# laomao0/BIN

Measured on AMD Instinct MI355X. Metric: interpolated frames/sec at 1280x720, higher is better.
Workload: dtype f16x3 (fp16 hi+lo pairs = 22-bit significands, 3 MFMA products, f32 accumulate; fp32-class: 1e-6 vs the fp32 reference); 1 GPU; Adobe240 test_blur 1280x720 inference, batch=1 per GPU (6-frame window padded to 768x1344 by the test.py rule), window-sharded; precision=f16x3, streams=1, pipelined_steps=False, four_call_schedule=False, parity=max-abs <= 2e-5 (f16x3) vs the fp32 reference (tests/)

## Files before the change

### __graft_entry__.py

```python
import os
import sys

REPO = os.path.dirname(os.path.abspath(__file__))
if REPO not in sys.path:
    sys.path.insert(0, REPO)


def build():
    from bin_amd.build import build_library
    path = build_library(force=True)
    import bin_amd
    from bin_amd import _lib
    lib = _lib.lib()
    missing = [s for s in _lib.exported_symbols() if not hasattr(lib, s)]
    if missing:
        raise RuntimeError(f"libbinhip.so is missing symbols: {missing}")
    _lib.optlib()
    _lib.gradlib()
    _lib.emalib()
    from oracle import rdn_oracle
    print(f"built {path} (binhip version {lib.binhip_version()})")


def smoke():
    import torch
    from bin_amd.models.archs.RDN import bin_stage4_lstm
    from bin_amd.weights import reference_state_dict, canonical_weights, synthetic_frames
    from oracle import rdn_oracle as O

    assert torch.cuda.is_available(), "smoke() needs a GPU"
    dev = torch.device("cuda:0")
    net = bin_stage4_lstm()
    net.load_state_dict(reference_state_dict(0), strict=True)
    net = net.to(dev).eval()
    frames = synthetic_frames(1234, 1, 64, 64, 6)
    canon = {k: torch.from_numpy(v) for k, v in canonical_weights(0).items()}
    with torch.no_grad():
        ref = O.bin_stage4_forward(frames, canon)
        for prec, tol in (("f16x3", 2e-5), ("f16", 1e-3)):
            net.set_precision(prec)
            out = net(*[f.to(dev) for f in frames])
            torch.cuda.synchronize()
            from bin_amd import ops
            ops.check_status()
            err = max(float((a.cpu() - b).abs().max()) for a, b in zip(out, ref))
            print(f"smoke: precision={prec} 14 outputs {tuple(out[13].shape)} max|hip-oracle| = {err:.3e} (tol {tol})")
            assert err <= tol, f"parity failure: {err} > {tol}"
    print("smoke ok")


if __name__ == "__main__":
    build()
    if "--smoke" in sys.argv:
        smoke()
```

### bin_amd/_lib.py

```python
import ctypes as C
import os

from .build import EMA_LIB_PATH, GRAD_LIB_PATH, LIB_PATH, OPT_LIB_PATH

RDN_LAYERS = 66
RDN_MAX_LAYERS, RDN_MAX_CONVS = 192, 7
PLAN_KEEP_ACTS, PLAN_NO_FUSE, PLAN_RDB3, PLAN_FUSED_UPNET, PLAN_FUSED_UPNET_TRAIN = 1, 2, 4, 8, 16
BWD_ACCUMULATE = 1
BWD_SAVED_X3 = 2
BWD_FUSED_UPNET = 4
EPI_PLANES, EPI_SHUFFLE, EPI_FINAL, EPI_FINAL_SUBPIX = 0, 1, 2, 4
PROF_WGRAD = 16
LOSS_CHARBONNIER, LOSS_L1_SUM, LOSS_L2_SUM = 0, 1, 2
RDN_LAYOUT_WORDS, RDN_BWD_LAYOUT_WORDS = 16, 24


class BinConvDesc(C.Structure):
    _fields_ = [("N", C.c_int32), ("H", C.c_int32), ("W", C.c_int32), ("ksize", C.c_int32),
                ("cin_chunks", C.c_int32), ("cout", C.c_int32), ("cout_pad", C.c_int32),
                ("nterms", C.c_int32), ("epilogue", C.c_int32), ("relu", C.c_int32),
                ("x_cpg", C.c_int32), ("x_group_stride", C.c_int64), ("n_images", C.c_int32),
                ("reserved", C.c_int32), ("status", C.c_void_p)]


LOSS_MAX_TERMS = 24
CONV_HALF_LAST_CHUNK = 1


class BinLossTerms(C.Structure):
    _fields_ = [("x", C.c_void_p * LOSS_MAX_TERMS), ("y", C.c_void_p * LOSS_MAX_TERMS), ("n_terms", C.c_int32)]


class BinLossGrads(C.Structure):
    _fields_ = [("out", C.c_void_p * LOSS_MAX_TERMS), ("term_a", C.c_int32 * LOSS_MAX_TERMS),
                ("term_b", C.c_int32 * LOSS_MAX_TERMS), ("sign_a", C.c_float * LOSS_MAX_TERMS),
                ("sign_b", C.c_float * LOSS_MAX_TERMS), ("n_out", C.c_int32)]


class BinRdnShape(C.Structure):
    _fields_ = [("G0", C.c_int32), ("D", C.c_int32), ("C", C.c_int32), ("G", C.c_int32)]


class BinRdnPlan(C.Structure):
    _fields_ = [("N", C.c_int32), ("H", C.c_int32), ("W", C.c_int32), ("n_inputs", C.c_int32),
                ("nterms", C.c_int32), ("reserved", C.c_int32), ("shape", BinRdnShape),
                ("w_hi", C.c_void_p * RDN_MAX_LAYERS), ("w_lo", C.c_void_p * RDN_MAX_LAYERS),
                ("bias", C.c_void_p * RDN_MAX_LAYERS), ("status", C.c_void_p), ("profiler", C.c_void_p)]


class BinRdnBwdPlan(C.Structure):
    _fields_ = [("N", C.c_int32), ("H", C.c_int32), ("W", C.c_int32), ("n_inputs", C.c_int32),
                ("nterms", C.c_int32), ("reserved", C.c_int32), ("shape", BinRdnShape),
                ("wt_hi", C.c_void_p * RDN_MAX_LAYERS), ("wt_lo", C.c_void_p * RDN_MAX_LAYERS),
                ("zero_bias", C.c_void_p),
                ("dw", C.c_void_p * RDN_MAX_LAYERS), ("db", C.c_void_p * RDN_MAX_LAYERS), ("gin", C.c_void_p * 5),
                ("status", C.c_void_p), ("aux_stream", C.c_void_p), ("profiler", C.c_void_p)]


class BinRelayoutItem(C.Structure):
    _fields_ = [("w", C.c_void_p * (RDN_MAX_CONVS + 1)), ("bias", C.c_void_p), ("w_hi", C.c_void_p), ("w_lo", C.c_void_p),
                ("bias_out", C.c_void_p), ("kind", C.c_int32), ("cout", C.c_int32), ("cin", C.c_int32),
                ("ksize", C.c_int32), ("rows_pad", C.c_int32), ("cin_chunks", C.c_int32), ("cout_block", C.c_int32),
                ("shuffle_or_group", C.c_int32), ("shape", BinRdnShape)]


RELAYOUT_FWD, RELAYOUT_DGRAD, RELAYOUT_RDB_GATHER = 0, 1, 2
SCORE_SSIM_G11, SCORE_SSIM_U7 = 1, 2
SCORE_MAX_PAIRS = 32

ADAM_MAX_TENSORS = 64


class BinAdamTensor(C.Structure):
    _fields_ = [("p", C.c_void_p), ("g", C.c_void_p), ("m", C.c_void_p), ("v", C.c_void_p), ("numel", C.c_int64),
                ("step_size", C.c_float), ("inv_sqrt_bc2", C.c_float)]


GRAD_MAX_TENSORS = 128
GRAD_FLAG_NONFINITE, GRAD_FLAG_STATUS = 1, 2


class BinGradTensor(C.Structure):
    _fields_ = [("g", C.c_void_p), ("numel", C.c_int64)]


class BinGradRecord(C.Structure):
    _fields_ = [("sumsq", C.c_double), ("norm", C.c_float), ("coef", C.c_float), ("flags", C.c_int32), ("status", C.c_uint32),
                ("reserved", C.c_int32 * 2)]


EMA_MAX_TENSORS = 136


class BinEmaTensor(C.Structure):
    _fields_ = [("e", C.c_void_p), ("p", C.c_void_p), ("numel", C.c_int64)]


_SIGNATURES = {
    "binhip_version": (C.c_int, []),
    "binhip_device_cus": (C.c_int, []),
    "binhip_conv_cout_block": (C.c_int, [C.c_int, C.c_int, C.c_int]),
    "binhip_weights_bytes": (C.c_size_t, [C.c_int, C.c_int, C.c_int]),
    "binhip_weights_relayout": (C.c_int, [C.c_void_p, C.c_void_p, C.c_int, C.c_int, C.c_int, C.c_int, C.c_int,
                                          C.c_int, C.c_int, C.c_void_p, C.c_void_p, C.c_void_p, C.c_void_p]),
    "binhip_weights_relayout_batch": (C.c_int, [C.POINTER(BinRelayoutItem), C.c_int, C.c_void_p]),
    "binhip_conv2d_fwd": (C.c_int, [C.POINTER(BinConvDesc)] + [C.c_void_p] * 10 +
                          [C.POINTER(C.c_void_p), C.c_void_p]),
    "binhip_nchw_to_planes": (C.c_int, [C.c_void_p, C.c_int, C.c_int, C.c_int, C.c_int, C.c_void_p, C.c_void_p,
                                        C.c_void_p, C.c_void_p]),
    "binhip_planes_to_nchw": (C.c_int, [C.c_void_p, C.c_void_p, C.c_int, C.c_int, C.c_int, C.c_int, C.c_void_p,
                                        C.c_void_p]),
    "binhip_pixel_unshuffle_f32": (C.c_int, [C.c_void_p, C.c_int, C.c_int, C.c_int, C.c_int, C.c_int, C.c_void_p,
                                             C.c_void_p]),
    "binhip_pack_inputs": (C.c_int, [C.POINTER(C.c_void_p), C.c_int, C.c_int, C.c_int, C.c_int, C.c_void_p,
                                     C.c_void_p, C.c_void_p, C.c_void_p]),
    "binhip_u8_to_frame": (C.c_int, [C.c_void_p, C.c_int, C.c_int, C.c_int, C.c_int, C.c_int, C.c_int, C.c_void_p,
                                     C.c_void_p]),
    "binhip_frame_to_u8": (C.c_int, [C.c_void_p, C.c_int, C.c_int, C.c_int, C.c_int, C.c_int, C.c_int, C.c_void_p,
                                     C.c_void_p]),
    "binhip_convlstm_fwd": (C.c_int, [C.c_void_p] * 5 + [C.c_float, C.c_int, C.c_int, C.c_int, C.c_void_p,
                                                          C.c_void_p, C.c_void_p]),
    "binhip_lstm_gates_fwd": (C.c_int, [C.c_void_p, C.c_void_p, C.c_float, C.c_int, C.c_int, C.c_int, C.c_int, C.c_void_p,
                                        C.c_void_p, C.c_void_p]),
    "binhip_lstm_gates_bwd": (C.c_int, [C.c_void_p] * 4 + [C.c_float, C.c_int, C.c_int, C.c_int, C.c_int, C.c_void_p, C.c_void_p,
                                        C.c_void_p]),
    "binhip_charbonnier_partials": (C.c_int, [C.c_int64]),
    "binhip_charbonnier_fwd": (C.c_int, [C.c_void_p, C.c_void_p, C.c_int64, C.c_float, C.c_void_p, C.c_void_p,
                                         C.c_void_p]),
    "binhip_charbonnier_bwd": (C.c_int, [C.c_void_p, C.c_void_p, C.c_int64, C.c_float, C.c_void_p, C.c_void_p,
                                         C.c_void_p, C.c_void_p]),
    "binhip_pixel_loss_fwd": (C.c_int, [C.c_int, C.c_void_p, C.c_void_p, C.c_int64, C.c_float, C.c_void_p, C.c_void_p,
                                        C.c_void_p]),
    "binhip_pixel_loss_bwd": (C.c_int, [C.c_int, C.c_void_p, C.c_void_p, C.c_int64, C.c_float, C.c_void_p, C.c_void_p,
                                        C.c_void_p, C.c_void_p]),
    "binhip_multi_loss_fwd": (C.c_int, [C.c_int, C.POINTER(BinLossTerms), C.c_int64, C.c_float, C.c_void_p, C.c_void_p,
                                        C.c_void_p, C.c_void_p]),
    "binhip_multi_loss_bwd": (C.c_int, [C.c_int, C.POINTER(BinLossTerms), C.c_int64, C.c_float, C.c_void_p,
                                        C.POINTER(BinLossGrads), C.c_void_p]),
    "binhip_dgrad_rows_pad": (C.c_int, [C.c_int, C.c_int]),
    "binhip_weights_relayout_dgrad": (C.c_int, [C.c_void_p, C.c_int, C.c_int, C.c_int, C.c_int, C.c_int, C.c_int,
                                                C.c_int, C.c_void_p, C.c_void_p, C.c_void_p, C.c_void_p]),
    "binhip_weights_relayout_rdb_gather": (C.c_int, [C.c_void_p, C.c_int, C.c_int, C.c_void_p, C.c_void_p, C.c_void_p,
                                                     C.c_void_p]),
    "binhip_conv2d_bwd_data": (C.c_int, [C.POINTER(BinConvDesc)] + [C.c_void_p] * 7 + [C.c_int, C.c_void_p,
                                         C.c_void_p, C.c_void_p, C.c_int, C.c_int, C.c_int64, C.c_void_p,
                                         C.c_void_p, C.c_void_p]),
    "binhip_wgrad_workspace_bytes": (C.c_size_t, [C.c_int] * 6),
    "binhip_conv2d_bwd_weight": (C.c_int, [C.POINTER(BinConvDesc)] + [C.c_void_p] * 6 + [C.c_size_t, C.c_void_p,
# ... 4 lines not shown
    "binhip_unshuffle_planes": (C.c_int, [C.c_void_p, C.c_void_p, C.c_int, C.c_int, C.c_int, C.c_int, C.c_void_p,
                                          C.c_void_p, C.c_void_p]),
    "binhip_unpack_input_grads": (C.c_int, [C.c_void_p, C.c_void_p, C.c_void_p, C.c_void_p, C.c_int, C.c_int, C.c_int,
                                            C.c_int, C.POINTER(C.c_void_p), C.c_void_p]),
    "binhip_convlstm_bwd_workspace_bytes": (C.c_size_t, [C.c_int, C.c_int, C.c_int]),
    "binhip_convlstm_bwd": (C.c_int, [C.c_void_p] * 5 + [C.c_float, C.c_int, C.c_int, C.c_int, C.c_void_p, C.c_void_p,
                                      C.c_void_p, C.c_size_t] + [C.c_void_p] * 6),
    "binhip_rdn_backward_workspace_bytes": (C.c_size_t, [C.c_int] * 5 + [C.POINTER(BinRdnShape)]),
    "binhip_rdn_backward": (C.c_int, [C.POINTER(BinRdnBwdPlan), C.c_void_p, C.c_size_t, C.c_void_p, C.c_void_p,
                                      C.c_size_t, C.c_void_p]),
    "binhip_profiler_create": (C.c_int, [C.c_int, C.c_int, C.c_int, C.c_int, C.POINTER(C.c_void_p)]),
    "binhip_profiler_read": (C.c_int, [C.c_void_p, C.POINTER(C.c_double), C.POINTER(C.c_int)]),
    "binhip_profiler_destroy": (None, [C.c_void_p]),
    "binhip_rdb_tail_fwd": (C.c_int, [C.c_int, C.c_int, C.c_int, C.c_int] + [C.c_void_p] * 10 +
                            [C.c_int, C.c_void_p, C.c_void_p]),
    "binhip_rdn_workspace_bytes": (C.c_size_t, [C.c_int, C.c_int, C.c_int, C.c_int, C.c_int, C.POINTER(BinRdnShape)]),
    "binhip_rdn_workspace_layout": (C.c_int, [C.c_int] * 5 + [C.POINTER(BinRdnShape), C.POINTER(C.c_int64), C.c_int]),
    "binhip_rdn_backward_workspace_layout": (C.c_int, [C.c_int] * 5 + [C.POINTER(BinRdnShape), C.POINTER(C.c_int64), C.c_int]),
    "binhip_rdn_forward": (C.c_int, [C.POINTER(BinRdnPlan), C.POINTER(C.c_void_p), C.c_void_p, C.c_void_p,
                                     C.c_size_t, C.c_void_p]),
    "binhip_image_score_workspace_bytes": (C.c_size_t, [C.c_int] * 4),
    "binhip_image_score": (C.c_int, [C.c_void_p, C.c_void_p, C.c_int, C.c_int, C.c_int, C.c_int, C.POINTER(C.c_double),
                                     C.c_void_p, C.c_size_t, C.c_void_p, C.c_void_p]),
    "binhip_frame_score_workspace_bytes": (C.c_size_t, [C.c_int] * 4),
    "binhip_frame_score": (C.c_int, [C.POINTER(C.c_void_p), C.POINTER(C.c_void_p), C.c_int, C.c_int, C.c_int, C.c_int,
                                     C.POINTER(C.c_double), C.c_void_p, C.c_size_t, C.c_void_p, C.c_void_p]),
    "binhip_gather_windows": (C.c_int, [C.c_void_p, C.c_int, C.c_int, C.c_int, C.c_void_p, C.c_int, C.c_int, C.c_int, C.c_int,
                                        C.c_void_p, C.c_void_p]),
    "binhip_gather_windows_blur": (C.c_int, [C.c_void_p, C.c_int, C.c_int, C.c_int, C.c_void_p] + [C.c_int] * 5 +
                                   [C.c_void_p, C.c_void_p]),
}

OPT_VERSION = 100
_OPT_SIGNATURES = {
    "binopt_version": (C.c_int, []),
    "binopt_adam_step": (C.c_int, [C.POINTER(BinAdamTensor), C.c_int, C.c_float, C.c_float, C.c_float, C.c_float, C.c_void_p]),
}

GRAD_VERSION = 100
_GRAD_SIGNATURES = {
    "bingrad_version": (C.c_int, []),
    "bingrad_norm_workspace_bytes": (C.c_int64, [C.POINTER(BinGradTensor), C.c_int]),
    "bingrad_norm": (C.c_int, [C.POINTER(BinGradTensor), C.c_int, C.c_float, C.c_void_p, C.c_uint32, C.c_void_p, C.c_void_p,
                               C.c_void_p]),
    "bingrad_scale": (C.c_int, [C.POINTER(BinGradTensor), C.c_int, C.c_void_p, C.c_void_p]),
}

EMA_VERSION = 100
_EMA_SIGNATURES = {
    "binema_version": (C.c_int, []),
    "binema_step": (C.c_int, [C.POINTER(BinEmaTensor), C.c_int, C.c_float, C.c_void_p]),
}

STATUS_SATURATED = 1
STATUS_SYNC_TIMEOUT = 2

_lib = None


def exported_symbols():
    return sorted(_SIGNATURES)


def lib():
    global _lib
    if _lib is None:
        path = os.environ.get("BIN_AMD_LIB", LIB_PATH)
        if not os.path.exists(path):
            raise RuntimeError(
                f"bin_amd: HIP library {LIB_PATH} not built. Run `python -c 'import __graft_entry__ as g; "
                f"g.build()'` (hipcc --offload-arch=gfx950). There is no CPU fallback by design.")
        h = C.CDLL(path)
        for name, (res, args) in _SIGNATURES.items():
            fn = getattr(h, name)
            fn.restype = res
            fn.argtypes = args
        _lib = h
    return _lib


_optlib = None


def opt_exported_symbols():
    return sorted(_OPT_SIGNATURES)


def optlib():
    global _optlib
    if _optlib is None:
        path = OPT_LIB_PATH
        if not os.path.exists(path):
            raise RuntimeError(
                f"bin_amd: HIP library {OPT_LIB_PATH} not built. Run `python -c 'import __graft_entry__ as g; "
                f"g.build()'` (hipcc --offload-arch=gfx950). There is no CPU fallback by design.")
        h = C.CDLL(path)
        for name, (res, args) in _OPT_SIGNATURES.items():
            fn = getattr(h, name)
            fn.restype = res
            fn.argtypes = args
        if h.binopt_version() != OPT_VERSION:
            raise RuntimeError(f"bin_amd: {path} is version {h.binopt_version()}, this binding is for {OPT_VERSION}")
        _optlib = h
    return _optlib


_gradlib = None


def grad_exported_symbols():
    return sorted(_GRAD_SIGNATURES)


def gradlib():
    global _gradlib
    if _gradlib is None:
        path = GRAD_LIB_PATH
        if not os.path.exists(path):
            raise RuntimeError(
                f"bin_amd: HIP library {GRAD_LIB_PATH} not built. Run `python -c 'import __graft_entry__ as g; "
                f"g.build()'` (hipcc --offload-arch=gfx950). There is no CPU fallback by design.")
        h = C.CDLL(path)
        for name, (res, args) in _GRAD_SIGNATURES.items():
            fn = getattr(h, name)
            fn.restype = res
            fn.argtypes = args
        if h.bingrad_version() != GRAD_VERSION:
            raise RuntimeError(f"bin_amd: {path} is version {h.bingrad_version()}, this binding is for {GRAD_VERSION}")
        _gradlib = h
    return _gradlib


_emalib = None


def ema_exported_symbols():
    return sorted(_EMA_SIGNATURES)


def emalib():
    global _emalib
    if _emalib is None:
        path = EMA_LIB_PATH
        if not os.path.exists(path):
            raise RuntimeError(
                f"bin_amd: HIP library {EMA_LIB_PATH} not built. Run `python -c 'import __graft_entry__ as g; "
                f"g.build()'` (hipcc --offload-arch=gfx950). There is no CPU fallback by design.")
        h = C.CDLL(path)
        for name, (res, args) in _EMA_SIGNATURES.items():
            fn = getattr(h, name)
            fn.restype = res
            fn.argtypes = args
        if h.binema_version() != EMA_VERSION:
            raise RuntimeError(f"bin_amd: {path} is version {h.binema_version()}, this binding is for {EMA_VERSION}")
        _emalib = h
    return _emalib


def check(rc, what):
    if rc != 0:
        kind = {-1: "bad argument", -2: "unsupported shape", -3: "workspace too small"}.get(rc, f"hipError {rc}")
        raise RuntimeError(f"bin_amd: {what} failed: {kind}")
```

### bin_amd/autograd.py

```python
import ctypes as C
import os

import torch

from . import _lib as L
from .ops import _ptr, _stream, on_device, status_word
from .rdn_plan import c_shape, layer_names, rdn_forward, workspace



def default_wgrad_side_stream():
    return os.environ.get("BIN_AMD_WGRAD_STREAM", "1") != "0"


_aux_streams = {}


def _aux_stream(device):
    s = _aux_streams.get(device.index)
    if s is None:
        s = torch.cuda.Stream(device=device)
        _aux_streams[device.index] = s
    return s


def train_fused_upnet():
    return os.environ.get("BIN_AMD_FUSED_UPNET_TRAIN", "1") != "0"


def default_backward_precision():
    return os.environ.get("BIN_AMD_BACKWARD_PRECISION") or None


def train_precision(module):
    from .models.archs.RDN import PRECISIONS
    p = module.precision or os.environ.get("BIN_AMD_TRAIN_PRECISION", "f16x3")
    if PRECISIONS[p] == 1 and not getattr(module, "allow_f16_training", False):
        if not any(q.requires_grad for q in module.parameters()):
            if not getattr(module, "_warned_f16_input_grads", False):
                import warnings
                warnings.warn("bin_amd: differentiating through an RDN in precision 'f16' with frozen parameters: input gradients "
                              "are computed with single fp16 products (a few per cent of noise); use 'f16x3' for fp32-class gradients",
                              stacklevel=3)
                module._warned_f16_input_grads = True
            return PRECISIONS[p]
        raise RuntimeError(
            "bin_amd: training with precision 'f16' (one fp16 product in forward and backward) is not a supported mode — its "
            "parameter gradients are only verified to 25 %.  Train in 'f16x3' (the default; set network_G.precision: f16x3 or "
            "leave it unset), optionally with network_G.backward_precision: f16 for the faster mixed mode; 'f16' is the "
            "inference mode (wrap inference in torch.no_grad()).  To train in it regardless (it converged like f16x3 on the synthetic "
            "task of profiles/r06_training_modes.md) set network_G.allow_f16_training: true, or module.allow_f16_training = True.")
    return PRECISIONS[p]


class _RdnFn(torch.autograd.Function):
    @staticmethod
    def forward(ctx, module, nterms, n_frames, *args):
        frames = [a.contiguous().float() for a in args[:n_frames]]
        weights = module.kernel_weights(nterms)
        n, _, h, w = frames[0].shape
        lib = L.lib()
        nbytes = lib.binhip_rdn_workspace_bytes(n, h, w, n_frames, nterms, C.byref(c_shape(weights.shape)))
        if nbytes == 0:
            raise RuntimeError(f"bin_amd: unsupported RDN shape N={n} H={h} W={w}")
        saved = torch.empty(nbytes, dtype=torch.uint8, device=frames[0].device)
        fused = (bool(module.plan_flags & L.PLAN_FUSED_UPNET) and train_fused_upnet() and
                 weights.ensure_fused_upnet(train=True) is not None)
        flags = module.plan_flags | L.PLAN_KEEP_ACTS | (L.PLAN_FUSED_UPNET_TRAIN if fused else 0)
        out = rdn_forward(weights, frames, ws=saved, flags=flags, profiler=module.profiler)
        ctx.fused_up = fused
        if module.debug_hook is not None:
            module.debug_hook("forward", module, (n, h, w, n_frames, nterms), saved, {"shape": module.shape, "fused_upnet": fused})
        ctx.module, ctx.nterms, ctx.n_frames = module, nterms, n_frames
        ctx.saved_ws = saved
        ctx.weights = weights
        ctx.dims = (n, h, w)
        ctx.param_meta = [(tuple(a.shape), a.device) for a in args[n_frames:]]
        ctx.params = args[n_frames:]
        ctx.param_versions = [(a._version, a.data_ptr()) for a in args[n_frames:]]
        ctx.weights_gen = module._wgen
        module._bwd_pending = getattr(module, "_bwd_pending", 0) + 1
        ctx.owes_backward = True
        return out

    @staticmethod
    def backward(ctx, gout):
        if ctx.saved_ws is None:
            raise RuntimeError("bin_amd: the saved activations of this RDN call were released by an earlier backward through it (the "
                               "forward's private workspace is freed as soon as its backward has run or was refused; "
                               "retain_graph=True does not keep it): run the forward again")
        try:
            return _RdnFn._backward(ctx, gout)
        except BaseException:
            ctx.saved_ws = ctx.weights = None
            _RdnFn._settle(ctx)
            raise

    @staticmethod
    def _settle(ctx):
        if ctx.owes_backward:
            ctx.owes_backward = False
            ctx.module._bwd_pending = getattr(ctx.module, "_bwd_pending", 1) - 1

    @staticmethod
    def _backward(ctx, gout):
        module, nterms, k = ctx.module, ctx.nterms, ctx.n_frames
        n, h, w = ctx.dims
        if ctx.weights_gen != module._wgen or any((a._version, a.data_ptr()) != v for a, v in zip(ctx.params, ctx.param_versions)):
            raise RuntimeError("bin_amd: a parameter of this RDN was modified in place between its forward and its backward "
                               "(optimizer step, load_state_dict, broadcast, re-pointed storage ...): the gradient would be computed with "
                               "weights the forward did not use")
        dev = gout.device
        gout = gout.contiguous().float()
        lib = L.lib()
        weights = ctx.weights
        fused = ctx.fused_up
        nt_bwd = 1 if (module.backward_precision == "f16" and nterms == 3) else nterms
        dgw = weights.dgrad(module, nt_bwd, fused=fused)
        plan = L.BinRdnBwdPlan()
        plan.N, plan.H, plan.W, plan.n_inputs, plan.nterms = n, h, w, k, nt_bwd
        if nt_bwd != nterms:
            plan.reserved = L.BWD_SAVED_X3
        dgw.fill_plan(plan)
        plan.status = status_word(dev).data_ptr()
        plan.aux_stream = (_aux_stream(dev).cuda_stream
                           if module.wgrad_side_stream and not torch.cuda.is_current_stream_capturing() else None)
        plan.profiler = module.bwd_profiler if module.bwd_profiler else None
        params = ctx.params
        direct = module._direct_grads and all(ctx.needs_input_grad[3 + k:])
        have = False
        if direct:
            states = [p.grad is not None for p in params]
            have = all(states)
            direct = (have or not any(states)) and all(
                p.grad is None or (p.grad.dtype == torch.float32 and p.grad.is_contiguous() and p.grad.device == dev)
                for p in params)
        if direct and have:
            grads = [p.grad for p in params]
            plan.reserved |= L.BWD_ACCUMULATE
        else:
            grads = [torch.empty(shape, dtype=torch.float32, device=dev) for shape, _ in ctx.param_meta]
        for i in range(len(grads) // 2):
            plan.dw[i] = grads[2 * i].data_ptr()
            plan.db[i] = grads[2 * i + 1].data_ptr()
        if fused:
            nl, g0 = len(grads) // 2, module.shape[0]
            plan.reserved |= L.BWD_FUSED_UPNET
            up_dw4 = torch.empty((12, g0, 5, 5), dtype=torch.float32, device=dev)
            up_db4 = torch.empty((12,), dtype=torch.float32, device=dev)
            up_dwr = torch.zeros((n, 9, 12, 25, g0), dtype=torch.float32, device=dev)
            up_dbr = torch.zeros((n, 9, 12), dtype=torch.float32, device=dev)
            plan.dw[nl], plan.db[nl], plan.dw[nl + 1], plan.db[nl + 1] = (up_dw4.data_ptr(), up_db4.data_ptr(), up_dwr.data_ptr(),
                                                                        up_dbr.data_ptr())
        gins = []
        for i in range(k):
            if ctx.needs_input_grad[3 + i]:
                g = torch.empty((n, 3, h, w), dtype=torch.float32, device=dev)
                plan.gin[i] = g.data_ptr()
                gins.append(g)
            else:
                plan.gin[i] = None
                gins.append(None)
        nbytes = lib.binhip_rdn_backward_workspace_bytes(n, h, w, k, nt_bwd, C.byref(plan.shape))
        ws = workspace(nbytes, dev, key="bwd")
        with on_device(gout):
            L.check(lib.binhip_rdn_backward(C.byref(plan), _ptr(ctx.saved_ws), ctx.saved_ws.numel(), _ptr(gout),
                                            _ptr(ws), ws.numel(), _stream()), "rdn_backward")
        if module.debug_hook is not None:
            module.debug_hook("backward", module, (n, h, w, k, nt_bwd), ws, {"input_grads": any(g is not None for g in gins),
                                                                              "shape": module.shape, "fused_upnet": fused})
        ctx.saved_ws = ctx.weights = None
        if fused:
            nl = len(grads) // 2
            dW = up_dwr.sum(0)
            dB = up_dbr.sum(0)
            dW[4], dB[4] = up_dw4.reshape(12, g0, 25).permute(0, 2, 1), up_db4
            leaves, Wr, Br = weights.fused_graph
            gup = torch.autograd.grad([Wr, Br], leaves, [dW, dB], retain_graph=True)
            for slot, g in zip((2 * (nl - 2), 2 * (nl - 2) + 1, 2 * (nl - 1), 2 * (nl - 1) + 1), gup):
                if plan.reserved & L.BWD_ACCUMULATE:
                    grads[slot].add_(g.float())
                else:
                    grads[slot].copy_(g.float())
        _RdnFn._settle(ctx)
        if module._bwd_pending == 0 and direct:
            cb = getattr(module, "_grads_ready_cb", None)
            if cb is not None:
                cb()
        if direct:
            if not have:
                for p, g in zip(params, grads):
                    p.grad = g
            return (None, None, None, *gins, *([None] * len(grads)))
        pgrads = [g if ctx.needs_input_grad[3 + k + i] else None for i, g in enumerate(grads)]
        return (None, None, None, *gins, *pgrads)


def rdn_apply(module, frames):
    nterms = train_precision(module)
    params = dict(module.named_parameters())
    flat = []
    for nm in layer_names(module.shape):
        flat += [params[nm + ".weight"], params[nm + ".bias"]]
    return _RdnFn.apply(module, nterms, len(frames), *frames, *flat)


class _ConvLstmFn(torch.autograd.Function):
    @staticmethod
    def forward(ctx, x, c_prev, h_prev, weight, bias, forget_bias):
        from . import ops
        state = None if c_prev is None else [c_prev, h_prev]
        h, (c, _) = ops.convlstm_cell(x, state, weight, bias, forget_bias)
        ctx.save_for_backward(x.contiguous().float(), None if c_prev is None else c_prev.contiguous().float(),
                              None if h_prev is None else h_prev.contiguous().float(),
                              weight.detach().contiguous().float(), bias.detach().contiguous().float())
        ctx.fb = float(forget_bias)
        return h, c

    @staticmethod
    def backward(ctx, gh, gc):
        x, cp, hp, w, b = ctx.saved_tensors
        n, _, hh, ww = x.shape
        dev = x.device
        lib = L.lib()
        gh = gh.contiguous().float() if gh is not None else None
        gc = gc.contiguous().float() if gc is not None else None
        if gh is None and gc is None:
            return None, None, None, None, None, None
        gx = torch.empty_like(x) if ctx.needs_input_grad[0] else None
        gcp = torch.empty_like(x) if (cp is not None and ctx.needs_input_grad[1]) else None
        ghp = torch.empty_like(x) if (hp is not None and ctx.needs_input_grad[2]) else None
        need_w = ctx.needs_input_grad[3] or ctx.needs_input_grad[4]
        dw = torch.zeros_like(w) if need_w else None
        db = torch.zeros_like(b) if need_w else None
        ws = workspace(lib.binhip_convlstm_bwd_workspace_bytes(n, hh, ww), dev, key="clstm")
        L.check(lib.binhip_convlstm_bwd(_ptr(x), _ptr(cp), _ptr(hp), _ptr(w), _ptr(b), ctx.fb, n, hh, ww, _ptr(gh),
                                        _ptr(gc), _ptr(ws), ws.numel(), _ptr(gx), _ptr(ghp), _ptr(gcp), _ptr(dw),
                                        _ptr(db), _stream()), "convlstm_bwd")
        return gx, gcp, ghp, dw, db, None


GENERAL_NTERMS = 3


class _ConvFn(torch.autograd.Function):

    @staticmethod
    def forward(ctx, x, weight, bias):
        from . import ops
        nt = GENERAL_NTERMS
        cw = ops.ConvWeights(weight, bias, nterms=nt)
        xp = ops.nchw_to_planes(x, nt)
        y = ops.planes_to_nchw(ops.conv2d(xp, cw), weight.shape[0])
        ctx.xp, ctx.weight, ctx.has_bias = xp, weight, bias is not None
        ctx.weight_version = weight._version
        return y

    @staticmethod
    def backward(ctx, gy):
        from . import ops
        nt = GENERAL_NTERMS
        if ctx.weight._version != ctx.weight_version:
            raise RuntimeError("bin_amd: a ConvLSTM gate weight was modified in place between forward and backward "
                               "(optimizer step / broadcast / load_state_dict): its gradient would not belong to the forward")
        cout, cin, ks, _ = ctx.weight.shape
        gp, sc = ops.grad_planes(gy, nt)
        dw = db = gx = None
        if ctx.needs_input_grad[1] or ctx.needs_input_grad[2]:
            dw, db = ops.conv2d_bwd_weight(ctx.xp, gp, cout, cin, ks, nt, inv_scale=sc[1:2])
        if ctx.needs_input_grad[0]:
            gxs = ops.planes_to_nchw(ops.conv2d_bwd_data(gp, ops.DgradWeights(ctx.weight, nterms=nt)), cin)
            gx = gxs * sc[1]
        return gx, dw, (db if ctx.has_bias else None)


class _LstmGatesFn(torch.autograd.Function):
    @staticmethod
    def forward(ctx, gates, c_prev, forget_bias, hidden):
        from . import ops
        c1, h1 = ops.lstm_gates(gates, c_prev, forget_bias, hidden)
        ctx.save_for_backward(gates, c_prev)
        ctx.fb, ctx.hidden = float(forget_bias), hidden
        return h1, c1

    @staticmethod
    def backward(ctx, gh, gc):
        from . import ops
# ... 24 lines not shown
```

### bin_amd/build.py

```python
import os
import subprocess
import sys

HERE = os.path.dirname(os.path.abspath(__file__))
CSRC = os.path.join(HERE, "csrc")
SOURCES = ["binhip_conv.hip", "binhip_conv_x3.hip", "binhip_fused.hip", "binhip_fused_x3.hip", "binhip_wgrad.hip", "binhip_misc.hip", "binhip_plan.hip",
           "binhip_metrics.hip", "binhip_data.hip"]
LIB_PATH = os.path.join(CSRC, "libbinhip.so")
OPT_SOURCES = ["binopt_adam.hip"]
OPT_LIB_PATH = os.path.join(CSRC, "libbinopt.so")
OPT_HEADER = os.path.join(os.path.dirname(HERE), "include", "binopt.h")
GRAD_SOURCES = ["bingrad_norm.hip"]
GRAD_LIB_PATH = os.path.join(CSRC, "libbingrad.so")
GRAD_HEADER = os.path.join(os.path.dirname(HERE), "include", "bingrad.h")
EMA_SOURCES = ["binema_step.hip"]
EMA_LIB_PATH = os.path.join(CSRC, "libbinema.so")
EMA_HEADER = os.path.join(os.path.dirname(HERE), "include", "binema.h")


HEADER = os.path.join(os.path.dirname(HERE), "include", "binhip.h")


def abi_symbols():
    import re
    with open(HEADER) as f:
        return re.findall(r"(?m)^BINHIP_API\s+[\w\s\*]+?\b(binhip_\w+)\s*\(", f.read())


def opt_abi_symbols():
    import re
    with open(OPT_HEADER) as f:
        return re.findall(r"(?m)^BINOPT_API\s+[\w\s\*]+?\b(binopt_\w+)\s*\(", f.read())


def grad_abi_symbols():
    import re
    with open(GRAD_HEADER) as f:
        return re.findall(r"(?m)^BINGRAD_API\s+[\w\s\*]+?\b(bingrad_\w+)\s*\(", f.read())


def ema_abi_symbols():
    import re
    with open(EMA_HEADER) as f:
        return re.findall(r"(?m)^BINEMA_API\s+[\w\s\*]+?\b(binema_\w+)\s*\(", f.read())


def _stale():
    libs = (LIB_PATH, OPT_LIB_PATH, GRAD_LIB_PATH, EMA_LIB_PATH)
    if not all(os.path.exists(p) for p in libs):
        return True
    t = min(os.path.getmtime(p) for p in libs)
    deps = [os.path.join(CSRC, f) for f in os.listdir(CSRC) if f.endswith((".hip", ".h"))]
    deps += [os.path.join(os.path.dirname(HERE), "include", "binhip.h"), OPT_HEADER, GRAD_HEADER, EMA_HEADER]
    return any(os.path.getmtime(d) > t for d in deps)


def build_library(force=False, verbose=True, defines=(), out=None):
    lib_path = out or LIB_PATH
    if out is None and not force and not _stale():
        return LIB_PATH
    hipcc = os.environ.get("HIPCC", "/opt/rocm/bin/hipcc")
    objdir = CSRC if out is None else os.path.dirname(os.path.abspath(out))
    os.makedirs(objdir, exist_ok=True)
    tag = "" if out is None else "." + os.path.splitext(os.path.basename(out))[0]
    procs, objs, opt_objs, grad_objs, ema_objs = [], [], [], [], []
    for src in SOURCES + (OPT_SOURCES + GRAD_SOURCES + EMA_SOURCES if out is None else []):
        obj = os.path.join(objdir, src.replace(".hip", tag + ".o"))
        cmd = [hipcc, "--offload-arch=gfx950", "-O3", "-std=c++17", "-fPIC", "-fvisibility=hidden"] + [f"-D{d}" for d in defines] + \
              ["-c", os.path.join(CSRC, src), "-o", obj]
        if verbose:
            print(" ".join(cmd), file=sys.stderr)
        procs.append((cmd, subprocess.Popen(cmd)))
        (opt_objs if src in OPT_SOURCES else grad_objs if src in GRAD_SOURCES else ema_objs if src in EMA_SOURCES else objs).append(obj)
    for cmd, p in procs:
        if p.wait() != 0:
            raise subprocess.CalledProcessError(p.returncode, cmd)
    vmap = os.path.join(objdir, "binhip_exports" + tag + ".map")
    names = abi_symbols() + (["binhip_set_timeline"] if any(d.startswith("BINHIP_TIMELINE") for d in defines) else [])
    with open(vmap, "w") as f:
        f.write("{\n  global:\n" + "".join(f"    {n};\n" for n in names) + "  local: *;\n};\n")
    cmd = [hipcc, "--offload-arch=gfx950", "-shared", "-fPIC", "-Wl,-z,defs", f"-Wl,--version-script={vmap}",
           "-o", lib_path] + objs
    if verbose:
        print(" ".join(cmd), file=sys.stderr)
    subprocess.check_call(cmd)
    for name, symbols, path, lib_objs in ((("binopt", opt_abi_symbols(), OPT_LIB_PATH, opt_objs),
                                           ("bingrad", grad_abi_symbols(), GRAD_LIB_PATH, grad_objs),
                                           ("binema", ema_abi_symbols(), EMA_LIB_PATH, ema_objs)) if out is None else ()):
        vmap = os.path.join(objdir, f"binhip_exports.{name}.map")
        with open(vmap, "w") as f:
            f.write("{\n  global:\n" + "".join(f"    {n};\n" for n in symbols) + "  local: *;\n};\n")
        cmd = [hipcc, "--offload-arch=gfx950", "-shared", "-fPIC", "-Wl,-z,defs", f"-Wl,--version-script={vmap}",
               "-o", path] + lib_objs
        if verbose:
            print(" ".join(cmd), file=sys.stderr)
        subprocess.check_call(cmd)
    return lib_path


if __name__ == "__main__":
    build_library(force="--force" in sys.argv)
    print(LIB_PATH)
```

### bin_amd/csrc/binhip_conv.hip

```cpp
#include "binhip_conv_common.h"
#include <vector>
#include <cstdio>
#include <cstdlib>

template <int KS, int MT, int WM, int R, int WN, int KC, int NT, int NBUF, int EPI>
struct ConvCfg {
    static constexpr int PAD = KS / 2;
    static constexpr int COUTB = 32 * MT * WM;
    static constexpr int TH = R * WN;
    static constexpr int PH = TH + KS - 1;
    static constexpr int PW = 32 + KS - 1;
    static constexpr int PP = (PH * PW * 2 + 63) / 64;
    static constexpr int WP = KS * KS * MT * WM;
    static constexpr int CHUNK_BYTES = (PP + WP) * 1024;
    static constexpr int NPL = (NT == 3) ? 2 : 1;
    static constexpr int PLANE_BYTES = KC * CHUNK_BYTES;
    static constexpr int BUF_BYTES = NPL * PLANE_BYTES;
    static constexpr int NW = WM * WN;
    static constexpr int LDS_BYTES = NBUF * BUF_BYTES + 1024;
    static constexpr int NPJ = (PP + NW - 1) / NW;
    static constexpr int NWJ = (WP + NW - 1) / NW;
    static constexpr int PS = NPL * KC * (NPJ + NWJ);
    static_assert(NW == 4 || NW == 8 || NW == 16, "4, 8 or 16 waves per workgroup");
    static_assert(LDS_BYTES <= 160 * 1024, "LDS budget");
// ... 221 lines not shown
    int ks = 0, cout_pad = 0, epi = 0;
    std::vector<hipEvent_t> ev;
    size_t used = 0;
};
namespace { constexpr size_t PROF_MAX_PAIRS = 16384; }

int bh_conv_cout_block(int ksize, int cout_pad, int nterms) {
    if (cout_pad <= 0 || cout_pad % 32) return -1;
    if (ksize == 3 && nterms == 3) return 32;
    if (ksize == 3 && cout_pad == 256) return 128;
    if (ksize == 5) return 32;
    if (ksize == 1 && cout_pad == 224) return 224;
    if (ksize == 1 && cout_pad == 1152) return 192;
    if (cout_pad % 96 == 0) return 96;
    if (ksize == 3 && cout_pad % 64 == 0) return 64;
    return 32;
}

static int bh_dispatch_conv(const ConvKArgs& a, int k, int cp, int nt, int e, hipStream_t s);
int bh_launch_conv_x3(const ConvKArgs& a, int cout_pad, int epilogue, hipStream_t s);
int bh_launch_final_dot2(const ConvKArgs& a, hipStream_t s);
int bh_launch_conv_x3_k5(const ConvKArgs& a, int cout_pad, hipStream_t s);
int bh_launch_conv_x3_k5_subpix(const ConvKArgs& a, hipStream_t s);
int bh_launch_final_m16(const ConvKArgs& a, hipStream_t s);

int bh_prepare_conv(const BhConvCall& c, ConvKArgs* out) {
    const BinConvDesc& d = c.d;
    if (!c.x_hi || !c.w_hi || !c.bias) return BINHIP_E_ARG;
    if (d.nterms != 1 && d.nterms != 3) return BINHIP_E_ARG;
    if (d.nterms == 3 && (!c.x_lo || !c.w_lo)) return BINHIP_E_ARG;
    if (d.N <= 0 || d.H <= 0 || d.W <= 0 || d.cin_chunks <= 0) return BINHIP_E_SHAPE;
    if ((long long)d.N * d.H * d.W >= (1ll << 26)) return BINHIP_E_SHAPE;
    ConvKArgs a;
    a.x_hi = (const _Float16*)c.x_hi; a.x_lo = (const _Float16*)c.x_lo;
    a.w_hi = (const _Float16*)c.w_hi; a.w_lo = (const _Float16*)c.w_lo;
    a.bias = c.bias;
    a.y_hi = (_Float16*)c.y_hi; a.y_lo = (_Float16*)c.y_lo;
    a.r_hi = (const _Float16*)c.r_hi; a.r_lo = (const _Float16*)c.r_lo;
    a.r2_hi = (const _Float16*)c.r2_hi; a.r2_lo = (const _Float16*)c.r2_lo;
    a.m_hi = (const _Float16*)c.m_hi;
    a.flags = (unsigned*)c.status;
    a.res_chunks = c.res_chunks > 0 ? c.res_chunks : (1 << 30);
    a.mask_from = c.mask_from;
    a.y_cpg = c.y_cpg; a.y_group_stride = c.y_group_stride;
    a.y_cpg_inv = c.y_cpg > 0 ? (unsigned)(((1u << 20) + c.y_cpg - 1) / c.y_cpg) : 0u;
    if (c.y_cpg > 128 || (c.y_cpg > 0 && d.cout_pad / 16 >= 4096)) return BINHIP_E_SHAPE;
    a.half_last = (d.reserved & BINHIP_CONV_HALF_LAST_CHUNK) ? 1 : 0;
    a.y_unshuf = c.y_unshuf;
    if (c.y_unshuf && (d.epilogue != BINHIP_EPI_PLANES || c.y_cpg > 0 || (d.H & 1) || (d.W & 1) || c.y_unshuf * 16 < d.cout))
        return BINHIP_E_SHAPE;
    if (c.r2_hi && d.nterms == 3 && !c.r2_lo) return BINHIP_E_ARG;
    a.out_f32 = c.y_f32;
    for (int i = 0; i < 5; ++i) a.img[i] = c.images[i];
    a.group_stride = d.x_group_stride;
    a.N = d.N; a.H = d.H; a.W = d.W;
    a.nchunks = d.cin_chunks;
    a.cpg = d.x_cpg;
    a.relu = d.relu; a.has_res = (c.r_hi != nullptr); a.nimg = d.n_images; a.cout = d.cout;
    a.och_limit = (d.epilogue == BINHIP_EPI_PLANES) ? (d.cout + 15) / 16 : (1 << 30);
    a.tiles_x = a.tiles_y = 0;
    a.ncol = 1;
    a.xcd_remap = 1;
    a.dbg = 0;
    a.wt = 0;
    a.prog_prio = 0;
#if BINHIP_TIMELINE
    a.tl = nullptr; a.tl_launch = 0; a.tl_base = 0;
#endif
    const int P = BINHIP_EPI_PLANES, S = BINHIP_EPI_SHUFFLE, F = BINHIP_EPI_FINAL;
    if (d.epilogue == P) {
        if (!c.y_hi || (d.nterms == 3 && !c.y_lo)) return BINHIP_E_ARG;
        if (a.has_res && d.nterms == 3 && !c.r_lo) return BINHIP_E_ARG;
    } else if (d.epilogue == S) {
        if (!c.y_hi || (d.nterms == 3 && !c.y_lo)) return BINHIP_E_ARG;
        if (d.cout % 4) return BINHIP_E_SHAPE;
    } else if (d.epilogue == F) {
        if (!c.y_f32 || d.cout > 4 || d.n_images < 0 || d.n_images > 5) return BINHIP_E_ARG;
    } else if (d.epilogue == BINHIP_EPI_FINAL_SUBPIX) {
        if (!c.y_f32 || d.cout <= 0 || (d.cout & 3) || d.cout > 12 || d.n_images < 0 || d.n_images > 5) return BINHIP_E_ARG;
        if (d.ksize != 5 || d.cout_pad != 32) return BINHIP_E_SHAPE;
    } else {
        return BINHIP_E_ARG;
    }
    {
        const int e = d.epilogue, cp = d.cout_pad;
        const long long out_chunks = (e == BINHIP_EPI_SHUFFLE) ? (a.cout / 4 + 15) / 16 : (cp + 15) / 16;
        const long long px = (long long)a.N * a.H * a.W * ((e == BINHIP_EPI_SHUFFLE) ? 4 : 1);
        const long long span = (a.y_cpg > 0 ? ((out_chunks + a.y_cpg - 1) / a.y_cpg) * a.y_group_stride * 2 : out_chunks * px * 32);
        a.wt = (e == BINHIP_EPI_PLANES && span < (1ll << 32) - 64) ? 1 : 0;
    }
    *out = a;
    return 0;
}

bool bh_prof_begin(BinhipProfiler* pr, int ks, int cout_pad, int epi, hipStream_t s) {
    if (!pr || ks != pr->ks || cout_pad != pr->cout_pad || epi != pr->epi || pr->used + 2 > pr->ev.size()) return false;
    (void)hipEventRecord(pr->ev[pr->used], s);
    return true;
}
void bh_prof_end(BinhipProfiler* pr, hipStream_t s) {
    (void)hipEventRecord(pr->ev[pr->used + 1], s);
    pr->used += 2;
}

int bh_launch_conv(const BhConvCall& c, hipStream_t s) {
    ConvKArgs a;
// ... 407 lines not shown
```

### bin_amd/csrc/binhip_conv_common.h

```cpp
#pragma once
#include "binhip_internal.h"
#ifndef BINHIP_TIMELINE
#define BINHIP_TIMELINE 0
#endif

typedef _Float16 half8 __attribute__((ext_vector_type(8)));
typedef _Float16 half4 __attribute__((ext_vector_type(4)));
typedef float floatx16 __attribute__((ext_vector_type(16)));
typedef float floatx4 __attribute__((ext_vector_type(4)));
typedef __attribute__((address_space(3))) void lds_void_t;
typedef unsigned u32x4 __attribute__((ext_vector_type(4)));

int bh_launch_upnet_ring(const void* x_hi, const void* x_lo, const float* wvar, const float* bvar, float* out, const float* const* images,
                         int nimg, int N, int H, int W, int cin, hipStream_t s);
int bh_upnet_gsub(const float* g, int N, int H, int W, const float* scale, void* y_hi, void* y_lo, void* status, hipStream_t s);
int bh_upnet_ring_dgrad(const float* g, const float* wvar, const float* scale, void* gx_hi, void* gx_lo, void* status, int N, int H, int W,
                        int cin, hipStream_t s);
int bh_upnet_ring_wgrad(const float* g, const void* x_hi, const void* x_lo, float* dwvar, float* dbvar, int N, int H, int W, int cin,
                        int accumulate, hipStream_t s);
struct ConvKArgs {
    const _Float16* x_hi;
    const _Float16* x_lo;
    const _Float16* w_hi;
    const _Float16* w_lo;
    const float* bias;
    _Float16* y_hi;
    _Float16* y_lo;
    const _Float16* r_hi;
    const _Float16* r_lo;
    const _Float16* r2_hi;
    const _Float16* r2_lo;
    const _Float16* m_hi;
    float* out_f32;
    const float* img[5];
    unsigned* flags;
    long long group_stride;
    int N, H, W;
    int nchunks;
    int cpg;
    int tiles_x, tiles_y;
    int ncol;
    int relu, has_res, nimg, cout;
    int xcd_remap;
    int wt;
    int och_limit;
    int dbg;
    int res_chunks;
    int mask_from;
    int y_cpg;
    unsigned y_cpg_inv;
    long long y_group_stride;
    int prog_prio;
    int half_last;
#if BINHIP_TIMELINE
    void* tl;
    unsigned tl_launch;
    unsigned tl_base;
#endif
    int y_unshuf;
};

#if BINHIP_TIMELINE
#include <atomic>
struct BhTlRec {
    unsigned kind_launch, bid, hwid, xcc;
    unsigned long long rt[5];
    unsigned long long clk[2];
    unsigned long long pad;
};
static_assert(sizeof(BhTlRec) == 80, "record size (tools/wg_timeline.py)");
struct BhTlBuf { unsigned cursor, cap, pad[2]; BhTlRec rec[1]; };
inline void* g_bh_tl_buf = nullptr;
inline unsigned g_bh_tl_cap = 0;
inline std::atomic<unsigned> g_bh_tl_serial{0}, g_bh_tl_next{0};
inline void* bh_tl_reserve(unsigned n, unsigned* base) {
    if (!g_bh_tl_buf) return nullptr;
    const unsigned b = g_bh_tl_next.fetch_add(n);
    *base = b;
    return (b + n <= g_bh_tl_cap) ? g_bh_tl_buf : nullptr;
}
struct BhTl {
    unsigned long long rt[5], clk[2];
    __device__ __forceinline__ void stamp(int i) {
        __builtin_amdgcn_sched_barrier(0);
        rt[i] = __builtin_amdgcn_s_memrealtime();
        __builtin_amdgcn_sched_barrier(0);
    }
    __device__ __forceinline__ void begin() { clk[0] = __builtin_amdgcn_s_memtime(); stamp(0); }
    __device__ __forceinline__ void finish(void* tl, unsigned kind_launch, unsigned i) {
        stamp(3);
        if (threadIdx.x < 64) asm volatile("s_waitcnt vmcnt(0)" ::: "memory");
        stamp(4);
        clk[1] = __builtin_amdgcn_s_memtime();
        if (tl && threadIdx.x == 0) {
            BhTlBuf* b = (BhTlBuf*)tl;
            {
                BhTlRec& r = b->rec[i];
                r.kind_launch = kind_launch; r.bid = blockIdx.x;
                r.hwid = __builtin_amdgcn_s_getreg((31 << 11) | 4);
                r.xcc = __builtin_amdgcn_s_getreg((31 << 11) | 20);
                for (int k = 0; k < 5; ++k) r.rt[k] = rt[k];
                r.clk[0] = clk[0]; r.clk[1] = clk[1];
            }
        }
    }
};
#define BH_TL_DECL BhTl tl__
#define BH_TL_BEGIN() tl__.begin()
#define BH_TL_STAMP(i) tl__.stamp(i)
#define BH_TL_FINISH(a, i) tl__.finish((a).tl, (a).tl_launch, (a).tl_base + (unsigned)(i))
#else
#define BH_TL_DECL
#define BH_TL_BEGIN()
#define BH_TL_STAMP(i)
#define BH_TL_FINISH(a, i)
#endif

#define BINHIP_EPI_PLANES_LFFD 3

template <int N>
__device__ __forceinline__ void wait_vmcnt() {
    asm volatile("s_waitcnt vmcnt(%0)" ::"n"(N) : "memory");
}

__device__ __forceinline__ void store16(_Float16* base, long long off_elems, uint4 v, int wt) {
    if (wt) {
        __amdgpu_buffer_rsrc_t rs = __builtin_amdgcn_make_buffer_rsrc((void*)base, 0, 0xFFFFFFFFu, 0x00020000);
        u32x4 d = {v.x, v.y, v.z, v.w};
        __builtin_amdgcn_raw_buffer_store_b128(d, rs, (int)(off_elems * 2), 0, 16);
    } else {
        *reinterpret_cast<uint4*>(base + off_elems) = v;
    }
}

__device__ __forceinline__ int xcd_band(int bid, int nwg) {
    const int q = nwg >> 3, r = nwg & 7, xcd = bid & 7, k = bid >> 3;
    return (xcd < r ? xcd * (q + 1) : r * (q + 1) + (xcd - r) * q) + k;
}

template <int MT, int R, int NT, int EPI, bool XTRA>
__device__ __forceinline__ void conv_epilogue(const ConvKArgs& a, const float* __restrict__ bias, floatx16 (&acc)[MT][R],
                                              int img, int row0, int tx0, int co0, bool first_col, int n, int kg,
                                              long long plane_elems) {
    const int H = a.H, W = a.W;
    const int gx = tx0 + n;
    auto bias4 = [&](int co_u, float (&bv)[4]) {
        float b8[8];
#pragma unroll
        for (int j = 0; j < 8; ++j) b8[j] = bias[co_u + j];
#pragma unroll
        for (int j = 0; j < 4; ++j) bv[j] = kg ? b8[4 + j] : b8[j];
    };
    if constexpr (EPI == BINHIP_EPI_FINAL_SUBPIX) {
        const int ncolour = a.cout >> 2;
        const int H2 = 2 * H, W2 = 2 * W;
        float bv[2][4];
        bias4(co0, bv[0]);
        bias4(co0 + 8, bv[1]);
        const bool col_ok = first_col && (gx < W);
        float sum[R][2][4];
#pragma unroll
        for (int r = 0; r < R; ++r) {
            const int gy = row0 + r;
#pragma unroll
            for (int g = 0; g < 2; ++g) {
                const int c = 2 * g + kg;
                const bool ok = col_ok && gy < H && c < ncolour;
#pragma unroll
                for (int q = 0; q < 4; ++q) {
                    float sj = 0.f;
                    if (ok && a.nimg > 0) {
                        const long long idx = (((long long)img * ncolour + c) * H2 + 2 * gy + (q >> 1)) * W2 + 2 * gx + (q & 1);
                        sj = a.img[0][idx];
                        for (int t = 1; t < a.nimg; ++t) sj += a.img[t][idx];
                        sj = sj / (float)a.nimg;
                    }
                    sum[r][g][q] = sj;
                }
            }
        }
#pragma unroll
        for (int r = 0; r < R; ++r) {
            const int gy = row0 + r;
#pragma unroll
            for (int g = 0; g < 2; ++g) {
                const int c = 2 * g + kg;
                if (!(col_ok && gy < H && c < ncolour)) continue;
#pragma unroll
                for (int q = 0; q < 4; ++q) {
                    const long long idx = (((long long)img * ncolour + c) * H2 + 2 * gy + (q >> 1)) * W2 + 2 * gx + (q & 1);
                    a.out_f32[idx] = (acc[0][r][4 * g + q] + bv[g][q]) + sum[r][g][q];
                }
            }
        }
    } else if constexpr (EPI == BINHIP_EPI_FINAL) {
        float bv[4];
        bias4(co0, bv);
        const bool mine = (kg == 0) && first_col && (gx < W);
        float sum[R][4];
#pragma unroll
        for (int r = 0; r < R; ++r) {
            const int gy = row0 + r;
#pragma unroll
            for (int j = 0; j < 4; ++j) {
                float sj = 0.f;
                if (mine && gy < H && j < a.cout && a.nimg > 0) {
                    const long long idx = (((long long)img * a.cout + j) * H + gy) * W + gx;
                    sj = a.img[0][idx];
                    for (int t = 1; t < a.nimg; ++t) sj += a.img[t][idx];
                    sj = sj / (float)a.nimg;
                }
                sum[r][j] = sj;
            }
        }
#pragma unroll
        for (int r = 0; r < R; ++r) {
            const int gy = row0 + r;
            if (!(mine && gy < H)) continue;
#pragma unroll
            for (int j = 0; j < 4; ++j) {
                if (j >= a.cout) break;
                const long long idx = (((long long)img * a.cout + j) * H + gy) * W + gx;
                a.out_f32[idx] = (acc[0][r][j] + bv[j]) + sum[r][j];
            }
        }
    } else {
        union H4 { half4 h; unsigned u[2]; };
        unsigned sat = 0;
        const int gxc = gx < W ? gx : W - 1;
        constexpr bool X = XTRA && (EPI == BINHIP_EPI_PLANES || EPI == BINHIP_EPI_PLANES_LFFD);
        constexpr int MTG = (X && MT >= 6) ? 2 : 1;
        const bool use_res = X && a.has_res;
        const bool use_r2 = X && (a.r2_hi != nullptr);
        const bool use_m = X && (a.m_hi != nullptr);
        constexpr bool LFFD = EPI == BINHIP_EPI_PLANES_LFFD;
        static_assert(!LFFD || (XTRA && MT == 7 && NT == 3), "the LFF backward-data epilogue");
        if constexpr (LFFD) {
            {
#pragma unroll
                for (int r = 0; r < R; ++r) {
                    const int gy = row0 + r;
                    const bool ok = (gy < H) && (gx < W);
                    const int gyc = gy < H ? gy : H - 1;
                    const long long pix = (((long long)img * H + gyc) * W + gxc) << 4;
                    auto emit = [&](const int mt, const half4 (&xr)[4], const half4 (&xrl)[4], const half4 (&xm)[4], const int kind)
                        __attribute__((always_inline)) {
#pragma unroll
                        for (int gp = 0; gp < 2; ++gp) {
                            H4 hv[2], lv[2];
                            long long o_slot = 0;
#pragma unroll
                            for (int ge = 0; ge < 2; ++ge) {
                                const int g = 2 * gp + ge;
                                float bv[4];
                                bias4(mt * 32 + 8 * g, bv);
                                float v[4] = {acc[mt][r][4 * g + 0] + bv[0], acc[mt][r][4 * g + 1] + bv[1],
                                              acc[mt][r][4 * g + 2] + bv[2], acc[mt][r][4 * g + 3] + bv[3]};
                                const int co = mt * 32 + 8 * g + 4 * kg;
                                const long long o = (long long)(co >> 4) * plane_elems + pix + (co & 15);
                                if (kind == 1) {
#pragma unroll
                                    for (int j = 0; j < 4; ++j) v[j] += (float)xr[g][j];
// ... 208 lines not shown
```

### bin_amd/csrc/binhip_conv_x3.hip

```cpp
#include "binhip_conv_common.h"
constexpr int X3_R = 2, X3_WN = 8;

template <int KS, int R, int WN>
struct X3Cfg {
    static constexpr int PAD = KS / 2;
    static constexpr int TH = R * WN;
    static constexpr int PH = TH + KS - 1;
    static constexpr int PW = 32 + KS - 1;
    static constexpr int PP = (PH * PW * 2 + 63) / 64;
    static constexpr int WP = KS * KS;
    static constexpr int NW = WN;
    static constexpr int PATCH_BYTES = PP * 1024;
    static constexpr int WBUF_BYTES = 2 * WP * 1024;
    static constexpr int LDS_BYTES = 2 * PATCH_BYTES + 2 * WBUF_BYTES;
    static constexpr int NPJ = (PP + NW - 1) / NW;
    static constexpr int NWJ = (2 * WP + NW - 1) / NW;
    static_assert((KS == 3 ? 2 : 1) * LDS_BYTES <= 160 * 1024, "LDS budget");
};

template <class C>
__device__ __forceinline__ void x3_issue_patch(const ConvKArgs& a, char* smem, int c, int pl, int buf, int wave,
                                               const unsigned* voff, long long plane_elems, unsigned plane_bytes) {
    const _Float16* xb = pl ? a.x_lo : a.x_hi;
    const long long coff = (a.cpg > 0) ? (long long)(c / a.cpg) * a.group_stride + (long long)(c % a.cpg) * plane_elems
// ... 414 lines not shown
    union W2 { unsigned u; half2v p; };

    const int nchunks = a.nchunks;
    auto compute = [&](const char* pb, int c, bool hi_plane) {
        const unsigned* wh = w_hi32 + (long long)c * (9 * 32 * 8);
        const unsigned* wl = w_lo32 + (long long)c * (9 * 32 * 8);
#pragma unroll
        for (int t = 0; t < 9; ++t) {
            const int dy = t / 3, dx = t % 3;
#pragma unroll
            for (int cg = 0; cg < 2; ++cg) {
                X8 x;
                x.h = *reinterpret_cast<const half8*>(pb + cg * (C::PH * C::PW * 16) + base_off + (dy * C::PW + dx) * 16);
#pragma unroll
                for (int r = 0; r < 3; ++r) {
#pragma unroll
                    for (int k = 0; k < 4; ++k) {
                        W2 w;
                        w.u = wh[(t * 32 + r) * 8 + cg * 4 + k];
                        acc[r] = __builtin_amdgcn_fdot2(x.p[k], w.p, acc[r], false);
                        if (NT == 3 && hi_plane) {
                            W2 v;
                            v.u = wl[(t * 32 + r) * 8 + cg * 4 + k];
                            acc[r] = __builtin_amdgcn_fdot2(x.p[k], v.p, acc[r], false);
                        }
                    }
                }
            }
        }
    };

    x3_issue_patch<C>(a, smem, 0, 0, 0, wave, voff, plane_elems, plane_bytes);
    for (int c = 0; c < nchunks; ++c) {
        wait_vmcnt<0>();
        __builtin_amdgcn_s_barrier();
        __builtin_amdgcn_sched_barrier(0);
        if constexpr (NT == 3) {
            x3_issue_patch<C>(a, smem, c, 1, 1, wave, voff, plane_elems, plane_bytes);
            compute(smem, c, true);
            wait_vmcnt<0>();
            __builtin_amdgcn_s_barrier();
            __builtin_amdgcn_sched_barrier(0);
            if (c + 1 < nchunks) x3_issue_patch<C>(a, smem, c + 1, 0, 0, wave, voff, plane_elems, plane_bytes);
            compute(smem + C::PATCH_BYTES, c, false);
        } else {
            if (c + 1 < nchunks) x3_issue_patch<C>(a, smem, c + 1, 0, (c + 1) & 1, wave, voff, plane_elems, plane_bytes);
            compute(smem + (c & 1) * C::PATCH_BYTES, c, true);
        }
    }
    const int gy = ty0 + py, gx = tx0 + px;
    if (gy < H && gx < W) {
        float sum[3], bj[3];
        const int nimg = a.nimg;
#pragma unroll
        for (int j = 0; j < 3; ++j) {
            const long long idx = (((long long)img * a.cout + (j < a.cout ? j : 0)) * H + gy) * W + gx;
            float v[5];
#pragma unroll
            for (int t = 0; t < 5; ++t) v[t] = (t < nimg) ? a.img[t][idx] : 0.f;
            bj[j] = a.bias[j < a.cout ? j : 0];
            float sj = v[0];
#pragma unroll
            for (int t = 1; t < 5; ++t)
                if (t < nimg) sj += v[t];
            sum[j] = nimg > 0 ? sj / (float)nimg : 0.f;
        }
#pragma unroll
        for (int j = 0; j < 3; ++j) asm volatile("" : "+v"(sum[j]), "+v"(bj[j]));
        __builtin_amdgcn_sched_barrier(0);
#pragma unroll
        for (int j = 0; j < 3; ++j) {
            if (j >= a.cout) break;
            const long long idx = (((long long)img * a.cout + j) * H + gy) * W + gx;
            a.out_f32[idx] = (acc[j] + bj[j]) + sum[j];
        }
    }
}

struct M16 {
    using C = X3Cfg<3, 2, 8>;
    static constexpr int NSTAGE = 3;
    static constexpr int WPIECES = 5;
    static constexpr int W_OFF = NSTAGE * C::PATCH_BYTES;
    static constexpr int LDS_BYTES = W_OFF + 2 * WPIECES * 1024;
    static_assert(2 * LDS_BYTES <= 160 * 1024, "two workgroups per CU");
};

template <bool HI>
__device__ __forceinline__ void m16_compute(const char* pb, const char* wb, int a_lane_off, int b_lane_off, int slot, int a_zero,
                                            floatx4 (&acc)[2][2]) {
    using C = X3Cfg<3, 2, 8>;
    half8 Ah[2], Al[2], B[2][2][2];
    auto tap_off = [](int t) { return ((t / 3) * C::PW + (t % 3)) * 16; };
    auto load = [&](int p, half8& ah, half8& al, half8 (&b)[2][2]) {
        const int aoff = (p < 4) ? (2 * p + slot) * 128 + a_lane_off : (slot ? 8 * 128 + a_zero : 8 * 128 + a_lane_off);
        ah = x3_ld8(wb + aoff);
        if constexpr (HI) al = x3_ld8(wb + M16::WPIECES * 1024 + aoff);
        const int boff = b_lane_off + tap_off(2 * p) + slot * (p < 4 ? tap_off(2 * p + 1) - tap_off(2 * p) : 0);
#pragma unroll
        for (int r = 0; r < 2; ++r)
#pragma unroll
            for (int g = 0; g < 2; ++g) b[r][g] = x3_ld8(pb + boff + (r * C::PW + g * 16) * 16);
    };
    load(0, Ah[0], Al[0], B[0]);
#pragma unroll
    for (int p = 0; p < 5; ++p) {
        if (p + 1 < 5) load(p + 1, Ah[(p + 1) & 1], Al[(p + 1) & 1], B[(p + 1) & 1]);
        __builtin_amdgcn_sched_barrier(0);
#pragma unroll
        for (int r = 0; r < 2; ++r)
#pragma unroll
            for (int g = 0; g < 2; ++g) {
// ... 29 lines not shown
        const int q = i * 64 + lane;
        const int cg = q >= C::PH * C::PW ? 1 : 0;
        const int p = q - cg * (C::PH * C::PW);
        const int py = p / C::PW;
        const int px = p - py * C::PW;
        const int gy = ty0 + py - 1;
        const int gx = tx0 + px - 1;
        const bool ok = (p < C::PH * C::PW) && (gy >= 0) && (gy < H) && (gx >= 0) && (gx < W);
        voff[j] = ok ? (unsigned)((((long long)img * H + gy) * W + gx) * 32 + cg * 16) : 0x80000000u;
    }
    const int n16 = lane & 15, kb = lane >> 4;
    const int slot = kb >> 1;
    const int a_lane_off = ((n16 < 3 ? n16 : 3) * 2 + (kb & 1)) * 16;
    const int a_zero = (3 * 2 + (kb & 1)) * 16;
    const int b_lane_off = ((kb & 1) * (C::PH * C::PW) + wave * 2 * C::PW + n16) * 16;
    floatx4 acc[2][2];
#pragma unroll
    for (int r = 0; r < 2; ++r)
#pragma unroll
        for (int g = 0; g < 2; ++g) acc[r][g] = floatx4{0.f, 0.f, 0.f, 0.f};

    const int nchunks = a.nchunks;
    const int nstage = 2 * nchunks;
    {
        const int ntaps = nchunks * 9;
        for (int i = wave; i < 2 * M16::WPIECES; i += C::NW) {
            const int pl = i >= M16::WPIECES ? 1 : 0;
            const int t = (i - pl * M16::WPIECES) * 8 + (lane >> 3);
            __amdgpu_buffer_rsrc_t rs = __builtin_amdgcn_make_buffer_rsrc((void*)(pl ? a.w_lo : a.w_hi), 0, (unsigned)(ntaps * 1024), 0x00020000);
            const unsigned off = t < ntaps ? (unsigned)(t * 1024 + (lane & 7) * 16) : 0x80000000u;
            __builtin_amdgcn_raw_ptr_buffer_load_lds(rs, (lds_void_t*)(smem + M16::W_OFF + i * 1024), 16, off, 0, 0, 0);
        }
    }
    x3_issue_patch<C>(a, smem, 0, 0, 0, wave, voff, plane_elems, plane_bytes);
    if (nstage > 1) x3_issue_patch<C>(a, smem, 0, 1, 1, wave, voff, plane_elems, plane_bytes);
    const bool three = wave < (C::PP - 2 * C::NW);
    for (int s = 0; s < nstage; ++s) {
        if (s + 1 < nstage) {
            if (three) wait_vmcnt<3>(); else wait_vmcnt<2>();
        } else {
            wait_vmcnt<0>();
        }
        __builtin_amdgcn_s_barrier();
        __builtin_amdgcn_sched_barrier(0);
        if (s + 2 < nstage) x3_issue_patch<C>(a, smem, (s + 2) >> 1, (s + 2) & 1, (s + 2) % 3, wave, voff, plane_elems, plane_bytes);
        const char* pb = smem + (s % 3) * C::PATCH_BYTES;
        const char* wb = smem + M16::W_OFF + (s >> 1) * (9 * 128);
        if (s & 1) m16_compute<false>(pb, wb, a_lane_off, b_lane_off, slot, a_zero, acc);
        else m16_compute<true>(pb, wb, a_lane_off, b_lane_off, slot, a_zero, acc);
    }
    if (kb == 0) {
        float sum[2][2][3];
        const int nimg = a.nimg;
#pragma unroll
        for (int r = 0; r < 2; ++r)
#pragma unroll
            for (int g = 0; g < 2; ++g) {
                const int gy = ty0 + wave * 2 + r, gx = tx0 + g * 16 + n16;
                const bool ok = gy < H && gx < W;
                const int gyc = gy < H ? gy : H - 1, gxc = gx < W ? gx : W - 1;
#pragma unroll
                for (int j = 0; j < 3; ++j) {
                    const long long idx = (((long long)img * a.cout + (j < a.cout ? j : 0)) * H + gyc) * W + gxc;
                    float v[5];
#pragma unroll
                    for (int t = 0; t < 5; ++t) v[t] = (t < nimg) ? a.img[t][idx] : 0.f;
                    float sj = v[0];
#pragma unroll
                    for (int t = 1; t < 5; ++t)
                        if (t < nimg) sj += v[t];
                    sum[r][g][j] = (ok && nimg > 0) ? sj / (float)nimg : 0.f;
                }
            }
        float bj[3];
#pragma unroll
        for (int j = 0; j < 3; ++j) bj[j] = bias[j < a.cout ? j : 0];
#pragma unroll
        for (int r = 0; r < 2; ++r)
#pragma unroll
            for (int g = 0; g < 2; ++g)
#pragma unroll
                for (int j = 0; j < 3; ++j) asm volatile("" : "+v"(sum[r][g][j]));
#pragma unroll
        for (int j = 0; j < 3; ++j) asm volatile("" : "+v"(bj[j]));
        __builtin_amdgcn_sched_barrier(0);
#pragma unroll
        for (int r = 0; r < 2; ++r)
#pragma unroll
            for (int g = 0; g < 2; ++g) {
                const int gy = ty0 + wave * 2 + r, gx = tx0 + g * 16 + n16;
                if (gy >= H || gx >= W) continue;
#pragma unroll
                for (int j = 0; j < 3; ++j) {
                    if (j >= a.cout) break;
                    const long long idx = (((long long)img * a.cout + j) * H + gy) * W + gx;
                    a.out_f32[idx] = (acc[r][g][j] + bj[j]) + sum[r][g][j];
                }
            }
    }
}

int bh_launch_final_m16(const ConvKArgs& ka, hipStream_t s) {
    using C = X3Cfg<3, 2, 8>;
    static std::atomic<unsigned long long> lds_set{0};
    if (ka.nchunks * 9 > M16::WPIECES * 8) return BINHIP_E_SHAPE;
    if (int rc = bh_set_max_lds(&final_m16_kernel, M16::LDS_BYTES, lds_set)) return rc;
    ConvKArgs a = ka;
    a.tiles_x = (a.W + 31) / 32;
    a.tiles_y = (a.H + C::TH - 1) / C::TH;
    a.ncol = 1;
    final_m16_kernel<<<dim3((unsigned)(a.tiles_x * a.tiles_y * a.N)), dim3(512), M16::LDS_BYTES, s>>>(a, a.bias);
    BH_CHECK_LAUNCH();
    return 0;
}

int bh_launch_final_dot2(const ConvKArgs& ka, hipStream_t s) {
    using C = X3Cfg<3, 2, 4>;
    ConvKArgs a = ka;
    a.tiles_x = (a.W + 31) / 32;
    a.tiles_y = (a.H + C::TH - 1) / C::TH;
    a.ncol = 1;
    dim3 grid((unsigned)(a.tiles_x * a.tiles_y * a.N));
    const unsigned* wh = reinterpret_cast<const unsigned*>(a.w_hi);
    final_dot2_kernel<1><<<grid, dim3(256), 2 * C::PATCH_BYTES, s>>>(a, wh, wh);
    BH_CHECK_LAUNCH();
    return 0;
}

int bh_launch_conv_x3_k5(const ConvKArgs& a, int cout_pad, hipStream_t s) {
    return launch_x3<5, X3_R, X3_WN, BINHIP_EPI_PLANES, 1>(a, cout_pad, s);
}

int bh_launch_conv_x3_k5_subpix(const ConvKArgs& a, hipStream_t s) {
    return launch_x3<5, X3_R, X3_WN, BINHIP_EPI_FINAL_SUBPIX, 0>(a, 32, s);
}

struct RingArgs {
    const _Float16* x_hi;
    const _Float16* x_lo;
    const float* wvar;
    const float* bvar;
    float* out;
    const float* img[5];
    int N, H, W, cin, nimg;
};
constexpr int RING_THREADS = 128;
__global__ void __launch_bounds__(RING_THREADS) upnet_ring_kernel(const RingArgs a) {
    __shared__ float red[3][RING_THREADS / 64];
    const int tid = threadIdx.x, lane = tid & 63, wave = tid >> 6;
    const int H = a.H, W = a.W, H2 = 2 * H, W2 = 2 * W;
    const int ring = 2 * W2 + 2 * (H2 - 2);
    int id = blockIdx.x;
    const int img = id / ring;
    id -= img * ring;
    int Y, X;
    if (id < W2) { Y = 0; X = id; }
    else if (id < 2 * W2) { Y = H2 - 1; X = id - W2; }
    else { const int k = id - 2 * W2; Y = 1 + (k >> 1); X = (k & 1) ? W2 - 1 : 0; }
    const int y = Y >> 1, i = Y & 1, x = X >> 1, j = X & 1;
    const int vy = (Y == 0) ? 0 : (Y == H2 - 1 ? 2 : 1), vx = (X == 0) ? 0 : (X == W2 - 1 ? 2 : 1);
    const int var = 3 * vy + vx, sub = 2 * i + j;
    const int cin = a.cin, ng = cin >> 3, items = 25 * ng;
    const long long wstride = (long long)25 * cin;
    const float* w = a.wvar + ((long long)var * 12 + sub) * wstride;
    float s0 = 0.f, s1 = 0.f, s2 = 0.f;
    for (int it = tid; it < items; it += RING_THREADS) {
        const int tap = it / ng, ci = (it - tap * ng) << 3;
        const int yy = y + tap / 5 - 2, xx = x + tap % 5 - 2;
        if (yy < 0 || yy >= H || xx < 0 || xx >= W) continue;
        const long long o = (((((long long)(ci >> 4) * a.N + img) * H + yy) * W + xx) << 4) + (ci & 15);
        const half8 xh = *reinterpret_cast<const half8*>(a.x_hi + o);
        half8 xl;
        if (a.x_lo) xl = *reinterpret_cast<const half8*>(a.x_lo + o);
        const float* wq = w + (long long)tap * cin + ci;
        floatx4 wa[3][2];
#pragma unroll
        for (int c = 0; c < 3; ++c) {
            wa[c][0] = *reinterpret_cast<const floatx4*>(wq + 4 * c * wstride);
            wa[c][1] = *reinterpret_cast<const floatx4*>(wq + 4 * c * wstride + 4);
        }
#pragma unroll
        for (int e = 0; e < 8; ++e) {
            float v = (float)xh[e];
            if (a.x_lo) v += (float)xl[e];
            s0 = fmaf(wa[0][e >> 2][e & 3], v, s0);
            s1 = fmaf(wa[1][e >> 2][e & 3], v, s1);
            s2 = fmaf(wa[2][e >> 2][e & 3], v, s2);
        }
    }
#pragma unroll
    for (int off = 32; off > 0; off >>= 1) {
        s0 += __shfl_xor(s0, off);
        s1 += __shfl_xor(s1, off);
        s2 += __shfl_xor(s2, off);
    }
    if (lane == 0) { red[0][wave] = s0; red[1][wave] = s1; red[2][wave] = s2; }
    __syncthreads();
    if (tid < 3) {
        const int c = tid;
        const float v = red[c][0] + red[c][1];
        const long long idx = (((long long)img * 3 + c) * H2 + Y) * W2 + X;
        float m = 0.f;
        if (a.nimg > 0) {
            m = a.img[0][idx];
            for (int t = 1; t < a.nimg; ++t) m += a.img[t][idx];
            m = m / (float)a.nimg;
        }
        a.out[idx] = (v + a.bvar[var * 12 + 4 * c + sub]) + m;
    }
}
int bh_launch_upnet_ring(const void* x_hi, const void* x_lo, const float* wvar, const float* bvar, float* out, const float* const* images,
                         int nimg, int N, int H, int W, int cin, hipStream_t s) {
    if (!x_hi || !wvar || !bvar || !out || N <= 0 || H <= 0 || W <= 0 || cin <= 0 || (cin & 15) || nimg < 0 || nimg > 5) return BINHIP_E_ARG;
    RingArgs a;
    a.x_hi = (const _Float16*)x_hi; a.x_lo = (const _Float16*)x_lo; a.wvar = wvar; a.bvar = bvar; a.out = out;
    for (int t = 0; t < 5; ++t) a.img[t] = (t < nimg) ? images[t] : nullptr;
    a.N = N; a.H = H; a.W = W; a.cin = cin; a.nimg = nimg;
    const long long ring = 4ll * W + 4ll * H - 4;
    upnet_ring_kernel<<<dim3((unsigned)(ring * N)), dim3(RING_THREADS), 0, s>>>(a);
    BH_CHECK_LAUNCH();
    return 0;
}

int bh_launch_conv_x3(const ConvKArgs& a, int cout_pad, int epilogue, hipStream_t s) {
    if (epilogue == BINHIP_EPI_PLANES)
        return cout_pad == 32 ? launch_x3<3, X3_R, X3_WN, BINHIP_EPI_PLANES, 0>(a, cout_pad, s)
                              : launch_x3<3, X3_R, X3_WN, BINHIP_EPI_PLANES, 1>(a, cout_pad, s);
    if (epilogue == BINHIP_EPI_SHUFFLE) return launch_x3<3, X3_R, X3_WN, BINHIP_EPI_SHUFFLE, 1>(a, cout_pad, s);
    if (epilogue == BINHIP_EPI_FINAL) return launch_x3<3, X3_R, X3_WN, BINHIP_EPI_FINAL, 0>(a, cout_pad, s);
    return BINHIP_E_SHAPE;
}
```

### bin_amd/csrc/binhip_internal.h

```cpp
#pragma once
#include <hip/hip_runtime.h>
#include <stdint.h>
#include "../../include/binhip.h"


static inline int64_t bh_plane_elems(int N, int H, int W) { return (int64_t)N * H * W * 16; }
static inline int bh_chunks(int C) { return (C + 15) / 16; }
__device__ static inline int bh_chunks_dev(int C) { return (C + 15) / 16; }

#define BH_CHECK_LAUNCH()                                   \
    do {                                                    \
        hipError_t e__ = hipGetLastError();                 \
        if (e__ != hipSuccess) return (int)e__;             \
    } while (0)

#define BINHIP_F16_MAX 65504.0f
#define BINHIP_FLAG_SATURATED 1u

__device__ __forceinline__ _Float16 split_hi(float v, unsigned& sat) {
    sat |= !(fabsf(v) <= BINHIP_F16_MAX) ? 1u : 0u;
    return (_Float16)__builtin_amdgcn_fmed3f(v, -BINHIP_F16_MAX, BINHIP_F16_MAX);
}
__device__ __forceinline__ _Float16 split_lo(float v, _Float16 hi) {
    return (_Float16)(__builtin_amdgcn_fmed3f(v, -BINHIP_F16_MAX, BINHIP_F16_MAX) - (float)hi);
}

__device__ __forceinline__ void split_pair(float a, float b, unsigned& sat, unsigned& hi2, unsigned& lo2, bool relu = false) {
    const unsigned smask = relu ? 0xffffffffu : 0x7fffffffu;
    const float lb = relu ? 0.f : -BINHIP_F16_MAX;
    sat |= !(__uint_as_float(__float_as_uint(a) & smask) <= BINHIP_F16_MAX) ? 1u : 0u;
    sat |= !(__uint_as_float(__float_as_uint(b) & smask) <= BINHIP_F16_MAX) ? 1u : 0u;
    const float ac = __builtin_amdgcn_fmed3f(a, lb, BINHIP_F16_MAX);
    const float bc = __builtin_amdgcn_fmed3f(b, lb, BINHIP_F16_MAX);
    unsigned h, l;
    asm("v_cvt_pk_f16_f32 %0, %1, %2" : "=v"(h) : "v"(ac), "v"(bc));
    asm("v_fma_mixlo_f16 %0, %1, -1.0, %2 op_sel_hi:[1,0,0]" : "=v"(l) : "v"(h), "v"(ac));
    asm("v_fma_mixhi_f16 %0, %1, -1.0, %2 op_sel:[1,0,0] op_sel_hi:[1,0,0]" : "+v"(l) : "v"(h), "v"(bc));
    hi2 = h; lo2 = l;
}

struct BhConvCall {
    BinConvDesc d;
    const void *x_hi, *x_lo, *w_hi, *w_lo;
    const float* bias;
    const void *r_hi, *r_lo;
    const void *r2_hi = nullptr, *r2_lo = nullptr;
    const void* m_hi = nullptr;
    int res_chunks = 0;
    int mask_from = 0;
    int y_cpg = 0;
    int64_t y_group_stride = 0;
    int y_unshuf = 0;
    void *y_hi, *y_lo;
    float* y_f32;
    const float* images[5];
    void* status = nullptr;
    BinhipProfiler* prof = nullptr;
};
int bh_launch_conv(const BhConvCall& c, hipStream_t s);
bool bh_prof_begin(BinhipProfiler* pr, int ks, int cout_pad, int epi, hipStream_t s);
void bh_prof_end(BinhipProfiler* pr, hipStream_t s);
struct ConvKArgs;
int bh_prepare_conv(const BhConvCall& c, ConvKArgs* out);
int bh_launch_rdb3_x3(const ConvKArgs* convs, unsigned* flags, unsigned epoch, int cus, hipStream_t s);

#define BH_WGRAD_BATCH 8
struct BhWgradReduce {
    const float* partial;
    const float* partial_b;
    float* dw;
    float* db;
    long long nrows;
    int PB, ncp, ncot, ks, tr, cout, cin, shuffle;
};
int bh_wgrad_partials(const BinConvDesc* d, const void* x_hi, const void* x_lo, const void* gy_hi, const void* gy_lo,
                      void* workspace, size_t workspace_bytes, float* dw_oihw, float* dbias, int cin, int shuffle_perm,
                      BhWgradReduce* out, void* stream);
int bh_wgrad_reduce_batch(const BhWgradReduce* items, int n, const float* inv_scale, int accumulate, void* stream);
int bh_conv_cout_block(int ksize, int cout_pad, int nterms);

#include <atomic>
template <class K>
static inline int bh_set_max_lds(K kernel, int bytes, std::atomic<unsigned long long>& done) {
    int dev = 0;
    hipError_t e = hipGetDevice(&dev);
    if (e != hipSuccess) return (int)e;
    const unsigned long long bit = 1ull << (dev & 63);
    if (done.load(std::memory_order_acquire) & bit) return 0;
    e = hipFuncSetAttribute(reinterpret_cast<const void*>(kernel), hipFuncAttributeMaxDynamicSharedMemorySize, bytes);
    if (e != hipSuccess) return (int)e;
    done.fetch_or(bit, std::memory_order_release);
    return 0;
}
```

### bin_amd/csrc/binhip_misc.hip

```cpp
#include "binhip_internal.h"

typedef _Float16 half8 __attribute__((ext_vector_type(8)));

__global__ void nchw_to_planes_kernel(const float* __restrict__ x, int N, int C, int H, int W,
                                      _Float16* __restrict__ y_hi, _Float16* __restrict__ y_lo,
                                      const float* __restrict__ scale, unsigned* __restrict__ flags) {
    const float sc = scale ? scale[0] : 1.f;
    const long long HW = (long long)H * W;
    const long long total = (long long)bh_chunks_dev(C) * N * HW * 2;
    const long long t = (long long)blockIdx.x * blockDim.x + threadIdx.x;
    if (t >= total) return;
    const int s = (int)(t & 1);
    long long u = t >> 1;
    const long long pix = u % HW; u /= HW;
    const int n = (int)(u % N);
    const int ch = (int)(u / N);
    half8 hv, lv;
    unsigned sat = 0;
#pragma unroll
    for (int e = 0; e < 8; ++e) {
        const int c = ch * 16 + s * 8 + e;
        const float v = (c < C) ? x[((long long)n * C + c) * HW + pix] * sc : 0.f;
        hv[e] = split_hi(v, sat);
        lv[e] = split_lo(v, hv[e]);
    }
    *reinterpret_cast<half8*>(y_hi + t * 8) = hv;
    if (y_lo) *reinterpret_cast<half8*>(y_lo + t * 8) = lv;
    if (sat != 0 && flags) atomicOr(flags, BINHIP_FLAG_SATURATED);
}

__global__ void planes_to_nchw_kernel(const _Float16* __restrict__ x_hi, const _Float16* __restrict__ x_lo,
                                      int N, int C, int H, int W, float* __restrict__ y) {
    const long long HW = (long long)H * W;
    const long long total = (long long)N * C * HW;
    const long long t = (long long)blockIdx.x * blockDim.x + threadIdx.x;
    if (t >= total) return;
    const long long pix = t % HW;
    const int c = (int)((t / HW) % C);
    const int n = (int)(t / (HW * C));
    const long long o = (((long long)(c >> 4) * N + n) * HW + pix) * 16 + (c & 15);
    float v = (float)x_hi[o];
    if (x_lo) v += (float)x_lo[o];
    y[t] = v;
}

__global__ void pixel_unshuffle_f32_kernel(const float* __restrict__ x, int N, int C, int H, int W, int r,
                                           float* __restrict__ y) {
    const int h = H / r, w = W / r;
    const long long total = (long long)N * C * H * W;
    const long long t = (long long)blockIdx.x * blockDim.x + threadIdx.x;
    if (t >= total) return;
    const int ox = (int)(t % w);
    const int oy = (int)((t / w) % h);
    const int oc = (int)((t / ((long long)w * h)) % (C * r * r));
    const int n = (int)(t / ((long long)w * h * C * r * r));
    const int c = oc / (r * r), i = (oc / r) % r, j = oc % r;
    y[t] = x[(((long long)n * C + c) * H + (oy * r + i)) * W + (ox * r + j)];
}

struct PackArgs {
    const float* img[5];
    int nimg, N, H, W;
};
__global__ void pack_inputs_kernel(PackArgs a, _Float16* __restrict__ y_hi, _Float16* __restrict__ y_lo,
                                   unsigned* __restrict__ flags) {
    const int h = a.H / 2, w = a.W / 2;
    const long long hw = (long long)h * w;
    const int C = 12 * a.nimg;
    const int nch = (C + 15) / 16;
    const long long total = (long long)nch * a.N * hw * 2;
    const long long t = (long long)blockIdx.x * blockDim.x + threadIdx.x;
    if (t >= total) return;
    const int s = (int)(t & 1);
    long long u = t >> 1;
    const long long pix = u % hw; u /= hw;
    const int n = (int)(u % a.N);
    const int ch = (int)(u / a.N);
    const int y = (int)(pix / w), x = (int)(pix % w);
    half8 hv, lv;
    unsigned sat = 0;
#pragma unroll
    for (int e = 0; e < 8; ++e) {
        const int c = ch * 16 + s * 8 + e;
        float v = 0.f;
        if (c < C) {
            const int cc = c >> 2, i = (c >> 1) & 1, j = c & 1;
            const int im = cc / 3, rgb = cc - im * 3;
            v = a.img[im][(((long long)n * 3 + rgb) * a.H + (2 * y + i)) * a.W + (2 * x + j)];
        }
        hv[e] = split_hi(v, sat);
        lv[e] = split_lo(v, hv[e]);
    }
    *reinterpret_cast<half8*>(y_hi + t * 8) = hv;
    if (y_lo) *reinterpret_cast<half8*>(y_lo + t * 8) = lv;
    if (sat != 0 && flags) atomicOr(flags, BINHIP_FLAG_SATURATED);
}

__global__ void u8_to_frame_kernel(const unsigned char* __restrict__ img, int H, int W, int pl, int pt, int Hp, int Wp,
                                   float* __restrict__ out) {
    const long long total = (long long)3 * Hp * Wp;
    const long long t = (long long)blockIdx.x * blockDim.x + threadIdx.x;
    if (t >= total) return;
    const int x = (int)(t % Wp), y = (int)((t / Wp) % Hp), c = (int)(t / ((long long)Wp * Hp));
    int sy = y - pt, sx = x - pl;
    sy = sy < 0 ? 0 : (sy >= H ? H - 1 : sy);
    sx = sx < 0 ? 0 : (sx >= W ? W - 1 : sx);
    out[t] = (float)img[((long long)sy * W + sx) * 3 + (2 - c)] / 255.f;
}
__global__ void frame_to_u8_kernel(const float* __restrict__ x, int Hp, int Wp, int top, int left, int H, int W,
                                   unsigned char* __restrict__ out) {
    const long long total = (long long)H * W * 3;
    const long long t = (long long)blockIdx.x * blockDim.x + threadIdx.x;
    if (t >= total) return;
    const int c = (int)(t % 3), xx = (int)((t / 3) % W), yy = (int)(t / (3LL * W));
    float v = x[((long long)(2 - c) * Hp + (yy + top)) * Wp + (xx + left)];
    v = fminf(fmaxf(v, 0.f), 1.f);
    out[t] = (unsigned char)rintf(v * 255.0f);
}

__device__ __forceinline__ float sigmoidf_(float v) { return 1.f / (1.f + __expf(-v)); }
__device__ __forceinline__ void lstm_point_fwd(float gi, float gj, float gf, float go, float cprev, float fb, float& c1, float& h1) {
    c1 = fmaf(cprev, sigmoidf_(gf + fb), __fmul_rn(sigmoidf_(gi), tanhf(gj)));
    h1 = __fmul_rn(tanhf(c1), sigmoidf_(go));
}
__device__ __forceinline__ void lstm_point_bwd(float gi, float gj, float gf, float go, float cprev, float fb, float ghv, float gcv,
                                               float& di, float& dj, float& df, float& dob, float& dcp) {
    const float si = sigmoidf_(gi), tj = tanhf(gj), sf = sigmoidf_(gf + fb), so = sigmoidf_(go);
    const float c1 = fmaf(cprev, sf, __fmul_rn(si, tj));
    const float tc = tanhf(c1);
    const float gct = fmaf(__fmul_rn(ghv, so), fmaf(-tc, tc, 1.f), gcv);
    di = __fmul_rn(__fmul_rn(gct, tj), __fmul_rn(si, 1.f - si));
    dj = __fmul_rn(__fmul_rn(gct, si), fmaf(-tj, tj, 1.f));
    df = __fmul_rn(__fmul_rn(gct, cprev), __fmul_rn(sf, 1.f - sf));
    dob = __fmul_rn(__fmul_rn(ghv, tc), __fmul_rn(so, 1.f - so));
    dcp = __fmul_rn(gct, sf);
}

__global__ void __launch_bounds__(256)
convlstm_kernel(const float* __restrict__ x, const float* __restrict__ cp, const float* __restrict__ hp,
                const float* __restrict__ w, const float* __restrict__ b, float fb, int N, int H, int W,
                float* __restrict__ cn, float* __restrict__ hn) {
// ... 712 lines not shown
#pragma unroll
        for (int c = 0; c < 3; ++c) {
            a.dwvar[(((((long long)n * 9 + var) * 12 + 4 * c + sub) * 25 + tap) * cin) + ci] = sv[c];
        }
    }
    if (tap == 0 && ci == 0) {
        const float bv[3] = {b0, b1, b2};
#pragma unroll
        for (int c = 0; c < 3; ++c) {
            a.dbvar[((long long)n * 9 + var) * 12 + 4 * c + sub] = bv[c];
        }
    }
}

int bh_upnet_gsub(const float* g, int N, int H, int W, const float* scale, void* y_hi, void* y_lo, void* status, hipStream_t s) {
    if (!g || !y_hi || N <= 0 || H <= 0 || W <= 0) return BINHIP_E_ARG;
    const long long total = (long long)N * H * W * 2;
    upnet_gsub_kernel<<<dim3((unsigned)((total + 255) / 256)), dim3(256), 0, s>>>(g, N, H, W, scale, (_Float16*)y_hi, (_Float16*)y_lo,
                                                                             (unsigned*)status);
    BH_CHECK_LAUNCH();
    return 0;
}
static int ring_bwd_args(RingBwdArgs& a, const float* g, const float* wvar, const float* scale, const void* x_hi, const void* x_lo,
                         void* gx_hi, void* gx_lo, float* dwvar, float* dbvar, void* status, int N, int H, int W, int cin, int accumulate) {
    if (!g || N <= 0 || H <= 0 || W <= 0 || cin <= 0 || (cin & 15) || cin > 256) return BINHIP_E_ARG;
    a.g = g; a.wvar = wvar; a.scale = scale; a.x_hi = (const _Float16*)x_hi; a.x_lo = (const _Float16*)x_lo;
    a.gx_hi = (_Float16*)gx_hi; a.gx_lo = (_Float16*)gx_lo; a.dwvar = dwvar; a.dbvar = dbvar; a.flags = (unsigned*)status;
    a.N = N; a.H = H; a.W = W; a.cin = cin; a.accumulate = accumulate;
    return 0;
}
int bh_upnet_ring_dgrad(const float* g, const float* wvar, const float* scale, void* gx_hi, void* gx_lo, void* status, int N, int H, int W,
                        int cin, hipStream_t s) {
    RingBwdArgs a;
    if (!wvar || !gx_hi) return BINHIP_E_ARG;
    if (int rc = ring_bwd_args(a, g, wvar, scale, nullptr, nullptr, gx_hi, gx_lo, nullptr, nullptr, status, N, H, W, cin, 0)) return rc;
    const int nrow = H < 6 ? H : 6, ncolx = W < 6 ? W : 6, mid = H > 6 ? H - 6 : 0;
    const long long total = ((long long)nrow * W + (long long)mid * ncolx) * N * (cin >> 3);
    upnet_ring_dgrad_kernel<<<dim3((unsigned)((total + 255) / 256)), dim3(256), 0, s>>>(a);
    BH_CHECK_LAUNCH();
    return 0;
}
int bh_upnet_ring_wgrad(const float* g, const void* x_hi, const void* x_lo, float* dwvar, float* dbvar, int N, int H, int W, int cin,
                        int accumulate, hipStream_t s) {
    RingBwdArgs a;
    if (!x_hi || !dwvar || !dbvar) return BINHIP_E_ARG;
    if (int rc = ring_bwd_args(a, g, nullptr, nullptr, x_hi, x_lo, nullptr, nullptr, dwvar, dbvar, nullptr, N, H, W, cin, accumulate)) return rc;
    const int ncg = (cin + 31) / 32;
    upnet_ring_wgrad_kernel<<<dim3((unsigned)(12 * 25 * N * ncg)), dim3(32, 8), 0, s>>>(a);
    BH_CHECK_LAUNCH();
    return 0;
}


extern "C" {


int binhip_version(void) { return BINHIP_VERSION; }

int binhip_device_cus(void) {
    int dev = 0;
    if (hipGetDevice(&dev) != hipSuccess) return -1;
    int n = 0;
    if (hipDeviceGetAttribute(&n, hipDeviceAttributeMultiprocessorCount, dev) != hipSuccess) return -1;
    return n;
}

int binhip_nchw_to_planes(const float* x, int N, int C, int H, int W, void* y_hi, void* y_lo, void* status, void* stream) {
    if (!x || !y_hi) return BINHIP_E_ARG;
    if (N <= 0 || C <= 0 || H <= 0 || W <= 0) return BINHIP_E_SHAPE;
    const long long total = (long long)bh_chunks(C) * N * H * W * 2;
    hipLaunchKernelGGL(nchw_to_planes_kernel, dim3((unsigned)((total + 255) / 256)), dim3(256), 0, (hipStream_t)stream,
                       x, N, C, H, W, (_Float16*)y_hi, (_Float16*)y_lo, (const float*)nullptr, (unsigned*)status);
    BH_CHECK_LAUNCH();
    return 0;
}

int binhip_nchw_to_planes_scaled(const float* x, int N, int C, int H, int W, const float* scale, void* y_hi,
                                 void* y_lo, void* status, void* stream) {
    if (!x || !y_hi || !scale) return BINHIP_E_ARG;
    if (N <= 0 || C <= 0 || H <= 0 || W <= 0) return BINHIP_E_SHAPE;
    const long long total = (long long)bh_chunks(C) * N * H * W * 2;
    hipLaunchKernelGGL(nchw_to_planes_kernel, dim3((unsigned)((total + 255) / 256)), dim3(256), 0, (hipStream_t)stream,
                       x, N, C, H, W, (_Float16*)y_hi, (_Float16*)y_lo, scale, (unsigned*)status);
    BH_CHECK_LAUNCH();
    return 0;
}

int binhip_planes_to_nchw(const void* x_hi, const void* x_lo, int N, int C, int H, int W, float* y, void* stream) {
    if (!x_hi || !y) return BINHIP_E_ARG;
    if (N <= 0 || C <= 0 || H <= 0 || W <= 0) return BINHIP_E_SHAPE;
    const long long total = (long long)N * C * H * W;
    hipLaunchKernelGGL(planes_to_nchw_kernel, dim3((unsigned)((total + 255) / 256)), dim3(256), 0, (hipStream_t)stream,
                       (const _Float16*)x_hi, (const _Float16*)x_lo, N, C, H, W, y);
    BH_CHECK_LAUNCH();
    return 0;
}

int binhip_pixel_unshuffle_f32(const float* x, int N, int C, int H, int W, int r, float* y, void* stream) {
    if (!x || !y) return BINHIP_E_ARG;
    if (N <= 0 || C <= 0 || H <= 0 || W <= 0 || r < 1 || H % r || W % r) return BINHIP_E_SHAPE;
    const long long total = (long long)N * C * H * W;
    hipLaunchKernelGGL(pixel_unshuffle_f32_kernel, dim3((unsigned)((total + 255) / 256)), dim3(256), 0, (hipStream_t)stream, x,
                       N, C, H, W, r, y);
    BH_CHECK_LAUNCH();
    return 0;
}

int binhip_pack_inputs(const float* const* images, int n_images, int N, int H, int W, void* y_hi, void* y_lo,
                       void* status, void* stream) {
    if (!images || !y_hi) return BINHIP_E_ARG;
    if (n_images < 1 || n_images > 5 || N <= 0 || H <= 0 || W <= 0 || (H & 1) || (W & 1)) return BINHIP_E_SHAPE;
    PackArgs a;
    for (int i = 0; i < 5; ++i) a.img[i] = (i < n_images) ? images[i] : nullptr;
    for (int i = 0; i < n_images; ++i) if (!images[i]) return BINHIP_E_ARG;
    a.nimg = n_images; a.N = N; a.H = H; a.W = W;
    const long long total = (long long)bh_chunks(12 * n_images) * N * (H / 2) * (W / 2) * 2;
    hipLaunchKernelGGL(pack_inputs_kernel, dim3((unsigned)((total + 255) / 256)), dim3(256), 0, (hipStream_t)stream,
                       a, (_Float16*)y_hi, (_Float16*)y_lo, (unsigned*)status);
    BH_CHECK_LAUNCH();
    return 0;
}

static inline bool convlstm_vec4_ok(int W, const void* a, const void* b, const void* c, const void* d, const void* e, const void* f,
                                    const void* g) {
    uintptr_t m = 0;
    for (const void* p : {a, b, c, d, e, f, g}) m |= (uintptr_t)p;
    return (W & 3) == 0 && (m & 15) == 0;
}

int binhip_convlstm_fwd(const float* x, const float* c_prev, const float* h_prev, const float* w, const float* b,
                        float forget_bias, int N, int H, int W, float* c_new, float* h_new, void* stream) {
    if (!x || !w || !b || !h_new) return BINHIP_E_ARG;
    if ((c_prev == nullptr) != (h_prev == nullptr)) return BINHIP_E_ARG;
    if (N <= 0 || H <= 0 || W <= 0) return BINHIP_E_SHAPE;
    const long long total = (long long)N * H * W;
    if (convlstm_vec4_ok(W, x, c_prev, h_prev, c_new, h_new, nullptr, nullptr))
        hipLaunchKernelGGL(convlstm4_kernel, dim3((unsigned)((total / 4 + 255) / 256)), dim3(256), 0, (hipStream_t)stream,
                           x, c_prev, h_prev, w, b, forget_bias, N, H, W, c_new, h_new);
    else
        hipLaunchKernelGGL(convlstm_kernel, dim3((unsigned)((total + 255) / 256)), dim3(256), 0, (hipStream_t)stream,
                           x, c_prev, h_prev, w, b, forget_bias, N, H, W, c_new, h_new);
    BH_CHECK_LAUNCH();
    return 0;
}

int binhip_lstm_gates_fwd(const float* gates, const float* c_prev, float forget_bias, int N, int hidden, int H, int W,
                          float* c_new, float* h_new, void* stream) {
    if (!gates || !c_new || !h_new) return BINHIP_E_ARG;
    if (N <= 0 || hidden <= 0 || H <= 0 || W <= 0) return BINHIP_E_SHAPE;
    const long long HW = (long long)H * W, total = (long long)N * hidden * HW;
    hipLaunchKernelGGL(lstm_gates_fwd_kernel, dim3((unsigned)((total + 255) / 256)), dim3(256), 0, (hipStream_t)stream, gates,
                       c_prev, forget_bias, hidden, HW, total, c_new, h_new);
    BH_CHECK_LAUNCH();
    return 0;
}

int binhip_lstm_gates_bwd(const float* gates, const float* c_prev, const float* g_h, const float* g_c, float forget_bias, int N,
                          int hidden, int H, int W, float* g_gates, float* g_cprev, void* stream) {
    if (!gates || !g_gates || (!g_h && !g_c)) return BINHIP_E_ARG;
    if (N <= 0 || hidden <= 0 || H <= 0 || W <= 0) return BINHIP_E_SHAPE;
    const long long HW = (long long)H * W, total = (long long)N * hidden * HW;
    hipLaunchKernelGGL(lstm_gates_bwd_kernel, dim3((unsigned)((total + 255) / 256)), dim3(256), 0, (hipStream_t)stream, gates,
                       c_prev, g_h, g_c, forget_bias, hidden, HW, total, g_gates, g_cprev);
    BH_CHECK_LAUNCH();
    return 0;
}

int binhip_charbonnier_partials(int64_t numel) { (void)numel; return CHARB_BLOCKS; }

int binhip_pixel_loss_fwd(int kind, const float* x, const float* y, int64_t numel, float eps, float* partials, float* loss,
                          void* stream) {
// ... 200 lines not shown
```

### bin_amd/csrc/binhip_plan.hip

```cpp
#include "binhip_conv_common.h"

namespace {

struct Shp {
    int G0, D, C, G;
    int c0, cg, cb;
    int L;
    bool stage4;
};
bool resolve_shape(const BinRdnShape* s, Shp* o) {
    Shp h;
    const bool dflt = !s || (s->G0 == 0 && s->D == 0 && s->C == 0 && s->G == 0);
    h.G0 = dflt ? 96 : s->G0; h.D = dflt ? 12 : s->D; h.C = dflt ? 4 : s->C; h.G = dflt ? 32 : s->G;
    if (h.G0 < 32 || h.G0 > 256 || h.G0 % 32 || h.G < 32 || h.G > 128 || h.G % 32) return false;
    if (h.C < 1 || h.C > BINHIP_RDN_MAX_CONVS || h.D < 1 || h.D > 20) return false;
    h.c0 = h.G0 / 16; h.cg = h.G / 16; h.cb = h.c0 + h.C * h.cg;
    h.L = 2 + h.D * (h.C + 1) + 4;
    if (h.L > BINHIP_RDN_MAX_LAYERS) return false;
    h.stage4 = (h.G0 == 96 && h.C == 4 && h.G == 32);
    *o = h;
    return true;
}
inline int layer_conv(const Shp& sh, int d, int c) { return 2 + d * (sh.C + 1) + c; }

struct Ws {
    int64_t P, PF;
    int kc0;
    int64_t x0, f1, blk, g0, g1, u, total;
    int64_t sync;
    int tiles;
    int64_t s_x0, s_f1, s_blk, s_g, s_u;
    int nt;
};

Ws make_ws(int N, int H, int W, int nin, int nt, const Shp& sh) {
    Ws w;
    const int h = H / 2, ww = W / 2;
    w.P = (int64_t)N * h * ww * 16;
    w.PF = (int64_t)N * H * W * 16;
    w.kc0 = (12 * nin + 15) / 16;
    w.nt = nt;
    const int mul = (nt == 3) ? 2 : 1;
    w.s_x0 = w.kc0 * w.P; w.s_f1 = sh.c0 * w.P; w.s_blk = (int64_t)(sh.D + 1) * sh.cb * w.P; w.s_g = sh.c0 * w.P;
    w.s_u = 4 * w.PF;
    int64_t o = 0;
    w.x0 = o; o += mul * w.s_x0;
    w.f1 = o; o += mul * w.s_f1;
    w.blk = o; o += mul * w.s_blk;
    w.g0 = o; o += mul * w.s_g;
    w.g1 = o; o += mul * w.s_g;
    w.u = o; o += mul * w.s_u;
    w.tiles = N * ((h + 15) / 16) * ((ww + 31) / 32);
    o = (o + 127) & ~(int64_t)127;
    w.sync = o; o += 2 * (32 + 2 * (int64_t)w.tiles);
    w.total = o;
    return w;
}

}

extern "C" {

size_t binhip_rdn_workspace_bytes(int N, int H, int W, int n_inputs, int nterms, const BinRdnShape* shape) {
    if (N <= 0 || H <= 0 || W <= 0 || (H & 1) || (W & 1)) return 0;
    if (n_inputs != 2 && n_inputs != 3 && n_inputs != 5) return 0;
    Shp sh;
    if (!resolve_shape(shape, &sh)) return 0;
    return (size_t)make_ws(N, H, W, n_inputs, nterms, sh).total * 2 + 256;
}

int binhip_rdn_workspace_layout(int N, int H, int W, int n_inputs, int nterms, const BinRdnShape* shape, int64_t* out,
                                int n_out) {
    if (!out || n_out < BINHIP_RDN_LAYOUT_WORDS) return BINHIP_E_ARG;
    Shp sh;
    if (!resolve_shape(shape, &sh) || binhip_rdn_workspace_bytes(N, H, W, n_inputs, nterms, shape) == 0) return BINHIP_E_SHAPE;
    const Ws w = make_ws(N, H, W, n_inputs, nterms, sh);
    const int64_t v[BINHIP_RDN_LAYOUT_WORDS] = {w.P, w.PF, w.kc0, w.x0, w.s_x0, w.f1, w.s_f1, w.blk, w.s_blk,
                                                 w.g0, w.s_g, w.g1, w.s_g, w.u, w.s_u, nterms == 3 ? 1 : 0};
    for (int i = 0; i < BINHIP_RDN_LAYOUT_WORDS; ++i) out[i] = v[i];
    return 0;
}

int binhip_rdn_forward(const BinRdnPlan* p, const float* const* inputs, float* out, void* workspace,
                       size_t workspace_bytes, void* stream) {
    if (!p || !inputs || !out || !workspace) return BINHIP_E_ARG;
    const int N = p->N, H = p->H, W = p->W, nin = p->n_inputs, nt = p->nterms;
    if (N <= 0 || H <= 0 || W <= 0 || (H & 1) || (W & 1)) return BINHIP_E_SHAPE;
    if (nin != 2 && nin != 3 && nin != 5) return BINHIP_E_SHAPE;
    if (nt != 1 && nt != 3) return BINHIP_E_ARG;
    Shp sh;
    if (!resolve_shape(&p->shape, &sh)) return BINHIP_E_SHAPE;
    const size_t need = binhip_rdn_workspace_bytes(N, H, W, nin, nt, &p->shape);
    if (workspace_bytes < need) return BINHIP_E_WORKSPACE;
    for (int i = 0; i < nin; ++i) if (!inputs[i]) return BINHIP_E_ARG;
    for (int i = 0; i < sh.L; ++i)
        if (!p->w_hi[i] || !p->bias[i] || (nt == 3 && !p->w_lo[i])) return BINHIP_E_ARG;

    hipStream_t s = (hipStream_t)stream;
    const Ws w = make_ws(N, H, W, nin, nt, sh);
    const int h = H / 2, ww = W / 2;
    _Float16* base = (_Float16*)(((uintptr_t)workspace + 255) & ~(uintptr_t)255);
    auto HI = [&](int64_t off) { return (void*)(base + off); };
    auto LO = [&](int64_t off, int64_t size) { return nt == 3 ? (void*)(base + off + size) : (void*)nullptr; };

    int rc = binhip_pack_inputs(inputs, nin, N, H, W, HI(w.x0), LO(w.x0, w.s_x0), p->status, stream);
    if (rc) return rc;

    auto mk = [&](int layer, int ks, int cin_chunks, int cout, int cout_pad, int epi, int relu, int Hc, int Wc,
                  int64_t x_off, int64_t x_size, int cpg, int64_t gstride,
                  int64_t y_off, int64_t y_size, int64_t r_off, int64_t r_size) -> BhConvCall {
        BhConvCall c;
        c.d.N = N; c.d.H = Hc; c.d.W = Wc; c.d.ksize = ks; c.d.cin_chunks = cin_chunks; c.d.cout = cout;
        c.d.cout_pad = cout_pad; c.d.nterms = nt; c.d.epilogue = epi; c.d.relu = relu;
        c.d.x_cpg = cpg; c.d.x_group_stride = gstride; c.d.n_images = 0; c.d.reserved = 0; c.d.status = p->status;
        if (ks == 1 && epi == BINHIP_EPI_PLANES && Wc > 32 && Wc % 32 == 0) { c.d.H = Hc * (Wc / 32); c.d.W = 32; }
        if (layer == 0 && ks == 5 && (12 * nin) % 16 >= 1 && (12 * nin) % 16 <= 8) c.d.reserved = BINHIP_CONV_HALF_LAST_CHUNK;
        c.x_hi = HI(x_off); c.x_lo = LO(x_off, x_size);
        c.w_hi = p->w_hi[layer]; c.w_lo = p->w_lo[layer]; c.bias = p->bias[layer];
        c.r_hi = (r_off >= 0) ? HI(r_off) : nullptr;
        c.r_lo = (r_off >= 0) ? LO(r_off, r_size) : nullptr;
        c.y_hi = (y_off >= 0) ? HI(y_off) : nullptr;
        c.y_lo = (y_off >= 0) ? LO(y_off, y_size) : nullptr;
        c.y_f32 = nullptr;
        c.status = p->status;
        c.prof = p->profiler;
        for (int i = 0; i < 5; ++i) c.images[i] = nullptr;
        if (epi == BINHIP_EPI_FINAL || epi == BINHIP_EPI_FINAL_SUBPIX) {
            c.y_f32 = out;
            c.d.n_images = nin;
            for (int i = 0; i < nin; ++i) c.images[i] = inputs[i];
        }
        return c;
    };
    auto conv = [&](int layer, int ks, int cin_chunks, int cout, int cout_pad, int epi, int relu, int Hc, int Wc,
                    int64_t x_off, int64_t x_size, int cpg, int64_t gstride,
                    int64_t y_off, int64_t y_size, int64_t r_off, int64_t r_size) -> int {
        return bh_launch_conv(mk(layer, ks, cin_chunks, cout, cout_pad, epi, relu, Hc, Wc, x_off, x_size, cpg, gstride,
                                 y_off, y_size, r_off, r_size), s);
    };
    const bool rdb3 = (p->reserved & BINHIP_PLAN_RDB3) && nt == 3 && sh.stage4;
    unsigned* sync_words = (unsigned*)(base + w.sync);
    const int cus = binhip_device_cus();
    if (rdb3) {
        hipError_t me = hipMemsetAsync(sync_words, 0, (size_t)(32 + 2 * (size_t)w.tiles) * 4, s);
        if (me != hipSuccess) return (int)me;
    }
    const int P_ = BINHIP_EPI_PLANES;
    const int64_t P = w.P;
    const int G0 = sh.G0, G = sh.G, C = sh.C, D = sh.D, c0 = sh.c0, cg = sh.cg, cb = sh.cb;
    if ((rc = conv(0, 5, w.kc0, G0, G0, P_, 0, h, ww, w.x0, w.s_x0, 0, 0, w.f1, w.s_f1, -1, 0))) return rc;
    if ((rc = conv(1, 3, c0, G0, G0, P_, 0, h, ww, w.f1, w.s_f1, 0, 0, w.blk, w.s_blk, -1, 0))) return rc;
    for (int d = 0; d < D; ++d) {
        const int64_t b = w.blk + (int64_t)d * cb * P;
        const bool fuse = sh.stage4 && !(p->reserved & BINHIP_PLAN_NO_FUSE);
        bool done3 = false;
        if (rdb3 && fuse) {
            ConvKArgs ka[3];
            bool ok3 = true;
            for (int c = 0; c < 3 && ok3; ++c) {
                BhConvCall cc = mk(layer_conv(sh, d, c), 3, c0 + cg * c, G, G, P_, 1, h, ww, b, w.s_blk, 0, 0,
                                   b + (int64_t)(c0 + cg * c) * P, w.s_blk, -1, 0);
                if ((rc = bh_prepare_conv(cc, &ka[c]))) return rc;
                ok3 = ok3 && ka[c].wt;
            }
            if (ok3) {
                rc = bh_launch_rdb3_x3(ka, sync_words + 32, (unsigned)(d + 1), cus, s);
                if (rc == 0) done3 = true;
                else if (rc != BINHIP_E_SHAPE) return rc;
            }
        }
        for (int c = 0; c < (fuse ? C - 1 : C) && !done3; ++c) {
            if ((rc = conv(layer_conv(sh, d, c), 3, c0 + cg * c, G, G, P_, 1, h, ww, b, w.s_blk, 0, 0,
                           b + (int64_t)(c0 + cg * c) * P, w.s_blk, -1, 0))) return rc;
        }
        if (fuse) {
            const int L3 = layer_conv(sh, d, 3), LF = layer_conv(sh, d, 4);
            if ((rc = binhip_rdb_tail_fwd(N, h, ww, nt, HI(b), LO(b, w.s_blk), p->w_hi[L3], p->w_lo[L3], p->bias[L3],
                                          p->w_hi[LF], p->w_lo[LF], p->bias[LF], HI(b + (int64_t)cb * P),
                                          LO(b + (int64_t)cb * P, w.s_blk), (p->reserved & BINHIP_PLAN_KEEP_ACTS) ? 1 : 0, p->status, stream)))
                return rc;
        } else if ((rc = conv(layer_conv(sh, d, C), 1, cb, G0, G0, P_, 0, h, ww, b, w.s_blk, 0, 0, b + (int64_t)cb * P, w.s_blk, b, w.s_blk)))
            return rc;
    }
    const int LG = sh.L - 4;
    if ((rc = conv(LG, 1, D * c0, G0, G0, P_, 0, h, ww, w.blk + (int64_t)cb * P, w.s_blk, c0, (int64_t)cb * P, w.g0, w.s_g, -1, 0))) return rc;
    if ((rc = conv(LG + 1, 3, c0, G0, G0, P_, 0, h, ww, w.g0, w.s_g, 0, 0, w.g1, w.s_g, w.f1, w.s_f1))) return rc;
    const bool fused_up = (p->reserved & BINHIP_PLAN_FUSED_UPNET) &&
                          (!(p->reserved & BINHIP_PLAN_KEEP_ACTS) || (p->reserved & BINHIP_PLAN_FUSED_UPNET_TRAIN)) &&
                          sh.L + 1 < BINHIP_RDN_MAX_LAYERS && p->w_hi[sh.L] && (nt == 1 || p->w_lo[sh.L]) && p->bias[sh.L] &&
                          p->w_hi[sh.L + 1] && p->bias[sh.L + 1];
    if (fused_up) {
        if ((rc = bh_launch_conv(mk(sh.L, 5, c0, 12, 32, BINHIP_EPI_FINAL_SUBPIX, 0, h, ww, w.g1, w.s_g, 0, 0, -1, 0, -1, 0), s))) return rc;
        return bh_launch_upnet_ring(HI(w.g1), LO(w.g1, w.s_g), (const float*)p->w_hi[sh.L + 1], p->bias[sh.L + 1], out, inputs, nin, N, h, ww,
                                    G0, s);
    }
    if ((rc = conv(LG + 2, 3, c0, 256, 256, BINHIP_EPI_SHUFFLE, 0, h, ww, w.g1, w.s_g, 0, 0, w.u, w.s_u, -1, 0))) return rc;
    if ((rc = conv(LG + 3, 3, 4, 3, 32, BINHIP_EPI_FINAL, 0, H, W, w.u, w.s_u, 0, 0, -1, 0, -1, 0))) return rc;
    return 0;
}

}

namespace {

struct Bws {
    int64_t P, PF;
    int kc0, gx0_chunks;
    int64_t gout, gu, guu, gg1, gg0, gf1, gy, gcat, gcat2, gx0, total_halfs;
    int64_t s_gout, s_gu, s_guu, s_g, s_gy, s_gcat, s_gx0;
    size_t wg_bytes, sc_off_bytes, wg_off_bytes, total_bytes;
};

Bws make_bws(int N, int H, int W, int nin, int nt, const Shp& sh) {
    Bws b;
    const int h = H / 2, w = W / 2;
    b.P = (int64_t)N * h * w * 16;
    b.PF = (int64_t)N * H * W * 16;
    b.kc0 = (12 * nin + 15) / 16;
    b.gx0_chunks = ((12 * nin + 31) / 32) * 2;
    const int mul = (nt == 3) ? 2 : 1;
    b.s_gout = b.PF; b.s_gu = 4 * b.PF; b.s_guu = 16 * b.P; b.s_g = sh.c0 * b.P; b.s_gy = (int64_t)(sh.D + 1) * sh.c0 * b.P;
    b.s_gcat = (int64_t)sh.cb * b.P; b.s_gx0 = (int64_t)b.gx0_chunks * b.P;
    int64_t o = 0;
    b.gout = o; o += mul * b.s_gout;
    b.gu = o; o += mul * b.s_gu;
    b.guu = o; o += mul * b.s_guu;
    b.gg1 = o; o += mul * b.s_g;
    b.gg0 = o; o += mul * b.s_g;
    b.gf1 = o; o += mul * b.s_g;
    b.gy = o; o += mul * b.s_gy;
    b.gcat = o; o += mul * b.s_gcat;
    b.gcat2 = o; o += mul * b.s_gcat;
    b.gx0 = o; o += mul * b.s_gx0;
    b.total_halfs = o;
    size_t wg = 0;
    auto mx = [&](size_t v) { if (v > wg) wg = v; };
    mx(binhip_wgrad_workspace_bytes(3, N, H, W, 4, 3));
    mx(binhip_wgrad_workspace_bytes(3, N, h, w, sh.c0, 256));
    mx(binhip_wgrad_workspace_bytes(3, N, h, w, sh.c0, sh.G0));
    mx(binhip_wgrad_workspace_bytes(1, N, h, w, sh.D * sh.c0, sh.G0));
    mx(binhip_wgrad_workspace_bytes(1, N, h, w, sh.cb, sh.G0));
    for (int c = 0; c < sh.C; ++c) mx(binhip_wgrad_workspace_bytes(3, N, h, w, sh.c0 + sh.cg * c, sh.G));
    mx(binhip_wgrad_workspace_bytes(5, N, h, w, b.kc0, sh.G0));
    b.wg_bytes = wg;
    size_t bytes = ((size_t)b.total_halfs * 2 + 255) & ~(size_t)255;
    b.sc_off_bytes = bytes; bytes += 8192;
    b.wg_off_bytes = bytes; bytes += (size_t)(sh.C + 1) * wg;
// ... 207 lines not shown
```

### bin_amd/models/archs/RDN.py

```python
import ctypes as C
import os

import torch
import torch.nn as nn
import torch.nn.init as weight_init

from ... import ops
from ...rdn_plan import RdnWeights, rdn_forward

PRECISIONS = {"f16": 1, "f16x3": 3}


def default_precision():
    p = os.environ.get("BIN_AMD_PRECISION", "f16x3")
    if p not in PRECISIONS:
        raise ValueError(f"BIN_AMD_PRECISION must be one of {sorted(PRECISIONS)}, got {p!r}")
    return p


class _nullctx:
    def __enter__(self):
        return self

    def __exit__(self, *a):
# ... 82 lines not shown
        self.shape = check_shape((G0, D, C, G))
        self.G0, self.D, self.C, self.G = G0, D, C, G
        kSize = 3
        self.SFENet1 = nn.Conv2d(12 * self.N_INPUTS, G0, 5, padding=2, stride=1)
        self.SFENet2 = nn.Conv2d(G0, G0, kSize, padding=1, stride=1)
        self.RDBs = nn.ModuleList([RDB(growRate0=G0, growRate=G, nConvLayers=C) for _ in range(D)])
        self.GFF = nn.Sequential(nn.Conv2d(D * G0, G0, 1, padding=0, stride=1),
                                 nn.Conv2d(G0, G0, kSize, padding=1, stride=1))
        self.UPNet = nn.Sequential(nn.Conv2d(G0, 256, kSize, padding=1, stride=1), nn.PixelShuffle(2),
                                   nn.Conv2d(64, 3, kSize, padding=1, stride=1))
        self.precision = None
        from ...autograd import default_backward_precision, default_wgrad_side_stream
        from ...rdn_plan import default_plan_flags
        self.backward_precision = default_backward_precision()
        self._direct_grads = False
        self.allow_f16_training = False
        self.wgrad_side_stream = default_wgrad_side_stream()
        self.plan_flags = default_plan_flags()
        self.profiler = None
        self.bwd_profiler = None
        self.debug_hook = None
        self._wcache = None
        self._wgen = 0

    def direct_param_grads(self, on=True):
        return _DirectParamGrads([self], on)

    def _weights_key(self, nterms):
        params = list(self.parameters())
        return (nterms, str(params[0].device), self._wgen, tuple((p.data_ptr(), p._version) for p in params))

    def invalidate_kernel_weights(self):
        self._wgen += 1

    def kernel_weights(self, nterms):
        key = self._weights_key(nterms)
        if self._wcache is None or self._wcache[0] != key:
            with torch.no_grad():
                self._wcache = (key, RdnWeights(dict(self.named_parameters()), self.N_INPUTS, nterms, shape=self.shape))
        return self._wcache[1]

    def _run(self, *frames):
        if len(frames) != self.N_INPUTS:
            raise TypeError(f"{type(self).__name__}.forward takes {self.N_INPUTS} frames")
        if not all(f.is_cuda for f in frames):
            raise RuntimeError("bin_amd: RDN sub-networks run on a HIP device only (no CPU fallback; see oracle/)")
        with torch.cuda.device(frames[0].device):
            if torch.is_grad_enabled() and (any(f.requires_grad for f in frames) or
                                             any(p.requires_grad for p in self.parameters())):
                from ...autograd import rdn_apply
                return rdn_apply(self, frames)
            nterms = PRECISIONS[self.precision or default_precision()]
            return rdn_forward(self.kernel_weights(nterms), list(frames), flags=self.plan_flags, profiler=self.profiler)


class RDN_residual_interp_2_input(_RDNBase):
    N_INPUTS = 2

    def forward(self, B0, B1):
        return self._run(B0, B1)


class RDN_residual_interp_2_1_input(_RDNBase):
    N_INPUTS = 3

    def forward(self, I0, I1, I2):
        return self._run(I0, I1, I2)


class RDN_residual_interp_4_1_input(_RDNBase):
    N_INPUTS = 5

    def forward(self, B0, B1, B2, B3, B4):
        return self._run(B0, B1, B2, B3, B4)


class RDN_residual_interp_5_input(nn.Module):

    def __init__(self, lstm=False, GO=64, D=6):
        super().__init__()
        if not lstm:
            raise NotImplementedError("reference RDN.py:358 references an undefined class when lstm=False")
        self.lstm = lstm
        self.model1_1 = RDN_residual_interp_2_input(G0=GO, D=D)
        self.model1_2 = self.model1_1
        self.model1_3 = self.model1_1
        self.model1_4 = self.model1_1
        self.model2_1 = RDN_residual_interp_2_1_input(G0=GO, D=D)
        self.model2_2 = self.model2_1
        self.model2_3 = self.model2_1
        self.model3_1 = RDN_residual_interp_4_1_input(G0=GO, D=D)
        self.model3_2 = self.model3_1
        self.model4_1 = RDN_residual_interp_4_1_input(G0=GO, D=D)

    def forward(self, B1, B3, B5, B7, B9, previous_input=None, stage1=None):
        s1 = stage1 or (None, None, None, None)
        I2 = s1[0] if s1[0] is not None else self.model1_1(B1, B3)
        I4 = s1[1] if s1[1] is not None else self.model1_2(B3, B5)
        I6 = s1[2] if s1[2] is not None else self.model1_3(B5, B7)
        I8 = s1[3] if s1[3] is not None else self.model1_4(B7, B9)
        if previous_input is not None and previous_input[0] is not None:
            p4, p6, p8, p5, p7, p6b = previous_input
            I3 = self.model2_1(p4, I2, I4)
            I5 = self.model2_2(p6, I4, I6)
            I7 = self.model2_3(p8, I6, I8)
            I4pp = self.model3_1(p5, B3, I3, I5, B5)
# ... 212 lines not shown

    def cell(si, c, x):
        return launch(si, lambda: c(x, None)[0], [x])

    B1, B3, B5, B7, B9, B11 = B

    touched = set()

    def memo(si, k, *ins):
        if stage1_cache is None:
            return rdn(si, k, *ins)
        key = (k, wkeys[k]) + tuple(id(t) for t in ins)
        touched.add(key)
        hit = stage1_cache.get(key)
        if hit is not None and all(a is b for a, b in zip(hit[1], ins)):
            if hit[2] is not None:
                ready[id(hit[0])] = hit[2]
            return hit[0]
        out = rdn(si, k, *ins)
        stage1_cache[key] = (out, ins, ready.get(id(out)))
        return out

    I2 = memo(0, 1, B1, B3); I4 = memo(1, 1, B3, B5); I6 = memo(2, 1, B5, B7); I8 = memo(3, 1, B7, B9)
    I3 = memo(0, 2, I2, I2, I4); I5 = memo(1, 2, I4, I4, I6); I7 = memo(2, 2, I6, I6, I8)
    h4 = cell(3, cells[0], I4); h6 = cell(3, cells[1], I6); h8 = cell(3, cells[2], I8)
    I4pp = memo(0, 3, I3, B3, I3, I5, B5); I6pp = memo(1, 3, I5, B5, I5, I7, B7)
    h5 = cell(2, cells[3], I5); h7 = cell(2, cells[4], I7)
    I8b = memo(2, 1, B9, B11)
    I5ppp = memo(0, 4, I4, I4, I4pp, I6pp, I6)
    h6pp = cell(1, cells[5], I6pp)
    J3 = rdn(0, 2, h4, I4, I6); J5 = rdn(1, 2, h6, I6, I8); J7 = rdn(2, 2, h8, I8, I8b)
    J4pp = rdn(0, 3, h5, B5, J3, J5, B7); J6pp = rdn(1, 3, h7, B7, J5, J7, B9)
    J5ppp = rdn(0, 4, h6pp, I6, J4pp, J6pp, I8)
    if stage1_cache is not None:
        for key in [key for key in stage1_cache if key not in touched]:
            del stage1_cache[key]
    for s in streams:
        if s is not main:
            main.wait_stream(s)
    outs = (I2, I4, I6, I8, I3, I5, I7, I4pp, I6pp, I5ppp, I8b, J7, J6pp, J5ppp)
    if ns > 1 and mode is None and not torch.cuda.is_current_stream_capturing():
        for t in outs + (h4, h6, h8, h5, h7, h6pp, J3, J5, J4pp):
            for s in streams:
                t.record_stream(s)
            t.record_stream(main)
    self.Ft_p_1 = (I6, I8, I8b, None, J3, J5, J7, J4pp, J6pp, J5ppp)
    return outs


RDN_residual_interp_5_input_ConvLSTM_L._forward_streams = _forward_streams


def _forward_four_calls(self, B):
    m = self.model
    n = B[0].shape[0]
    B1, B3, B5, B7, B9, B11 = B
    cat = torch.cat
    cells = (self.clstm_4_prime, self.clstm_6_prime, self.clstm_8_prime, self.clstm_5_prime_prime,
             self.clstm_7_prime_prime, self.clstm_6_prime_prime_prime)

    def parts(t, k):
        out = torch.split(t, n, 0)
        assert len(out) == k
        return list(out)

    I2, I4, I6, I8, I8b = parts(m.model1_1(cat((B1, B3, B5, B7, B9), 0), cat((B3, B5, B7, B9, B11), 0)), 5)
    h4, h6, h8 = (cells[k](x, None)[0] for k, x in enumerate((I4, I6, I8)))
    I3, I5, I7, J3, J5, J7 = parts(m.model2_1(cat((I2, I4, I6, h4, h6, h8), 0), cat((I2, I4, I6, I4, I6, I8), 0),
                                              cat((I4, I6, I8, I6, I8, I8b), 0)), 6)
    h5, h7 = cells[3](I5, None)[0], cells[4](I7, None)[0]
    I4pp, I6pp, J4pp, J6pp = parts(m.model3_1(cat((I3, I5, h5, h7), 0), cat((B3, B5, B5, B7), 0), cat((I3, I5, J3, J5), 0),
                                              cat((I5, I7, J5, J7), 0), cat((B5, B7, B7, B9), 0)), 4)
    h6pp = cells[5](I6pp, None)[0]
    I5ppp, J5ppp = parts(m.model4_1(cat((I4, h6pp), 0), cat((I4, I6), 0), cat((I4pp, J4pp), 0), cat((I6pp, J6pp), 0),
                                    cat((I6, I8), 0)), 2)
    self.Ft_p_1 = (I6, I8, I8b, None, J3, J5, J7, J4pp, J6pp, J5ppp)
    return (I2, I4, I6, I8, I3, I5, I7, I4pp, I6pp, I5ppp, I8b, J7, J6pp, J5ppp)


RDN_residual_interp_5_input_ConvLSTM_L._forward_four_calls = _forward_four_calls


def bin_stage4_lstm():
    return RDN_residual_interp_5_input_ConvLSTM_L()
```

### bin_amd/ops.py

```python
import ctypes as C
import os

import torch

from . import _lib as L


def _stream(device=None):
    return C.c_void_p(torch.cuda.current_stream(device).cuda_stream)


def on_device(t):
    return torch.cuda.device(t.device)


_status = {}


def status_word(device):
    key = _device_key(device)
    w = _status.get(key)
    if w is None:
        w = torch.zeros(1, dtype=torch.int32, device=torch.device("cuda", key))
        _status[key] = w
# ... 686 lines not shown
    assert raw.size == GRAD_RECORD_WORDS
    return L.BinGradRecord.from_buffer_copy(raw.tobytes())


def grad_norm(rows, workspace, record, max_norm=0.0, status=None, status_mask=0):
    _need_cuda(workspace, record, status)
    if workspace.numel() * workspace.element_size() < rows.workspace_bytes or not workspace.is_contiguous():
        raise ValueError(f"grad_norm: workspace of {workspace.numel() * workspace.element_size()} bytes, need {rows.workspace_bytes}")
    if workspace.data_ptr() % 8:
        raise ValueError("grad_norm: the workspace holds doubles: 8-byte aligned")
    if record.dtype != torch.int32 or record.numel() != GRAD_RECORD_WORDS or not record.is_contiguous() or record.data_ptr() % 8:
        raise ValueError("grad_norm: the record is 8 contiguous int32 words, 8-byte aligned (grad_record)")
    if any(t is not None and t.device != rows.device for t in (workspace, record, status)):
        raise ValueError("grad_norm: workspace, record and status word live on the rows' device")
    with torch.cuda.device(rows.device):
        L.check(L.gradlib().bingrad_norm(rows.table, rows.n, float(max_norm), _ptr(status), int(status_mask) & 0xFFFFFFFF, _ptr(workspace),
                                         _ptr(record), _stream()), "grad_norm")


def grad_scale(rows, record):
    _need_cuda(record)
    if record.dtype != torch.int32 or record.numel() != GRAD_RECORD_WORDS or record.device != rows.device:
        raise ValueError("grad_scale: the record grad_norm wrote (grad_record), on the rows' device")
    if rows.n == 0:
        return
    with torch.cuda.device(rows.device):
        L.check(L.gradlib().bingrad_scale(rows.table, rows.n, _ptr(record), _stream()), "grad_scale")


def ema_rows(n):
    return (L.BinEmaTensor * max(n, 1))()


def ema_row(table, i, e, p):
    _need_cuda(e, p)
    for name, t in (("e", e), ("p", p)):
        if t.dtype != torch.float32:
            raise ValueError(f"ema_step: float32 tensors, got {t.dtype} for {name}")
        if not t.is_contiguous():
            raise ValueError(f"ema_step: contiguous tensors, got strides {tuple(t.stride())} of shape {tuple(t.shape)} for {name}")
        if t.numel() != p.numel() or t.device != p.device:
            raise ValueError(f"ema_step: {name} has {t.numel()} elements on {t.device}, p has {p.numel()} on {p.device}")
    if p.numel() < 1:
        raise ValueError("ema_step: empty tensor")
    r = table[i]
    r.e, r.p, r.numel = e.data_ptr(), p.data_ptr(), p.numel()


def ema_launch(table, n, device, decay):
    if n == 0:
        return
    with torch.cuda.device(device):
        L.check(L.emalib().binema_step(table, n, decay, _stream()), "ema_step")
```

### bin_amd/rdn_plan.py

```python
import ctypes as C

import torch

from . import _lib as L
from .ops import ConvWeights, _ptr, _stream, _need_cuda, on_device, relayout_batch, relayout_item, status_word

STAGE4_SHAPE = (96, 12, 4, 32)


def check_shape(shape):
    G0, D, C, G = (int(v) for v in shape)
    if G0 % 32 or not 32 <= G0 <= 256 or G % 32 or not 32 <= G <= 128 or not 1 <= C <= L.RDN_MAX_CONVS or not 1 <= D <= 20 \
            or 2 + D * (C + 1) + 4 > L.RDN_MAX_LAYERS:
        raise NotImplementedError(
            f"bin_amd RDN: unsupported configuration G0={G0}, D={D}, C={C}, G={G} (built: G0 and G multiples of 32 with "
            f"32 <= G0 <= 256, G <= 128; 1 <= C <= {L.RDN_MAX_CONVS}; 1 <= D <= 20)")
    return G0, D, C, G


def c_shape(shape):
    s = L.BinRdnShape()
    s.G0, s.D, s.C, s.G = shape
    return s

# ... 161 lines not shown
        self.fused_train = None
        self.fused_train_w4 = None
        self.fused_graph = None

    def ensure_fused_upnet(self, train=False):
        if self._up_src is None:
            return None
        if train:
            if self.fused_train is None:
                with torch.enable_grad():
                    leaves = [t.detach().float().requires_grad_() for t in self._up_src]
                    Wr, Br = fused_upnet_operator(*leaves)
                self.fused_graph = (leaves, Wr, Br)
                with torch.no_grad():
                    g0 = Wr.shape[3]
                    self.fused_train_w4 = Wr[4].permute(0, 2, 1).reshape(12, g0, 5, 5).contiguous()
                    main = ConvWeights(self.fused_train_w4, Br[4].detach().contiguous(), nterms=self.nterms)
                    self.fused_train = (main, Wr.detach().contiguous(), Br.detach().contiguous())
            return self.fused_train
        if self.fused_up is None:
            with torch.no_grad():
                W, B = fused_upnet_weights(*self._up_src)
                self.fused_w4 = W[4].float().contiguous()
                main = ConvWeights(self.fused_w4, B[4].float().contiguous(), nterms=self.nterms)
                ring_w = W.permute(0, 1, 3, 4, 2).reshape(9, 12, 25, W.shape[2]).float().contiguous()
                self.fused_up = (main, ring_w, B.float().contiguous())
        return self.fused_up

    def fill_plan(self, plan, fused=None):
        plan.shape = c_shape(self.shape)
        for i, cw in enumerate(self.layers):
            plan.w_hi[i] = cw.w_hi.data_ptr()
            plan.w_lo[i] = cw.w_lo.data_ptr() if cw.w_lo is not None else None
            plan.bias[i] = cw.bias.data_ptr()
        n = len(self.layers)
        if fused is not None:
            main, ring_w, ring_b = fused
            plan.w_hi[n], plan.bias[n] = main.w_hi.data_ptr(), main.bias.data_ptr()
            plan.w_lo[n] = main.w_lo.data_ptr() if main.w_lo is not None else None
            plan.w_hi[n + 1], plan.w_lo[n + 1], plan.bias[n + 1] = ring_w.data_ptr(), None, ring_b.data_ptr()

    def dgrad(self, module, nterms=None, fused=False):
        nterms = self.nterms if nterms is None else nterms
        if self._dgrad is None:
            self._dgrad = {}
        key = (nterms, bool(fused))
        if key not in self._dgrad:
            if fused and self.fused_train is None:
                raise RuntimeError("bin_amd: backward of a fused-UPNet forward on weights that never built the training operands")
            with torch.no_grad():
                self._dgrad[key] = RdnDgradWeights(dict(module.named_parameters()), self.n_inputs, nterms, shape=self.shape,
                                                   fused=(self.fused_train_w4, self.fused_train[1]) if fused else None)
        return self._dgrad[key]


class RdnDgradWeights:

    def __init__(self, params, n_inputs, nterms, prefix="", shape=STAGE4_SHAPE, fused=None):
        lib = L.lib()
        self.shape = G0, D, C, G = check_shape(shape)
        self.w_hi, self.w_lo = [], []
        self.fused_ring_w = None
        dev = None
        names = layer_names(self.shape)
        fp32 = {nm: params[f"{prefix}{nm}.weight"].detach().contiguous().float() for nm in names}

        def alloc(rows, chunks, ks):
            nbytes = lib.binhip_weights_bytes(rows, chunks, ks)
            hi = torch.empty(nbytes // 2, dtype=torch.float16, device=dev)
            lo = torch.empty(nbytes // 2, dtype=torch.float16, device=dev) if nterms == 3 else None
            return hi, lo, torch.empty(rows, dtype=torch.float32, device=dev)

        items, scratch = [], []
        self._src = fp32
        for nm in names:
            w = fp32[nm]
            dev = w.device
            cout, cin, ks, _ = w.shape
            if ".convs." in nm:
                d, g = int(nm.split(".")[1]), int(nm.split(".")[3])
                rows, chunks = (G0 if g == 0 else G), (C - g) * G // 16
                hi, lo, zb = alloc(rows, chunks, 3)
                srcs = [fp32[f"RDBs.{d}.convs.{c}.conv.0"] for c in range(C)]
                cb = lib.binhip_conv_cout_block(3, rows, nterms)
                items.append(relayout_item(L.RELAYOUT_RDB_GATHER, srcs, None, hi, lo, zb, G, G0 + G * g, 3, rows, chunks, cb, g,
                                           shape=self.shape))
            else:
                rows_pad = lib.binhip_dgrad_rows_pad(ks, cin)
                cin_chunks = (cout + 15) // 16
                cb = lib.binhip_conv_cout_block(ks, rows_pad, nterms)
                hi, lo, zb = alloc(rows_pad, cin_chunks, ks)
                items.append(relayout_item(L.RELAYOUT_DGRAD, [w], None, hi, lo, zb, cout, cin, ks, rows_pad, cin_chunks, cb,
                                           1 if nm == "UPNet.0" else 0))
            self.w_hi.append(hi)
            self.w_lo.append(lo)
            scratch.append(zb)
        if fused is not None:
            w4, self.fused_ring_w = fused
            rows_pad = lib.binhip_dgrad_rows_pad(5, G0)
            cb = lib.binhip_conv_cout_block(5, rows_pad, nterms)
            hi, lo, zb = alloc(rows_pad, 1, 5)
            items.append(relayout_item(L.RELAYOUT_DGRAD, [w4], None, hi, lo, zb, 12, G0, 5, rows_pad, 1, cb, 0))
            self.w_hi.append(hi)
            self.w_lo.append(lo)
            scratch.append(zb)
        relayout_batch(items)
        del scratch
        self.zero_bias = torch.zeros(max(D * G0, G0 + C * G, 256, 1152), dtype=torch.float32, device=dev)

    def fill_plan(self, plan):
        plan.shape = c_shape(self.shape)
        for i in range(len(self.w_hi)):
            plan.wt_hi[i] = self.w_hi[i].data_ptr()
            plan.wt_lo[i] = self.w_lo[i].data_ptr() if self.w_lo[i] is not None else None
        if self.fused_ring_w is not None:
            plan.wt_hi[len(self.w_hi)] = self.fused_ring_w.data_ptr()
        plan.zero_bias = self.zero_bias.data_ptr()


from collections import OrderedDict as _OrderedDict

_workspaces = _OrderedDict()
WORKSPACE_CACHE_ENTRIES = 12


def workspace(nbytes, device, key="fwd"):
    stream = torch.cuda.current_stream(device)
    if torch.cuda.is_current_stream_capturing():
        return torch.empty(nbytes, dtype=torch.uint8, device=device)
    key = (device.type, device.index, stream.cuda_stream, key)
    ws = _workspaces.get(key)
    if ws is None or ws.numel() < nbytes:
        ws = torch.empty(nbytes, dtype=torch.uint8, device=device)
        _workspaces[key] = ws
        while len(_workspaces) > WORKSPACE_CACHE_ENTRIES:
            _workspaces.popitem(last=False)
    _workspaces.move_to_end(key)
    return ws


def release_workspaces(stream=None):
    if stream is None:
        _workspaces.clear()
        return
    for k in [k for k in _workspaces if k[2] == stream.cuda_stream and k[1] == stream.device.index]:
        del _workspaces[k]


import os as _os


def default_plan_flags():
    flags = L.PLAN_RDB3 if _os.environ.get("BIN_AMD_RDB3", "0") == "1" else 0
    if _os.environ.get("BIN_AMD_FUSED_UPNET", "1") != "0":
        flags |= L.PLAN_FUSED_UPNET
    return flags


def rdn_forward(weights, inputs, out=None, ws=None, flags=0, profiler=None):
    _need_cuda(*inputs)
    with on_device(inputs[0]):
        return _rdn_forward(weights, inputs, out, ws, flags, profiler)


def _rdn_forward(weights, inputs, out, ws, flags, profiler):
    inputs = [t.contiguous().float() for t in inputs]
    n, c, h, w = inputs[0].shape
    assert c == 3 and len(inputs) == weights.n_inputs
    lib = L.lib()
    plan = L.BinRdnPlan()
    plan.N, plan.H, plan.W, plan.n_inputs, plan.nterms = n, h, w, weights.n_inputs, weights.nterms
    plan.reserved = int(flags or 0)
    plan.status = status_word(inputs[0].device).data_ptr()
    plan.profiler = profiler if profiler else None
    fused = None
    if plan.reserved & L.PLAN_FUSED_UPNET:
        if plan.reserved & L.PLAN_FUSED_UPNET_TRAIN:
            fused = weights.ensure_fused_upnet(train=True)
        elif not (plan.reserved & L.PLAN_KEEP_ACTS):
            fused = weights.ensure_fused_upnet()
    weights.fill_plan(plan, fused)
    nbytes = lib.binhip_rdn_workspace_bytes(n, h, w, weights.n_inputs, weights.nterms, C.byref(plan.shape))
    if nbytes == 0:
        raise RuntimeError(f"bin_amd: unsupported RDN shape N={n} H={h} W={w} (H, W must be even)")
    if ws is None:
        ws = workspace(nbytes, inputs[0].device)
    if out is None:
        out = torch.empty((n, 3, h, w), dtype=torch.float32, device=inputs[0].device)
    arr = (C.c_void_p * len(inputs))(*[t.data_ptr() for t in inputs])
    L.check(lib.binhip_rdn_forward(C.byref(plan), arr, _ptr(out), _ptr(ws), ws.numel(), _stream()), "rdn_forward")
    return out
```

### include/binhip.h

```cpp
#ifndef BINHIP_H
#define BINHIP_H

#include <stddef.h>
#include <stdint.h>

#ifdef __cplusplus
extern "C" {
#endif

#define BINHIP_API __attribute__((visibility("default")))

#define BINHIP_VERSION 622
#define BINHIP_ABI_EXPORTS 51

#define BINHIP_E_ARG      (-1)
#define BINHIP_E_SHAPE    (-2)
#define BINHIP_E_WORKSPACE (-3)

#define BINHIP_STATUS_SATURATED 1u
#define BINHIP_STATUS_SYNC_TIMEOUT 2u

#define BINHIP_EPI_PLANES  0
#define BINHIP_EPI_SHUFFLE 1
#define BINHIP_EPI_FINAL   2
// ... 80 lines not shown
                       int pad_top, int pad_bottom, float* out_chw, void* stream);
BINHIP_API int binhip_frame_to_u8(const float* chw, int Hp, int Wp, int top, int left, int H, int W,
                       unsigned char* bgr_hwc, void* stream);

BINHIP_API int binhip_convlstm_fwd(const float* x, const float* c_prev, const float* h_prev,
                        const float* w , const float* b , float forget_bias,
                        int N, int H, int W, float* c_new, float* h_new, void* stream);

BINHIP_API int binhip_lstm_gates_fwd(const float* gates, const float* c_prev, float forget_bias, int N, int hidden, int H, int W,
                          float* c_new, float* h_new, void* stream);
BINHIP_API int binhip_lstm_gates_bwd(const float* gates, const float* c_prev, const float* g_h, const float* g_c,
                          float forget_bias, int N, int hidden, int H, int W, float* g_gates, float* g_cprev, void* stream);

BINHIP_API int binhip_charbonnier_partials(int64_t numel);
BINHIP_API int binhip_charbonnier_fwd(const float* x, const float* y, int64_t numel, float eps,
                           float* partials, float* loss, void* stream);
BINHIP_API int binhip_charbonnier_bwd(const float* x, const float* y, int64_t numel, float eps,
                           const float* gloss, float* gx, float* gy, void* stream);
#define BINHIP_LOSS_CHARBONNIER 0
#define BINHIP_LOSS_L1_SUM      1
#define BINHIP_LOSS_L2_SUM      2
BINHIP_API int binhip_pixel_loss_fwd(int kind, const float* x, const float* y, int64_t numel, float eps,
                          float* partials, float* loss, void* stream);
BINHIP_API int binhip_pixel_loss_bwd(int kind, const float* x, const float* y, int64_t numel, float eps,
                          const float* gloss, float* gx, float* gy, void* stream);

#define BINHIP_LOSS_MAX_TERMS 24
typedef struct {
    const float* x[BINHIP_LOSS_MAX_TERMS];
    const float* y[BINHIP_LOSS_MAX_TERMS];
    int32_t n_terms;
} BinLossTerms;
BINHIP_API int binhip_multi_loss_fwd(int kind, const BinLossTerms* t, int64_t numel, float eps, float* partials, float* terms,
                          float* loss, void* stream);
typedef struct {
    float* out[BINHIP_LOSS_MAX_TERMS];
    int32_t term_a[BINHIP_LOSS_MAX_TERMS], term_b[BINHIP_LOSS_MAX_TERMS];
    float sign_a[BINHIP_LOSS_MAX_TERMS], sign_b[BINHIP_LOSS_MAX_TERMS];
    int32_t n_out;
} BinLossGrads;
BINHIP_API int binhip_multi_loss_bwd(int kind, const BinLossTerms* t, int64_t numel, float eps, const float* gloss,
                          const BinLossGrads* g, void* stream);

BINHIP_API int binhip_rdb_tail_fwd(int N, int H, int W, int nterms, const void* blk_hi, const void* blk_lo,
                        const void* wc_hi, const void* wc_lo, const float* bias_c,
                        const void* wl_hi, const void* wl_lo, const float* bias_l,
                        void* y_hi, void* y_lo, int store_o3, void* status, void* stream);

#define BINHIP_PLAN_KEEP_ACTS 1
#define BINHIP_PLAN_NO_FUSE   2
#define BINHIP_PLAN_RDB3      4
#define BINHIP_PLAN_FUSED_UPNET 8
#define BINHIP_PLAN_FUSED_UPNET_TRAIN 16
typedef struct BinRdnPlan {
    int32_t N, H, W;
    int32_t n_inputs;
    int32_t nterms;
    int32_t reserved;
    BinRdnShape shape;
    const void* w_hi[BINHIP_RDN_MAX_LAYERS];
    const void* w_lo[BINHIP_RDN_MAX_LAYERS];
    const float* bias[BINHIP_RDN_MAX_LAYERS];
    void* status;
    struct BinhipProfiler* profiler;
} BinRdnPlan;

BINHIP_API size_t binhip_rdn_workspace_bytes(int N, int H, int W, int n_inputs, int nterms, const BinRdnShape* shape );
#define BINHIP_RDN_LAYOUT_WORDS 16
BINHIP_API int binhip_rdn_workspace_layout(int N, int H, int W, int n_inputs, int nterms, const BinRdnShape* shape,
                                int64_t* out, int n_out);
BINHIP_API int binhip_rdn_forward(const BinRdnPlan* plan, const float* const* inputs , float* out ,
                       void* workspace, size_t workspace_bytes, void* stream);

BINHIP_API size_t binhip_wgrad_workspace_bytes(int ksize, int N, int H, int W, int cin_chunks, int cout);
BINHIP_API int binhip_conv2d_bwd_weight(const BinConvDesc* d, const void* x_hi, const void* x_lo,
                             const void* gy_hi, const void* gy_lo, const float* inv_scale,
                             void* workspace, size_t workspace_bytes, float* dw_oihw, float* dbias,
                             int cin, int shuffle_perm, int accumulate, void* stream);

BINHIP_API int binhip_grad_scale(const float* g, int64_t numel, float target, float* partials, float* scale_out,
                      void* stream);
BINHIP_API int binhip_nchw_to_planes_scaled(const float* x, int N, int C, int H, int W, const float* scale,
                                 void* y_hi, void* y_lo, void* status, void* stream);
BINHIP_API int binhip_unshuffle_planes(const void* x_hi, const void* x_lo, int N, int H, int W, int nchunks,
                            void* y_hi, void* y_lo, void* stream);
BINHIP_API int binhip_unpack_input_grads(const void* gx0_hi, const void* gx0_lo, const float* gout,
                              const float* scale, int n_images, int N, int H, int W,
                              float* const* outs, void* stream);

BINHIP_API size_t binhip_convlstm_bwd_workspace_bytes(int N, int H, int W);
BINHIP_API int binhip_convlstm_bwd(const float* x, const float* c_prev, const float* h_prev, const float* w,
                        const float* b, float forget_bias, int N, int H, int W, const float* g_h,
                        const float* g_c, void* workspace, size_t workspace_bytes, float* gx,
                        float* g_hprev, float* g_cprev, float* dw, float* db, void* stream);

#define BINHIP_BWD_ACCUMULATE 1
#define BINHIP_BWD_FUSED_UPNET 4
#define BINHIP_BWD_SAVED_X3   2
typedef struct BinRdnBwdPlan {
    int32_t N, H, W, n_inputs, nterms, reserved;
    BinRdnShape shape;
    const void* wt_hi[BINHIP_RDN_MAX_LAYERS];
    const void* wt_lo[BINHIP_RDN_MAX_LAYERS];
    const float* zero_bias;
    float* dw[BINHIP_RDN_MAX_LAYERS];
    float* db[BINHIP_RDN_MAX_LAYERS];
// ... 44 lines not shown
```

Baseline: 16.31 interpolated frames/s.

## Gather RDN input frames via pointer tables instead of torch.cat copies

```diff
diff --git a/__graft_entry__.py b/__graft_entry__.py
--- a/__graft_entry__.py
+++ b/__graft_entry__.py
@@ -18,6 +18,7 @@
     _lib.optlib()
     _lib.gradlib()
     _lib.emalib()
+    _lib.zerolib()
     from oracle import rdn_oracle
     print(f"built {path} (binhip version {lib.binhip_version()})")
 
diff --git a/bin_amd/_lib.py b/bin_amd/_lib.py
--- a/bin_amd/_lib.py
+++ b/bin_amd/_lib.py
@@ -1,11 +1,14 @@
 import ctypes as C
 import os
 
-from .build import EMA_LIB_PATH, GRAD_LIB_PATH, LIB_PATH, OPT_LIB_PATH
+from .build import EMA_LIB_PATH, GRAD_LIB_PATH, LIB_PATH, OPT_LIB_PATH, ZERO_LIB_PATH
 
 RDN_LAYERS = 66
 RDN_MAX_LAYERS, RDN_MAX_CONVS = 192, 7
 PLAN_KEEP_ACTS, PLAN_NO_FUSE, PLAN_RDB3, PLAN_FUSED_UPNET, PLAN_FUSED_UPNET_TRAIN = 1, 2, 4, 8, 16
+PLAN_GATHER_INPUTS = 32
+GATHER_MAX = 6
+E_ARG, E_SHAPE, E_WORKSPACE = -1, -2, -3
 BWD_ACCUMULATE = 1
 BWD_SAVED_X3 = 2
 BWD_FUSED_UPNET = 4
@@ -94,6 +97,13 @@
 
 class BinEmaTensor(C.Structure):
     _fields_ = [("e", C.c_void_p), ("p", C.c_void_p), ("numel", C.c_int64)]
+
+
+ZERO_MAX_REGIONS = 128
+
+
+class BinZeroRegion(C.Structure):
+    _fields_ = [("ptr", C.c_void_p), ("bytes", C.c_int64)]
 
 
 _SIGNATURES = {
@@ -204,6 +214,12 @@
     "binema_step": (C.c_int, [C.POINTER(BinEmaTensor), C.c_int, C.c_float, C.c_void_p]),
 }
 
+ZERO_VERSION = 100
+_ZERO_SIGNATURES = {
+    "binzero_version": (C.c_int, []),
+    "binzero_regions": (C.c_int, [C.POINTER(BinZeroRegion), C.c_int, C.c_void_p]),
+}
+
 STATUS_SATURATED = 1
 STATUS_SYNC_TIMEOUT = 2
 
@@ -309,6 +325,32 @@
     return _emalib
 
 
+_zerolib = None
+
+
+def zero_exported_symbols():
+    return sorted(_ZERO_SIGNATURES)
+
+
+def zerolib():
+    global _zerolib
+    if _zerolib is None:
+        path = ZERO_LIB_PATH
+        if not os.path.exists(path):
+            raise RuntimeError(
+                f"bin_amd: HIP library {ZERO_LIB_PATH} not built. Run `python -c 'import __graft_entry__ as g; "
+                f"g.build()'` (hipcc --offload-arch=gfx950). There is no CPU fallback by design.")
+        h = C.CDLL(path)
+        for name, (res, args) in _ZERO_SIGNATURES.items():
+            fn = getattr(h, name)
+            fn.restype = res
+            fn.argtypes = args
+        if h.binzero_version() != ZERO_VERSION:
+            raise RuntimeError(f"bin_amd: {path} is version {h.binzero_version()}, this binding is for {ZERO_VERSION}")
+        _zerolib = h
+    return _zerolib
+
+
 def check(rc, what):
     if rc != 0:
         kind = {-1: "bad argument", -2: "unsupported shape", -3: "workspace too small"}.get(rc, f"hipError {rc}")
diff --git a/bin_amd/autograd.py b/bin_amd/autograd.py
--- a/bin_amd/autograd.py
+++ b/bin_amd/autograd.py
@@ -4,8 +4,8 @@
 import torch
 
 from . import _lib as L
-from .ops import _ptr, _stream, on_device, status_word
-from .rdn_plan import c_shape, layer_names, rdn_forward, workspace
+from .ops import _ptr, _stream, on_device, status_word, zero_regions
+from .rdn_plan import c_shape, gather_lists, layer_names, rdn_forward, workspace
 
 
 
@@ -55,15 +55,20 @@
 
 class _RdnFn(torch.autograd.Function):
     @staticmethod
-    def forward(ctx, module, nterms, n_frames, *args):
-        frames = [a.contiguous().float() for a in args[:n_frames]]
+    def forward(ctx, module, nterms, n_frames, k, *args):
+        nt_in = n_frames * max(k, 1)
+        frames = [a.contiguous().float() for a in args[:nt_in]]
         weights = module.kernel_weights(nterms)
         n, _, h, w = frames[0].shape
+        if k:
+            frames = [frames[i * k:(i + 1) * k] for i in range(n_frames)][::-1]
+            gather_lists(frames, n_frames)
+            n *= k
         lib = L.lib()
         nbytes = lib.binhip_rdn_workspace_bytes(n, h, w, n_frames, nterms, C.byref(c_shape(weights.shape)))
         if nbytes == 0:
             raise RuntimeError(f"bin_amd: unsupported RDN shape N={n} H={h} W={w}")
-        saved = torch.empty(nbytes, dtype=torch.uint8, device=frames[0].device)
+        saved = torch.empty(nbytes, dtype=torch.uint8, device=args[0].device)
         fused = (bool(module.plan_flags & L.PLAN_FUSED_UPNET) and train_fused_upnet() and
                  weights.ensure_fused_upnet(train=True) is not None)
         flags = module.plan_flags | L.PLAN_KEEP_ACTS | (L.PLAN_FUSED_UPNET_TRAIN if fused else 0)
@@ -71,13 +76,13 @@
         ctx.fused_up = fused
         if module.debug_hook is not None:
             module.debug_hook("forward", module, (n, h, w, n_frames, nterms), saved, {"shape": module.shape, "fused_upnet": fused})
-        ctx.module, ctx.nterms, ctx.n_frames = module, nterms, n_frames
+        ctx.module, ctx.nterms, ctx.n_frames, ctx.k = module, nterms, n_frames, k
         ctx.saved_ws = saved
         ctx.weights = weights
         ctx.dims = (n, h, w)
-        ctx.param_meta = [(tuple(a.shape), a.device) for a in args[n_frames:]]
-        ctx.params = args[n_frames:]
-        ctx.param_versions = [(a._version, a.data_ptr()) for a in args[n_frames:]]
+        ctx.param_meta = [(tuple(a.shape), a.device) for a in args[nt_in:]]
+        ctx.params = args[nt_in:]
+        ctx.param_versions = [(a._version, a.data_ptr()) for a in args[nt_in:]]
         ctx.weights_gen = module._wgen
         module._bwd_pending = getattr(module, "_bwd_pending", 0) + 1
         ctx.owes_backward = True
@@ -105,6 +110,8 @@
     @staticmethod
     def _backward(ctx, gout):
         module, nterms, k = ctx.module, ctx.nterms, ctx.n_frames
+        kg = max(ctx.k, 1)
+        first_p = 4 + k * kg
         n, h, w = ctx.dims
         if ctx.weights_gen != module._wgen or any((a._version, a.data_ptr()) != v for a, v in zip(ctx.params, ctx.param_versions)):
             raise RuntimeError("bin_amd: a parameter of this RDN was modified in place between its forward and its backward "
@@ -127,7 +134,7 @@
                            if module.wgrad_side_stream and not torch.cuda.is_current_stream_capturing() else None)
         plan.profiler = module.bwd_profiler if module.bwd_profiler else None
         params = ctx.params
-        direct = module._direct_grads and all(ctx.needs_input_grad[3 + k:])
+        direct = module._direct_grads and all(ctx.needs_input_grad[first_p:])
         have = False
         if direct:
             states = [p.grad is not None for p in params]
@@ -148,19 +155,24 @@
             plan.reserved |= L.BWD_FUSED_UPNET
             up_dw4 = torch.empty((12, g0, 5, 5), dtype=torch.float32, device=dev)
             up_db4 = torch.empty((12,), dtype=torch.float32, device=dev)
-            up_dwr = torch.zeros((n, 9, 12, 25, g0), dtype=torch.float32, device=dev)
-            up_dbr = torch.zeros((n, 9, 12), dtype=torch.float32, device=dev)
+            up_dwr = torch.empty((n, 9, 12, 25, g0), dtype=torch.float32, device=dev)
+            up_dbr = torch.empty((n, 9, 12), dtype=torch.float32, device=dev)
+            with on_device(gout):
+                zero_regions((up_dwr, up_dbr))
             plan.dw[nl], plan.db[nl], plan.dw[nl + 1], plan.db[nl + 1] = (up_dw4.data_ptr(), up_db4.data_ptr(), up_dwr.data_ptr(),
                                                                         up_dbr.data_ptr())
         gins = []
         for i in range(k):
-            if ctx.needs_input_grad[3 + i]:
+            a0 = 4 + ((k - 1 - i) if ctx.k else i) * kg
+            need = ctx.needs_input_grad[a0:a0 + kg]
+            if any(need):
                 g = torch.empty((n, 3, h, w), dtype=torch.float32, device=dev)
                 plan.gin[i] = g.data_ptr()
-                gins.append(g)
+                gins.append([g] if not ctx.k else [g[j * (n // kg):(j + 1) * (n // kg)] if need[j] else None for j in range(kg)])
             else:
                 plan.gin[i] = None
-                gins.append(None)
+                gins.append([None] * kg)
+        gins = [g for row in (gins[::-1] if ctx.k else gins) for g in row]
         nbytes = lib.binhip_rdn_backward_workspace_bytes(n, h, w, k, nt_bwd, C.byref(plan.shape))
         ws = workspace(nbytes, dev, key="bwd")
         with on_device(gout):
@@ -181,7 +193,7 @@
                 if plan.reserved & L.BWD_ACCUMULATE:
                     grads[slot].add_(g.float())
                 else:
-                    grads[slot].copy_(g.float())
+                    grads[slot] = g.float().contiguous()
         _RdnFn._settle(ctx)
         if module._bwd_pending == 0 and direct:
             cb = getattr(module, "_grads_ready_cb", None)
@@ -191,9 +203,9 @@
             if not have:
                 for p, g in zip(params, grads):
                     p.grad = g
-            return (None, None, None, *gins, *([None] * len(grads)))
-        pgrads = [g if ctx.needs_input_grad[3 + k + i] else None for i, g in enumerate(grads)]
-        return (None, None, None, *gins, *pgrads)
+            return (None, None, None, None, *gins, *([None] * len(grads)))
+        pgrads = [g if ctx.needs_input_grad[first_p + i] else None for i, g in enumerate(grads)]
+        return (None, None, None, None, *gins, *pgrads)
 
 
 def rdn_apply(module, frames):
@@ -202,7 +214,17 @@
     flat = []
     for nm in layer_names(module.shape):
         flat += [params[nm + ".weight"], params[nm + ".bias"]]
-    return _RdnFn.apply(module, nterms, len(frames), *frames, *flat)
+    return _RdnFn.apply(module, nterms, len(frames), 0, *frames, *flat)
+
+
+def rdn_apply_gathered(module, lists):
+    nterms = train_precision(module)
+    k, _ = gather_lists(lists, len(lists))
+    params = dict(module.named_parameters())
+    flat = []
+    for nm in layer_names(module.shape):
+        flat += [params[nm + ".weight"], params[nm + ".bias"]]
+    return _RdnFn.apply(module, nterms, len(lists), k, *[t for row in reversed(lists) for t in row], *flat)
 
 
 class _ConvLstmFn(torch.autograd.Function):
@@ -215,6 +237,7 @@
                               None if h_prev is None else h_prev.contiguous().float(),
                               weight.detach().contiguous().float(), bias.detach().contiguous().float())
         ctx.fb = float(forget_bias)
+        ctx.set_materialize_grads(False)
         return h, c
 
     @staticmethod
@@ -231,8 +254,8 @@
         gcp = torch.empty_like(x) if (cp is not None and ctx.needs_input_grad[1]) else None
         ghp = torch.empty_like(x) if (hp is not None and ctx.needs_input_grad[2]) else None
         need_w = ctx.needs_input_grad[3] or ctx.needs_input_grad[4]
-        dw = torch.zeros_like(w) if need_w else None
-        db = torch.zeros_like(b) if need_w else None
+        dw = torch.empty_like(w) if need_w else None
+        db = torch.empty_like(b) if need_w else None
         ws = workspace(lib.binhip_convlstm_bwd_workspace_bytes(n, hh, ww), dev, key="clstm")
         L.check(lib.binhip_convlstm_bwd(_ptr(x), _ptr(cp), _ptr(hp), _ptr(w), _ptr(b), ctx.fb, n, hh, ww, _ptr(gh),
                                         _ptr(gc), _ptr(ws), ws.numel(), _ptr(gx), _ptr(ghp), _ptr(gcp), _ptr(dw),
diff --git a/bin_amd/build.py b/bin_amd/build.py
--- a/bin_amd/build.py
+++ b/bin_amd/build.py
@@ -16,6 +16,9 @@
 EMA_SOURCES = ["binema_step.hip"]
 EMA_LIB_PATH = os.path.join(CSRC, "libbinema.so")
 EMA_HEADER = os.path.join(os.path.dirname(HERE), "include", "binema.h")
+ZERO_SOURCES = ["binzero_regions.hip"]
+ZERO_LIB_PATH = os.path.join(CSRC, "libbinzero.so")
+ZERO_HEADER = os.path.join(os.path.dirname(HERE), "include", "binzero.h")
 
 
 HEADER = os.path.join(os.path.dirname(HERE), "include", "binhip.h")
@@ -45,13 +48,19 @@
         return re.findall(r"(?m)^BINEMA_API\s+[\w\s\*]+?\b(binema_\w+)\s*\(", f.read())
 
 
+def zero_abi_symbols():
+    import re
+    with open(ZERO_HEADER) as f:
+        return re.findall(r"(?m)^BINZERO_API\s+[\w\s\*]+?\b(binzero_\w+)\s*\(", f.read())
+
+
 def _stale():
-    libs = (LIB_PATH, OPT_LIB_PATH, GRAD_LIB_PATH, EMA_LIB_PATH)
+    libs = (LIB_PATH, OPT_LIB_PATH, GRAD_LIB_PATH, EMA_LIB_PATH, ZERO_LIB_PATH)
     if not all(os.path.exists(p) for p in libs):
         return True
     t = min(os.path.getmtime(p) for p in libs)
     deps = [os.path.join(CSRC, f) for f in os.listdir(CSRC) if f.endswith((".hip", ".h"))]
-    deps += [os.path.join(os.path.dirname(HERE), "include", "binhip.h"), OPT_HEADER, GRAD_HEADER, EMA_HEADER]
+    deps += [os.path.join(os.path.dirname(HERE), "include", "binhip.h"), OPT_HEADER, GRAD_HEADER, EMA_HEADER, ZERO_HEADER]
     return any(os.path.getmtime(d) > t for d in deps)
 
 
@@ -63,15 +72,16 @@
     objdir = CSRC if out is None else os.path.dirname(os.path.abspath(out))
     os.makedirs(objdir, exist_ok=True)
     tag = "" if out is None else "." + os.path.splitext(os.path.basename(out))[0]
-    procs, objs, opt_objs, grad_objs, ema_objs = [], [], [], [], []
-    for src in SOURCES + (OPT_SOURCES + GRAD_SOURCES + EMA_SOURCES if out is None else []):
+    procs, objs, opt_objs, grad_objs, ema_objs, zero_objs = [], [], [], [], [], []
+    for src in SOURCES + (OPT_SOURCES + GRAD_SOURCES + EMA_SOURCES + ZERO_SOURCES if out is None else []):
         obj = os.path.join(objdir, src.replace(".hip", tag + ".o"))
         cmd = [hipcc, "--offload-arch=gfx950", "-O3", "-std=c++17", "-fPIC", "-fvisibility=hidden"] + [f"-D{d}" for d in defines] + \
               ["-c", os.path.join(CSRC, src), "-o", obj]
         if verbose:
             print(" ".join(cmd), file=sys.stderr)
         procs.append((cmd, subprocess.Popen(cmd)))
-        (opt_objs if src in OPT_SOURCES else grad_objs if src in GRAD_SOURCES else ema_objs if src in EMA_SOURCES else objs).append(obj)
+        (opt_objs if src in OPT_SOURCES else grad_objs if src in GRAD_SOURCES else ema_objs if src in EMA_SOURCES else
+         zero_objs if src in ZERO_SOURCES else objs).append(obj)
     for cmd, p in procs:
         if p.wait() != 0:
             raise subprocess.CalledProcessError(p.returncode, cmd)
@@ -86,7 +96,8 @@
     subprocess.check_call(cmd)
     for name, symbols, path, lib_objs in ((("binopt", opt_abi_symbols(), OPT_LIB_PATH, opt_objs),
                                            ("bingrad", grad_abi_symbols(), GRAD_LIB_PATH, grad_objs),
-                                           ("binema", ema_abi_symbols(), EMA_LIB_PATH, ema_objs)) if out is None else ()):
+                                           ("binema", ema_abi_symbols(), EMA_LIB_PATH, ema_objs),
+                                           ("binzero", zero_abi_symbols(), ZERO_LIB_PATH, zero_objs)) if out is None else ()):
         vmap = os.path.join(objdir, f"binhip_exports.{name}.map")
         with open(vmap, "w") as f:
             f.write("{\n  global:\n" + "".join(f"    {n};\n" for n in symbols) + "  local: *;\n};\n")
diff --git a/bin_amd/csrc/binhip_conv.hip b/bin_amd/csrc/binhip_conv.hip
--- a/bin_amd/csrc/binhip_conv.hip
+++ b/bin_amd/csrc/binhip_conv.hip
@@ -297,6 +297,8 @@
     if (c.r2_hi && d.nterms == 3 && !c.r2_lo) return BINHIP_E_ARG;
     a.out_f32 = c.y_f32;
     for (int i = 0; i < 5; ++i) a.img[i] = c.images[i];
+    a.gtab = c.gather_tab; a.img_per = c.gather_tab ? c.gather_per : 0;
+    if (c.gather_tab && (c.gather_per <= 0 || d.N % c.gather_per || d.N / c.gather_per > BINHIP_GATHER_MAX)) return BINHIP_E_SHAPE;
     a.group_stride = d.x_group_stride;
     a.N = d.N; a.H = d.H; a.W = d.W;
     a.nchunks = d.cin_chunks;
diff --git a/bin_amd/csrc/binhip_conv_common.h b/bin_amd/csrc/binhip_conv_common.h
--- a/bin_amd/csrc/binhip_conv_common.h
+++ b/bin_amd/csrc/binhip_conv_common.h
@@ -12,7 +12,8 @@
 typedef unsigned u32x4 __attribute__((ext_vector_type(4)));
 
 int bh_launch_upnet_ring(const void* x_hi, const void* x_lo, const float* wvar, const float* bvar, float* out, const float* const* images,
-                         int nimg, int N, int H, int W, int cin, hipStream_t s);
+                         int nimg, int N, int H, int W, int cin, hipStream_t s,
+                         const float* const* gather_tab = nullptr, int gather_per = 0);
 int bh_upnet_gsub(const float* g, int N, int H, int W, const float* scale, void* y_hi, void* y_lo, void* status, hipStream_t s);
 int bh_upnet_ring_dgrad(const float* g, const float* wvar, const float* scale, void* gx_hi, void* gx_lo, void* status, int N, int H, int W,
                         int cin, hipStream_t s);
@@ -58,7 +59,21 @@
     unsigned tl_base;
 #endif
     int y_unshuf;
+    const float* const* gtab;
+    int img_per;
 };
+
+template <class A>
+__device__ __forceinline__ void bh_frame_bases(const A& a, int img, long long per_img, const float* (&fb)[5]) {
+#pragma unroll
+    for (int t = 0; t < 5; ++t) fb[t] = a.img[t];
+    if (a.img_per > 0) {
+        const int slot = img / a.img_per;
+        const long long back = (long long)slot * a.img_per * per_img;
+#pragma unroll
+        for (int t = 0; t < 5; ++t) fb[t] = (t < a.nimg) ? a.gtab[t * BINHIP_GATHER_MAX + slot] - back : nullptr;
+    }
+}
 
 #if BINHIP_TIMELINE
 #include <atomic>
@@ -158,6 +173,8 @@
         bias4(co0, bv[0]);
         bias4(co0 + 8, bv[1]);
         const bool col_ok = first_col && (gx < W);
+        const float* fb[5];
+        bh_frame_bases(a, img, (long long)ncolour * H2 * W2, fb);
         float sum[R][2][4];
 #pragma unroll
         for (int r = 0; r < R; ++r) {
@@ -171,8 +188,8 @@
                     float sj = 0.f;
                     if (ok && a.nimg > 0) {
                         const long long idx = (((long long)img * ncolour + c) * H2 + 2 * gy + (q >> 1)) * W2 + 2 * gx + (q & 1);
-                        sj = a.img[0][idx];
-                        for (int t = 1; t < a.nimg; ++t) sj += a.img[t][idx];
+                        sj = fb[0][idx];
+                        for (int t = 1; t < a.nimg; ++t) sj += fb[t][idx];
                         sj = sj / (float)a.nimg;
                     }
                     sum[r][g][q] = sj;
@@ -197,6 +214,8 @@
         float bv[4];
         bias4(co0, bv);
         const bool mine = (kg == 0) && first_col && (gx < W);
+        const float* fb[5];
+        bh_frame_bases(a, img, (long long)a.cout * H * W, fb);
         float sum[R][4];
 #pragma unroll
         for (int r = 0; r < R; ++r) {
@@ -206,8 +225,8 @@
                 float sj = 0.f;
                 if (mine && gy < H && j < a.cout && a.nimg > 0) {
                     const long long idx = (((long long)img * a.cout + j) * H + gy) * W + gx;
-                    sj = a.img[0][idx];
-                    for (int t = 1; t < a.nimg; ++t) sj += a.img[t][idx];
+                    sj = fb[0][idx];
+                    for (int t = 1; t < a.nimg; ++t) sj += fb[t][idx];
                     sj = sj / (float)a.nimg;
                 }
                 sum[r][j] = sj;
diff --git a/bin_amd/csrc/binhip_conv_x3.hip b/bin_amd/csrc/binhip_conv_x3.hip
--- a/bin_amd/csrc/binhip_conv_x3.hip
+++ b/bin_amd/csrc/binhip_conv_x3.hip
@@ -490,12 +490,14 @@
     if (gy < H && gx < W) {
         float sum[3], bj[3];
         const int nimg = a.nimg;
+        const float* fb[5];
+        bh_frame_bases(a, img, (long long)a.cout * H * W, fb);
 #pragma unroll
         for (int j = 0; j < 3; ++j) {
             const long long idx = (((long long)img * a.cout + (j < a.cout ? j : 0)) * H + gy) * W + gx;
             float v[5];
 #pragma unroll
-            for (int t = 0; t < 5; ++t) v[t] = (t < nimg) ? a.img[t][idx] : 0.f;
+            for (int t = 0; t < 5; ++t) v[t] = (t < nimg) ? fb[t][idx] : 0.f;
             bj[j] = a.bias[j < a.cout ? j : 0];
             float sj = v[0];
 #pragma unroll
@@ -631,6 +633,8 @@
     if (kb == 0) {
         float sum[2][2][3];
         const int nimg = a.nimg;
+        const float* fb[5];
+        bh_frame_bases(a, img, (long long)a.cout * H * W, fb);
 #pragma unroll
         for (int r = 0; r < 2; ++r)
 #pragma unroll
@@ -643,7 +647,7 @@
                     const long long idx = (((long long)img * a.cout + (j < a.cout ? j : 0)) * H + gyc) * W + gxc;
                     float v[5];
 #pragma unroll
-                    for (int t = 0; t < 5; ++t) v[t] = (t < nimg) ? a.img[t][idx] : 0.f;
+                    for (int t = 0; t < 5; ++t) v[t] = (t < nimg) ? fb[t][idx] : 0.f;
                     float sj = v[0];
 #pragma unroll
                     for (int t = 1; t < 5; ++t)
@@ -722,6 +726,8 @@
     float* out;
     const float* img[5];
     int N, H, W, cin, nimg;
+    const float* const* gtab;
+    int img_per;
 };
 constexpr int RING_THREADS = 128;
 __global__ void __launch_bounds__(RING_THREADS) upnet_ring_kernel(const RingArgs a) {
@@ -781,19 +787,23 @@
         const long long idx = (((long long)img * 3 + c) * H2 + Y) * W2 + X;
         float m = 0.f;
         if (a.nimg > 0) {
-            m = a.img[0][idx];
-            for (int t = 1; t < a.nimg; ++t) m += a.img[t][idx];
+            const float* fb[5];
+            bh_frame_bases(a, img, (long long)3 * H2 * W2, fb);
+            m = fb[0][idx];
+            for (int t = 1; t < a.nimg; ++t) m += fb[t][idx];
             m = m / (float)a.nimg;
         }
         a.out[idx] = (v + a.bvar[var * 12 + 4 * c + sub]) + m;
     }
 }
 int bh_launch_upnet_ring(const void* x_hi, const void* x_lo, const float* wvar, const float* bvar, float* out, const float* const* images,
-                         int nimg, int N, int H, int W, int cin, hipStream_t s) {
+                         int nimg, int N, int H, int W, int cin, hipStream_t s, const float* const* gather_tab, int gather_per) {
     if (!x_hi || !wvar || !bvar || !out || N <= 0 || H <= 0 || W <= 0 || cin <= 0 || (cin & 15) || nimg < 0 || nimg > 5) return BINHIP_E_ARG;
+    if (gather_tab ? (gather_per <= 0 || N % gather_per || N / gather_per > BINHIP_GATHER_MAX) : (nimg > 0 && !images)) return BINHIP_E_ARG;
     RingArgs a;
     a.x_hi = (const _Float16*)x_hi; a.x_lo = (const _Float16*)x_lo; a.wvar = wvar; a.bvar = bvar; a.out = out;
-    for (int t = 0; t < 5; ++t) a.img[t] = (t < nimg) ? images[t] : nullptr;
+    for (int t = 0; t < 5; ++t) a.img[t] = (t < nimg && !gather_tab) ? images[t] : nullptr;
+    a.gtab = gather_tab; a.img_per = gather_tab ? gather_per : 0;
     a.N = N; a.H = H; a.W = W; a.cin = cin; a.nimg = nimg;
     const long long ring = 4ll * W + 4ll * H - 4;
     upnet_ring_kernel<<<dim3((unsigned)(ring * N)), dim3(RING_THREADS), 0, s>>>(a);
diff --git a/bin_amd/csrc/binhip_internal.h b/bin_amd/csrc/binhip_internal.h
--- a/bin_amd/csrc/binhip_internal.h
+++ b/bin_amd/csrc/binhip_internal.h
@@ -54,10 +54,14 @@
     void *y_hi, *y_lo;
     float* y_f32;
     const float* images[5];
+    const float* const* gather_tab = nullptr;
+    int gather_per = 0;
     void* status = nullptr;
     BinhipProfiler* prof = nullptr;
 };
 int bh_launch_conv(const BhConvCall& c, hipStream_t s);
+int bh_pack_inputs_gather(const float* const* table, int n_images, int k, int N, int H, int W, void* y_hi, void* y_lo,
+                          const float** table_dev, void* status, hipStream_t s);
 bool bh_prof_begin(BinhipProfiler* pr, int ks, int cout_pad, int epi, hipStream_t s);
 void bh_prof_end(BinhipProfiler* pr, hipStream_t s);
 struct ConvKArgs;
diff --git a/bin_amd/csrc/binhip_misc.hip b/bin_amd/csrc/binhip_misc.hip
--- a/bin_amd/csrc/binhip_misc.hip
+++ b/bin_amd/csrc/binhip_misc.hip
@@ -59,11 +59,27 @@
 }
 
 struct PackArgs {
+    static constexpr bool GATHER = false;
     const float* img[5];
     int nimg, N, H, W;
 };
-__global__ void pack_inputs_kernel(PackArgs a, _Float16* __restrict__ y_hi, _Float16* __restrict__ y_lo,
+struct PackGatherArgs {
+    static constexpr bool GATHER = true;
+    const float* tab[5 * BINHIP_GATHER_MAX];
+    int nimg, per, N, H, W;
+};
+template <class Args>
+__global__ void pack_inputs_kernel(Args a, _Float16* __restrict__ y_hi, _Float16* __restrict__ y_lo, const float** __restrict__ tab_dev,
                                    unsigned* __restrict__ flags) {
+    __shared__ const float* tab[Args::GATHER ? 5 * BINHIP_GATHER_MAX : 1];
+    if constexpr (Args::GATHER) {
+        if (threadIdx.x < 5 * BINHIP_GATHER_MAX) {
+            const float* p = a.tab[threadIdx.x];
+            tab[threadIdx.x] = p;
+            if (blockIdx.x == 0 && tab_dev) tab_dev[threadIdx.x] = p;
+        }
+        __syncthreads();
+    }
     const int h = a.H / 2, w = a.W / 2;
     const long long hw = (long long)h * w;
     const int C = 12 * a.nimg;
@@ -77,6 +93,8 @@
     const int n = (int)(u % a.N);
     const int ch = (int)(u / a.N);
     const int y = (int)(pix / w), x = (int)(pix % w);
+    int slot = 0, nl = n;
+    if constexpr (Args::GATHER) { slot = n / a.per; nl = n - slot * a.per; }
     half8 hv, lv;
     unsigned sat = 0;
 #pragma unroll
@@ -86,7 +104,9 @@
         if (c < C) {
             const int cc = c >> 2, i = (c >> 1) & 1, j = c & 1;
             const int im = cc / 3, rgb = cc - im * 3;
-            v = a.img[im][(((long long)n * 3 + rgb) * a.H + (2 * y + i)) * a.W + (2 * x + j)];
+            const float* frames;
+            if constexpr (Args::GATHER) frames = tab[im * BINHIP_GATHER_MAX + slot]; else frames = a.img[im];
+            v = frames[(((long long)nl * 3 + rgb) * a.H + (2 * y + i)) * a.W + (2 * x + j)];
         }
         hv[e] = split_hi(v, sat);
         lv[e] = split_lo(v, hv[e]);
@@ -905,6 +925,26 @@
 }
 
 
+int bh_pack_inputs_gather(const float* const* table, int n_images, int k, int N, int H, int W, void* y_hi, void* y_lo,
+                          const float** table_dev, void* status, hipStream_t s) {
+    if (!table || !y_hi) return BINHIP_E_ARG;
+    if (n_images < 1 || n_images > 5 || N <= 0 || H <= 0 || W <= 0 || (H & 1) || (W & 1)) return BINHIP_E_SHAPE;
+    if (k < 1 || k > BINHIP_GATHER_MAX || N % k) return BINHIP_E_SHAPE;
+    PackGatherArgs a;
+    for (int i = 0; i < 5; ++i)
+        for (int j = 0; j < BINHIP_GATHER_MAX; ++j) {
+            const float* p = (i < n_images && j < k) ? table[i * BINHIP_GATHER_MAX + j] : nullptr;
+            if (i < n_images && j < k && !p) return BINHIP_E_ARG;
+            a.tab[i * BINHIP_GATHER_MAX + j] = p;
+        }
+    a.nimg = n_images; a.per = N / k; a.N = N; a.H = H; a.W = W;
+    const long long total = (long long)bh_chunks(12 * n_images) * N * (H / 2) * (W / 2) * 2;
+    hipLaunchKernelGGL(pack_inputs_kernel<PackGatherArgs>, dim3((unsigned)((total + 255) / 256)), dim3(256), 0, s, a, (_Float16*)y_hi,
+                       (_Float16*)y_lo, table_dev, (unsigned*)status);
+    BH_CHECK_LAUNCH();
+    return 0;
+}
+
 extern "C" {
 
 
@@ -968,8 +1008,8 @@
     for (int i = 0; i < n_images; ++i) if (!images[i]) return BINHIP_E_ARG;
     a.nimg = n_images; a.N = N; a.H = H; a.W = W;
     const long long total = (long long)bh_chunks(12 * n_images) * N * (H / 2) * (W / 2) * 2;
-    hipLaunchKernelGGL(pack_inputs_kernel, dim3((unsigned)((total + 255) / 256)), dim3(256), 0, (hipStream_t)stream,
-                       a, (_Float16*)y_hi, (_Float16*)y_lo, (unsigned*)status);
+    hipLaunchKernelGGL(pack_inputs_kernel<PackArgs>, dim3((unsigned)((total + 255) / 256)), dim3(256), 0, (hipStream_t)stream,
+                       a, (_Float16*)y_hi, (_Float16*)y_lo, (const float**)nullptr, (unsigned*)status);
     BH_CHECK_LAUNCH();
     return 0;
 }
diff --git a/bin_amd/csrc/binhip_plan.hip b/bin_amd/csrc/binhip_plan.hip
--- a/bin_amd/csrc/binhip_plan.hip
+++ b/bin_amd/csrc/binhip_plan.hip
@@ -28,6 +28,7 @@
     int kc0;
     int64_t x0, f1, blk, g0, g1, u, total;
     int64_t sync;
+    int64_t tab;
     int tiles;
     int64_t s_x0, s_f1, s_blk, s_g, s_u;
     int nt;
@@ -53,6 +54,8 @@
     w.tiles = N * ((h + 15) / 16) * ((ww + 31) / 32);
     o = (o + 127) & ~(int64_t)127;
     w.sync = o; o += 2 * (32 + 2 * (int64_t)w.tiles);
+    o = (o + 127) & ~(int64_t)127;
+    w.tab = o; o += (int64_t)(5 * BINHIP_GATHER_MAX * sizeof(void*) / 2);
     w.total = o;
     return w;
 }
@@ -92,6 +95,20 @@
     if (!resolve_shape(&p->shape, &sh)) return BINHIP_E_SHAPE;
     const size_t need = binhip_rdn_workspace_bytes(N, H, W, nin, nt, &p->shape);
     if (workspace_bytes < need) return BINHIP_E_WORKSPACE;
+    const bool gather = (p->reserved & BINHIP_PLAN_GATHER_INPUTS) != 0;
+    int gk = 0;
+    if (gather) {
+        for (int i = 0; i < nin; ++i) {
+            int k = 0;
+            while (k < BINHIP_GATHER_MAX && inputs[i * BINHIP_GATHER_MAX + k]) ++k;
+            if (k == 0) return BINHIP_E_ARG;
+            for (int j = k; j < BINHIP_GATHER_MAX; ++j)
+                if (inputs[i * BINHIP_GATHER_MAX + j]) return BINHIP_E_ARG;
+            if (i == 0) gk = k;
+            else if (k != gk) return BINHIP_E_SHAPE;
+        }
+        if (N % gk) return BINHIP_E_SHAPE;
+    } else
     for (int i = 0; i < nin; ++i) if (!inputs[i]) return BINHIP_E_ARG;
     for (int i = 0; i < sh.L; ++i)
         if (!p->w_hi[i] || !p->bias[i] || (nt == 3 && !p->w_lo[i])) return BINHIP_E_ARG;
@@ -103,7 +120,10 @@
     auto HI = [&](int64_t off) { return (void*)(base + off); };
     auto LO = [&](int64_t off, int64_t size) { return nt == 3 ? (void*)(base + off + size) : (void*)nullptr; };
 
-    int rc = binhip_pack_inputs(inputs, nin, N, H, W, HI(w.x0), LO(w.x0, w.s_x0), p->status, stream);
+    const float** gtab = gather ? (const float**)(base + w.tab) : nullptr;
+    const int gper = gather ? N / gk : 0;
+    int rc = gather ? bh_pack_inputs_gather(inputs, nin, gk, N, H, W, HI(w.x0), LO(w.x0, w.s_x0), gtab, p->status, s)
+                    : binhip_pack_inputs(inputs, nin, N, H, W, HI(w.x0), LO(w.x0, w.s_x0), p->status, stream);
     if (rc) return rc;
 
     auto mk = [&](int layer, int ks, int cin_chunks, int cout, int cout_pad, int epi, int relu, int Hc, int Wc,
@@ -128,7 +148,8 @@
         if (epi == BINHIP_EPI_FINAL || epi == BINHIP_EPI_FINAL_SUBPIX) {
             c.y_f32 = out;
             c.d.n_images = nin;
-            for (int i = 0; i < nin; ++i) c.images[i] = inputs[i];
+            if (gather) { c.gather_tab = gtab; c.gather_per = gper; }
+            else for (int i = 0; i < nin; ++i) c.images[i] = inputs[i];
         }
         return c;
     };
@@ -191,8 +212,8 @@
                           p->w_hi[sh.L + 1] && p->bias[sh.L + 1];
     if (fused_up) {
         if ((rc = bh_launch_conv(mk(sh.L, 5, c0, 12, 32, BINHIP_EPI_FINAL_SUBPIX, 0, h, ww, w.g1, w.s_g, 0, 0, -1, 0, -1, 0), s))) return rc;
-        return bh_launch_upnet_ring(HI(w.g1), LO(w.g1, w.s_g), (const float*)p->w_hi[sh.L + 1], p->bias[sh.L + 1], out, inputs, nin, N, h, ww,
-                                    G0, s);
+        return bh_launch_upnet_ring(HI(w.g1), LO(w.g1, w.s_g), (const float*)p->w_hi[sh.L + 1], p->bias[sh.L + 1], out,
+                                    gather ? nullptr : inputs, nin, N, h, ww, G0, s, gtab, gper);
     }
     if ((rc = conv(LG + 2, 3, c0, 256, 256, BINHIP_EPI_SHUFFLE, 0, h, ww, w.g1, w.s_g, 0, 0, w.u, w.s_u, -1, 0))) return rc;
     if ((rc = conv(LG + 3, 3, 4, 3, 32, BINHIP_EPI_FINAL, 0, H, W, w.u, w.s_u, 0, 0, -1, 0, -1, 0))) return rc;
diff --git a/bin_amd/csrc/binzero_regions.hip b/bin_amd/csrc/binzero_regions.hip
--- /dev/null
+++ b/bin_amd/csrc/binzero_regions.hip
@@ -0,0 +1,93 @@
+#include <hip/hip_runtime.h>
+#include <stdint.h>
+#include "../../include/binzero.h"
+
+namespace {
+constexpr int ZR_THREADS = 256;
+constexpr int ZR_UNROLL = 4;
+constexpr int64_t ZR_CHUNK = (int64_t)ZR_THREADS * ZR_UNROLL * 16;
+
+struct ZeroTable {
+    BinZeroRegion row[BINZERO_MAX_REGIONS];
+    int first_block[BINZERO_MAX_REGIONS + 1];
+    int n;
+};
+static_assert(sizeof(BinZeroRegion) == 16, "BinZeroRegion layout");
+static_assert(sizeof(ZeroTable) <= 3840, "the table must fit the by-value argument limit");
+
+struct Split { int64_t head, nvec, tail; };
+__host__ __device__ inline Split split_region(uintptr_t p, int64_t bytes) {
+    Split s;
+    const int64_t to_boundary = (int64_t)((16 - (p & 15)) & 15);
+    s.head = to_boundary < bytes ? to_boundary : bytes;
+    s.nvec = (bytes - s.head) / 16;
+    s.tail = bytes - s.head - 16 * s.nvec;
+    return s;
+}
+inline int64_t region_blocks(const BinZeroRegion& r) {
+    const Split s = split_region((uintptr_t)r.ptr, r.bytes);
+    const int64_t nb = (16 * s.nvec + ZR_CHUNK - 1) / ZR_CHUNK;
+    return nb > 0 ? nb : 1;
+}
+}
+
+__global__ void __launch_bounds__(ZR_THREADS)
+zero_regions_kernel(const ZeroTable tab) {
+    int lo = 0, hi = tab.n;
+    while (hi - lo > 1) {
+        const int mid = (lo + hi) >> 1;
+        if (tab.first_block[mid] <= (int)blockIdx.x) lo = mid; else hi = mid;
+    }
+    const BinZeroRegion& r = tab.row[lo];
+    unsigned char* const p = (unsigned char*)r.ptr;
+    const Split s = split_region((uintptr_t)p, r.bytes);
+    const int blk = (int)blockIdx.x - tab.first_block[lo];
+    const int t = threadIdx.x;
+    uint4* const body = (uint4*)(p + s.head);
+    const uint4 z = make_uint4(0u, 0u, 0u, 0u);
+    const int64_t v0 = (int64_t)blk * (ZR_THREADS * ZR_UNROLL);
+#pragma unroll
+    for (int k = 0; k < ZR_UNROLL; ++k) {
+        const int64_t i = v0 + k * ZR_THREADS + t;
+        if (i < s.nvec) body[i] = z;
+    }
+    if (blk == 0) {
+        if (t < s.head) p[t] = 0;
+        if (t < s.tail) p[s.head + 16 * s.nvec + t] = 0;
+    }
+}
+
+int binzero_version(void) { return BINZERO_VERSION; }
+
+int binzero_regions(const BinZeroRegion* items, int n, void* stream) {
+    if (n < 0 || (n > 0 && !items)) return BINZERO_E_ARG;
+    const int64_t max_blocks = 0x7fffffff;
+    for (int i = 0; i < n; ++i) {
+        if (items[i].bytes < 0 || (items[i].bytes > 0 && !items[i].ptr)) return BINZERO_E_ARG;
+        if (items[i].bytes > 0 && region_blocks(items[i]) > max_blocks) return BINZERO_E_SHAPE;
+    }
+    hipStream_t s = (hipStream_t)stream;
+    int i = 0;
+    while (i < n) {
+        ZeroTable tab;
+        int64_t blocks = 0;
+        int k = 0;
+        for (; i < n && k < BINZERO_MAX_REGIONS; ++i) {
+            if (items[i].bytes == 0) continue;
+            const int64_t nb = region_blocks(items[i]);
+            if (blocks + nb > max_blocks) break;
+            tab.row[k] = items[i];
+            tab.first_block[k] = (int)blocks;
+            blocks += nb;
+            ++k;
+        }
+        for (int j = k; j <= BINZERO_MAX_REGIONS; ++j) tab.first_block[j] = (int)blocks;
+        for (int j = k; j < BINZERO_MAX_REGIONS; ++j) tab.row[j] = BinZeroRegion{};
+        tab.n = k;
+        if (k == 0) continue;
+        hipLaunchKernelGGL(zero_regions_kernel, dim3((unsigned)blocks), dim3(ZR_THREADS), 0, s, tab);
+        const hipError_t err = hipGetLastError();
+        if (err != hipSuccess) return (int)err;
+    }
+    return 0;
+}
diff --git a/bin_amd/models/archs/RDN.py b/bin_amd/models/archs/RDN.py
--- a/bin_amd/models/archs/RDN.py
+++ b/bin_amd/models/archs/RDN.py
@@ -158,6 +158,20 @@
                 return rdn_apply(self, frames)
             nterms = PRECISIONS[self.precision or default_precision()]
             return rdn_forward(self.kernel_weights(nterms), list(frames), flags=self.plan_flags, profiler=self.profiler)
+
+    def gathered(self, *lists):
+        from ...rdn_plan import gather_lists
+        gather_lists(lists, self.N_INPUTS)
+        flat = [t for row in lists for t in row]
+        if not all(f.is_cuda for f in flat):
+            raise RuntimeError("bin_amd: RDN sub-networks run on a HIP device only (no CPU fallback; see oracle/)")
+        with torch.cuda.device(flat[0].device):
+            if torch.is_grad_enabled() and (any(f.requires_grad for f in flat) or
+                                             any(p.requires_grad for p in self.parameters())):
+                from ...autograd import rdn_apply_gathered
+                return rdn_apply_gathered(self, [list(row) for row in lists])
+            nterms = PRECISIONS[self.precision or default_precision()]
+            return rdn_forward(self.kernel_weights(nterms), [list(row) for row in lists], flags=self.plan_flags, profiler=self.profiler)
 
 
 class RDN_residual_interp_2_input(_RDNBase):
@@ -476,6 +490,7 @@
 
 
 def _forward_four_calls(self, B):
+    from ...rdn_plan import gather_inputs_enabled
     m = self.model
     n = B[0].shape[0]
     B1, B3, B5, B7, B9, B11 = B
@@ -488,16 +503,22 @@
         assert len(out) == k
         return list(out)
 
-    I2, I4, I6, I8, I8b = parts(m.model1_1(cat((B1, B3, B5, B7, B9), 0), cat((B3, B5, B7, B9, B11), 0)), 5)
+    if gather_inputs_enabled():
+        def call(mod, *lists):
+            return mod.gathered(*lists)
+    else:
+        def call(mod, *lists):
+            return mod(*[cat(row, 0) for row in lists])
+
+    I2, I4, I6, I8, I8b = parts(call(m.model1_1, (B1, B3, B5, B7, B9), (B3, B5, B7, B9, B11)), 5)
     h4, h6, h8 = (cells[k](x, None)[0] for k, x in enumerate((I4, I6, I8)))
-    I3, I5, I7, J3, J5, J7 = parts(m.model2_1(cat((I2, I4, I6, h4, h6, h8), 0), cat((I2, I4, I6, I4, I6, I8), 0),
-                                              cat((I4, I6, I8, I6, I8, I8b), 0)), 6)
+    I3, I5, I7, J3, J5, J7 = parts(call(m.model2_1, (I2, I4, I6, h4, h6, h8), (I2, I4, I6, I4, I6, I8),
+                                        (I4, I6, I8, I6, I8, I8b)), 6)
     h5, h7 = cells[3](I5, None)[0], cells[4](I7, None)[0]
-    I4pp, I6pp, J4pp, J6pp = parts(m.model3_1(cat((I3, I5, h5, h7), 0), cat((B3, B5, B5, B7), 0), cat((I3, I5, J3, J5), 0),
-                                              cat((I5, I7, J5, J7), 0), cat((B5, B7, B7, B9), 0)), 4)
+    I4pp, I6pp, J4pp, J6pp = parts(call(m.model3_1, (I3, I5, h5, h7), (B3, B5, B5, B7), (I3, I5, J3, J5),
+                                        (I5, I7, J5, J7), (B5, B7, B7, B9)), 4)
     h6pp = cells[5](I6pp, None)[0]
-    I5ppp, J5ppp = parts(m.model4_1(cat((I4, h6pp), 0), cat((I4, I6), 0), cat((I4pp, J4pp), 0), cat((I6pp, J6pp), 0),
-                                    cat((I6, I8), 0)), 2)
+    I5ppp, J5ppp = parts(call(m.model4_1, (I4, h6pp), (I4, I6), (I4pp, J4pp), (I6pp, J6pp), (I6, I8)), 2)
     self.Ft_p_1 = (I6, I8, I8b, None, J3, J5, J7, J4pp, J6pp, J5ppp)
     return (I2, I4, I6, I8, I3, I5, I7, I4pp, I6pp, I5ppp, I8b, J7, J6pp, J5ppp)
 
diff --git a/bin_amd/ops.py b/bin_amd/ops.py
--- a/bin_amd/ops.py
+++ b/bin_amd/ops.py
@@ -762,3 +762,18 @@
         return
     with torch.cuda.device(device):
         L.check(L.emalib().binema_step(table, n, decay, _stream()), "ema_step")
+
+
+def zero_regions(tensors):
+    tensors = [t for t in tensors if t.numel() > 0]
+    if not tensors:
+        return
+    _need_cuda(*tensors)
+    for t in tensors:
+        if not t.is_contiguous() or t.device != tensors[0].device:
+            raise ValueError(f"zero_regions: contiguous tensors on one device, got strides {tuple(t.stride())} on {t.device}")
+    table = (L.BinZeroRegion * len(tensors))()
+    for r, t in zip(table, tensors):
+        r.ptr, r.bytes = t.data_ptr(), t.numel() * t.element_size()
+    with torch.cuda.device(tensors[0].device):
+        L.check(L.zerolib().binzero_regions(table, len(tensors), _stream()), "zero_regions")
diff --git a/bin_amd/rdn_plan.py b/bin_amd/rdn_plan.py
--- a/bin_amd/rdn_plan.py
+++ b/bin_amd/rdn_plan.py
@@ -237,6 +237,17 @@
                 self._dgrad[key] = RdnDgradWeights(dict(module.named_parameters()), self.n_inputs, nterms, shape=self.shape,
                                                    fused=(self.fused_train_w4, self.fused_train[1]) if fused else None)
         return self._dgrad[key]
+
+
+_ZERO_BIAS = {}
+
+
+def _zero_bias(device, n):
+    key = (device.type, device.index)
+    z = _ZERO_BIAS.get(key)
+    if z is None or z.numel() < n:
+        z = _ZERO_BIAS[key] = torch.zeros(n, dtype=torch.float32, device=device)
+    return z
 
 
 class RdnDgradWeights:
@@ -291,7 +302,7 @@
             scratch.append(zb)
         relayout_batch(items)
         del scratch
-        self.zero_bias = torch.zeros(max(D * G0, G0 + C * G, 256, 1152), dtype=torch.float32, device=dev)
+        self.zero_bias = _zero_bias(dev, max(D * G0, G0 + C * G, 256, 1152))
 
     def fill_plan(self, plan):
         plan.shape = c_shape(self.shape)
@@ -342,21 +353,77 @@
     return flags
 
 
+def gather_inputs_enabled():
+    return _os.environ.get("BIN_AMD_GATHER_INPUTS", "1") != "0"
+
+
+class GatherError(ValueError):
+
+    def __init__(self, code, msg):
+        super().__init__(f"bin_amd: gathered RDN inputs: {msg}")
+        self.code = code
+
+
+def gather_lists(lists, n_inputs):
+    if len(lists) != n_inputs:
+        raise GatherError(L.E_SHAPE, f"{len(lists)} input positions for a network of {n_inputs}")
+    first = None
+    for i, row in enumerate(lists):
+        if not isinstance(row, (list, tuple)) or len(row) == 0:
+            raise GatherError(L.E_ARG, f"position {i} is not a non-empty list of tensors")
+        if len(row) > L.GATHER_MAX:
+            raise GatherError(L.E_SHAPE, f"position {i} lists {len(row)} tensors, at most {L.GATHER_MAX} (BINHIP_GATHER_MAX) are gathered")
+        if len(row) != len(lists[0]):
+            raise GatherError(L.E_SHAPE, f"position {i} lists {len(row)} tensors, position 0 lists {len(lists[0])}")
+        for t in row:
+            if not isinstance(t, torch.Tensor):
+                raise GatherError(L.E_ARG, f"position {i} holds a {type(t).__name__}, not a tensor")
+            first = t if first is None else first
+            if t.device != first.device:
+                raise GatherError(L.E_ARG, f"tensors on {first.device} and {t.device} in one call")
+            if t.dim() != 4 or t.shape[1] != 3 or t.shape != first.shape or t.dtype != first.dtype:
+                raise GatherError(L.E_SHAPE, f"every tensor must be one [n,3,H,W] shape and dtype: {tuple(first.shape)} {first.dtype} "
+                                             f"and {tuple(t.shape)} {t.dtype}")
+    return len(lists[0]), first.shape[0]
+
+
+def gather_table(lists):
+    arr = (C.c_void_p * (len(lists) * L.GATHER_MAX))()
+    for i, row in enumerate(lists):
+        for j, t in enumerate(row):
+            arr[i * L.GATHER_MAX + j] = t.data_ptr()
+    return arr
+
+
 def rdn_forward(weights, inputs, out=None, ws=None, flags=0, profiler=None):
-    _need_cuda(*inputs)
-    with on_device(inputs[0]):
-        return _rdn_forward(weights, inputs, out, ws, flags, profiler)
-
-
-def _rdn_forward(weights, inputs, out, ws, flags, profiler):
-    inputs = [t.contiguous().float() for t in inputs]
-    n, c, h, w = inputs[0].shape
+    gathered = len(inputs) > 0 and isinstance(inputs[0], (list, tuple))
+    if gathered:
+        gather_lists(inputs, weights.n_inputs)
+        _need_cuda(*[t for row in inputs for t in row])
+    else:
+        _need_cuda(*inputs)
+    with on_device(inputs[0][0] if gathered else inputs[0]):
+        return _rdn_forward(weights, inputs, out, ws, flags, profiler, gathered)
+
+
+def _rdn_forward(weights, inputs, out, ws, flags, profiler, gathered=False):
+    if gathered:
+        inputs = [[t.contiguous().float() for t in row] for row in inputs]
+        first = inputs[0][0]
+        n, c, h, w = first.shape
+        n *= len(inputs[0])
+        flags = int(flags or 0) | L.PLAN_GATHER_INPUTS
+        inputs_dev = first.device
+    else:
+        inputs = [t.contiguous().float() for t in inputs]
+        n, c, h, w = inputs[0].shape
+        inputs_dev = inputs[0].device
     assert c == 3 and len(inputs) == weights.n_inputs
     lib = L.lib()
     plan = L.BinRdnPlan()
     plan.N, plan.H, plan.W, plan.n_inputs, plan.nterms = n, h, w, weights.n_inputs, weights.nterms
     plan.reserved = int(flags or 0)
-    plan.status = status_word(inputs[0].device).data_ptr()
+    plan.status = status_word(inputs_dev).data_ptr()
     plan.profiler = profiler if profiler else None
     fused = None
     if plan.reserved & L.PLAN_FUSED_UPNET:
@@ -369,9 +436,9 @@
     if nbytes == 0:
         raise RuntimeError(f"bin_amd: unsupported RDN shape N={n} H={h} W={w} (H, W must be even)")
     if ws is None:
-        ws = workspace(nbytes, inputs[0].device)
+        ws = workspace(nbytes, inputs_dev)
     if out is None:
-        out = torch.empty((n, 3, h, w), dtype=torch.float32, device=inputs[0].device)
-    arr = (C.c_void_p * len(inputs))(*[t.data_ptr() for t in inputs])
+        out = torch.empty((n, 3, h, w), dtype=torch.float32, device=inputs_dev)
+    arr = gather_table(inputs) if gathered else (C.c_void_p * len(inputs))(*[t.data_ptr() for t in inputs])
     L.check(lib.binhip_rdn_forward(C.byref(plan), arr, _ptr(out), _ptr(ws), ws.numel(), _stream()), "rdn_forward")
     return out
diff --git a/include/binhip.h b/include/binhip.h
--- a/include/binhip.h
+++ b/include/binhip.h
@@ -156,6 +156,8 @@
 #define BINHIP_PLAN_RDB3      4
 #define BINHIP_PLAN_FUSED_UPNET 8
 #define BINHIP_PLAN_FUSED_UPNET_TRAIN 16
+#define BINHIP_PLAN_GATHER_INPUTS 32
+#define BINHIP_GATHER_MAX 6
 typedef struct BinRdnPlan {
     int32_t N, H, W;
     int32_t n_inputs;
diff --git a/include/binzero.h b/include/binzero.h
--- /dev/null
+++ b/include/binzero.h
@@ -0,0 +1,28 @@
+#pragma once
+
+#include <stddef.h>
+#include <stdint.h>
+
+#ifdef __cplusplus
+extern "C" {
+#endif
+
+#define BINZERO_API __attribute__((visibility("default")))
+
+#define BINZERO_VERSION 100
+
+#define BINZERO_E_ARG   (-1)
+#define BINZERO_E_SHAPE (-2)
+
+BINZERO_API int binzero_version(void);
+
+#define BINZERO_MAX_REGIONS 128
+typedef struct BinZeroRegion {
+    void* ptr;
+    int64_t bytes;
+} BinZeroRegion;
+BINZERO_API int binzero_regions(const BinZeroRegion* items , int n, void* stream);
+
+#ifdef __cplusplus
+}
+#endif
```

Result: no change. 16.25 interpolated frames/s (-0.4%).
